# Shreyas911/MITgcm

Hardware: AMD Instinct MI355X
Metric: model-days/wallclock-sec (higher is better)
Workload: dtype f64; 1 GPU; BASELINE config 2, verification/global_ocean.90x40x15 as verified: 90x40x15 global lat-lon ocean, 1 tile of 90x40 (OL=3) on 1 GPU, restarted from the committed pickup at nIter0=36000; r* coordinate with non-linear free surface (UPDATE_CG2D every step), JMD95P, GM/Redi gkw91, CD scheme, biharmonic + harmonic viscosity, quasi-hydrostatic + NH metric + 3-D Coriolis, implicit vertical diffusion, IVDC,; tiles_per_gpu=1, parallelism=replicas1, cg2d=single-GPU kernel

## Files before the change

include/mitgcm_amd.h:

```cpp
#ifndef MITGCM_AMD_H
#define MITGCM_AMD_H

#include <stddef.h>

#ifdef __cplusplus
extern "C" {
#endif

typedef struct mgcm_model mgcm_model;

mgcm_model *mgcm_create(int sNx, int sNy, int OLx, int OLy, int Nr, int nSx, int nSy, int device);
void mgcm_destroy(mgcm_model *m);
const char *mgcm_last_error(void);

int mgcm_exch2_maps(int sNx, int sNy, int OL, int nTiles, int ldNb, int ldT, const int *tBasex, const int *tBasey,
                    const int *isNedge, const int *isSedge, const int *isEedge, const int *isWedge,
                    const int *nNeighbours, const int *neighbourId, const int *opposingSend, const int *pij,
                    const int *oi, const int *oj, const int *iLo, const int *iHi, const int *jLo, const int *jHi,
                    int useCubedSphereExchange, long *src, long *u1, long *v1, long *u0, long *v0);

int mgcm_set_param(mgcm_model *m, const char *name, double value);
double mgcm_get_param(mgcm_model *m, const char *name);

int mgcm_set_iter(mgcm_model *m, int myIter);
int mgcm_add_iter(mgcm_model *m, int inc);
int mgcm_tracer_parity(mgcm_model *m, int set);

int mgcm_ptracers_alloc(mgcm_model *m, int n);
int mgcm_ptracer_param(mgcm_model *m, int iTracer, const char *name, double value);
double mgcm_ptracer_param_get(mgcm_model *m, int iTracer, const char *name);
int mgcm_ptracers_count(mgcm_model *m);

int mgcm_put(mgcm_model *m, const char *name, const double *host, long count);
int mgcm_get(mgcm_model *m, const char *name, double *host, long count);
int mgcm_put_async(mgcm_model *m, const char *name, const double *host, long count);
int mgcm_put_batch_async(mgcm_model *m, int n, const char *const *names, const double *const *hosts,
                         const long *counts);
double *mgcm_device_ptr(mgcm_model *m, const char *name);

int mgcm_set_halo_map(mgcm_model *m, const long *src_of_point, long count);

int mgcm_set_uv_map(mgcm_model *m, const long *u1, const long *v1, const long *u0, const long *v0,
                    const int *tileFace, const int *tileEdge, long count);

int mgcm_init(mgcm_model *m);

int mgcm_thermodynamics(mgcm_model *m);
int mgcm_dynamics(mgcm_model *m);
int mgcm_solve_for_pressure(mgcm_model *m);
int mgcm_momentum_correction_step(mgcm_model *m);
int mgcm_integr_continuity(mgcm_model *m);
int mgcm_update_r_star(mgcm_model *m);
int mgcm_calc_r_star(mgcm_model *m);
int mgcm_blocking_exchanges(mgcm_model *m);
int mgcm_oceanic_phys(mgcm_model *m);
int mgcm_tracer_step(mgcm_model *m);
int mgcm_stagger_exchanges(mgcm_model *m);
int mgcm_exchange_host(mgcm_model *m, double *u, double *v, int nz, int vector, int withSigns);
const char *mgcm_param_name(int i);
long mgcm_field_count(mgcm_model *m, const char *name);
int mgcm_prepare(mgcm_model *m);
int mgcm_forward_step(mgcm_model *m, int nsteps);
int mgcm_set_tile_range(mgcm_model *m, int t0, int nT);
int mgcm_set_stream(mgcm_model *m, void *stream);
int mgcm_exchange_nfields(mgcm_model *m);
int mgcm_halo_pack(mgcm_model *m, const long *idx, long n, double *buf, int unpack);
int mgcm_exchange_nfields_group(mgcm_model *m, int group);
int mgcm_halo_pack_group(mgcm_model *m, int group, const long *idx, long n, double *buf, int unpack);
int mgcm_stream_handoff(mgcm_model *m, void *other, int direction);
int mgcm_tile_copy(mgcm_model *m, const char *name, int t0, int nT, void *buf, int toField);
int mgcm_begin_steps(mgcm_model *m);
int mgcm_end_steps(mgcm_model *m, int nsteps);
int mgcm_step_phase(mgcm_model *m, int phase);
int mgcm_cg2d_op(mgcm_model *m, int op, double a0, double *part);
int mgcm_cg2d_shared_bytes(mgcm_model *m);
int mgcm_cg2d_shared_export(mgcm_model *m, void *handle);
int mgcm_cg2d_shared_import(mgcm_model *m, const void *handle);
void *mgcm_get_stream(mgcm_model *m);
long mgcm_halo_sources(mgcm_model *m, int t0, int nT, long *out, long cap);
int mgcm_cg2d_tiles(mgcm_model *m, int t0, int nT);
int mgcm_cg2d_share(mgcm_model *m, mgcm_model *owner);
int mgcm_cg2d_record(mgcm_model *m, double firstResidual, double lastResidual, double rhsMax, double sumRHS,
                     int numIters, double minResidualSq, int nIterMin);
int mgcm_field_pack(mgcm_model *m, const char *name, const long *idx, long n, double *buf, int unpack);
int mgcm_exchange_field(mgcm_model *m, const char *name);

int mgcm_sync(mgcm_model *m);

int mgcm_cg2d(mgcm_model *m, double *cg2d_b, double *cg2d_x, double *firstResidual,
              double *minResidualSq, double *lastResidual, int *numIters, int *nIterMin);

int mgcm_cg2d_sum_plan(mgcm_model *m, int *plan, long capacity, int *NT, int *PPT, int *NG);

// ... 62 lines not shown
```

mitgcm_amd/_lib.py:

```python
import ctypes
import os

HERE = os.path.dirname(os.path.abspath(__file__))
LIBPATH = os.environ.get("MGCM_LIB") or os.path.join(HERE, "libmitgcm_amd.so")
_lib = None


class MgcmError(RuntimeError):
    pass


def lib():
    global _lib
    if _lib is not None:
        return _lib
    if not os.path.exists(LIBPATH):
        raise MgcmError("libmitgcm_amd.so not built (run __graft_entry__.build() or "
                        "python mitgcm_amd/build.py): the MI355X path has no CPU fallback")
    L = ctypes.CDLL(LIBPATH)
    vp, ci, cd, cs, cl = ctypes.c_void_p, ctypes.c_int, ctypes.c_double, ctypes.c_char_p, ctypes.c_long
    PD, PI, PL = ctypes.POINTER(cd), ctypes.POINTER(ci), ctypes.POINTER(cl)
    sig = {
        "mgcm_create": (vp, [ci] * 8),
        "mgcm_destroy": (None, [vp]),
        "mgcm_last_error": (cs, []),
        "mgcm_set_param": (ci, [vp, cs, cd]),
        "mgcm_set_iter": (ci, [vp, ci]),
        "mgcm_add_iter": (ci, [vp, ci]),
        "mgcm_exch2_maps": (ci, [ci] * 6 + [PI] * 16 + [ci] + [PL] * 5),
        "mgcm_tracer_parity": (ci, [vp, ci]),
        "mgcm_ptracers_alloc": (ci, [vp, ci]),
        "mgcm_ptracers_count": (ci, [vp]),
        "mgcm_ptracer_param": (ci, [vp, ci, cs, cd]),
        "mgcm_ptracer_param_get": (cd, [vp, ci, cs]),
        "mgcm_get_param": (cd, [vp, cs]),
        "mgcm_put": (ci, [vp, cs, PD, cl]),
        "mgcm_put_async": (ci, [vp, cs, PD, cl]),
        "mgcm_put_batch_async": (ci, [vp, ctypes.c_int, ctypes.POINTER(cs), ctypes.POINTER(PD), ctypes.POINTER(cl)]),
        "mgcm_get": (ci, [vp, cs, PD, cl]),
        "mgcm_device_ptr": (vp, [vp, cs]),
        "mgcm_set_halo_map": (ci, [vp, PL, cl]),
        "mgcm_set_uv_map": (ci, [vp, PL, PL, PL, PL, PI, PI, cl]),
        "mgcm_init": (ci, [vp]),
        "mgcm_dynamics": (ci, [vp]),
        "mgcm_thermodynamics": (ci, [vp]),
        "mgcm_prepare": (ci, [vp]),
        "mgcm_solve_for_pressure": (ci, [vp]),
        "mgcm_momentum_correction_step": (ci, [vp]),
        "mgcm_integr_continuity": (ci, [vp]),
        "mgcm_blocking_exchanges": (ci, [vp]),
        "mgcm_forward_step": (ci, [vp, ci]),
        "mgcm_sync": (ci, [vp]),
        "mgcm_cg2d": (ci, [vp, PD, PD, PD, PD, PD, PI, PI]),
        "mgcm_cg2d_sum_plan": (ci, [vp, PI, cl, PI, PI, PI]),
        "mgcm_solve_stats": (ci, [vp, ci, PD, PD, PI, PD]),
        "mgcm_solve_minres": (ci, [vp, ci, PD, PI]),
        "mgcm_stream_triad": (ci, [ci, cl, ci, PD]),
        "mgcm_solve_history": (ci, [vp, ci, PI, PD, PD]),
        "mgcm_monitor": (ci, [vp, PD]),
        "mgcm_kernel_ms": (cd, [vp, cs, PI]),
        "mgcm_kernel_timing": (None, [vp, ci]),
        "mgcm_set_tile_range": (ci, [vp, ci, ci]),
        "mgcm_set_stream": (ci, [vp, vp]),
        "mgcm_exchange_nfields": (ci, [vp]),
        "mgcm_halo_pack": (ci, [vp, vp, cl, vp, ci]),
        "mgcm_halo_pack_group": (ci, [vp, ci, vp, cl, vp, ci]),
        "mgcm_exchange_nfields_group": (ci, [vp, ci]),
        "mgcm_stream_handoff": (ci, [vp, vp, ci]),
        "mgcm_begin_steps": (ci, [vp]),
        "mgcm_end_steps": (ci, [vp, ci]),
        "mgcm_cg2d_shared_bytes": (ci, [vp]),
        "mgcm_cg2d_shared_export": (ci, [vp, vp]),
        "mgcm_cg2d_shared_import": (ci, [vp, vp]),
        "mgcm_tile_copy": (ci, [vp, cs, ci, ci, vp, ci]),
        "mgcm_step_phase": (ci, [vp, ci]),
        "mgcm_cg2d_op": (ci, [vp, ci, cd, vp]),
        "mgcm_cg2d_record": (ci, [vp, cd, cd, cd, cd, ci, cd, ci]),
        "mgcm_field_pack": (ci, [vp, cs, vp, cl, vp, ci]),
        "mgcm_exchange_field": (ci, [vp, cs]),
        "mgcm_oceanic_phys": (ci, [vp]),
        "mgcm_tracer_step": (ci, [vp]),
        "mgcm_stagger_exchanges": (ci, [vp]),
        "mgcm_exchange_host": (ci, [vp, PD, PD, ci, ci, ci]),
        "mgcm_field_count": (cl, [vp, cs]),
        "mgcm_param_name": (cs, [ci]),
        "mgcm_update_r_star": (ci, [vp]),
        "mgcm_calc_r_star": (ci, [vp]),
        "mgcm_get_stream": (vp, [vp]),
        "mgcm_halo_sources": (cl, [vp, ci, ci, PL, cl]),
        "mgcm_cg2d_tiles": (ci, [vp, ci, ci]),
        "mgcm_cg2d_share": (ci, [vp, vp]),
        "ini_cg2d_amd_": (None, [PI] * 6 + [PD] * 8 + [PI]),
        "cg2d_amd_": (None, [PD, PD, PD, PD, PD, PI, PI, PI]),
    }
    for name, (res, args) in sig.items():
        fn = getattr(L, name)
        fn.restype = res
        fn.argtypes = args
    _lib = L
    return L


EXPORTS = ["mgcm_create", "mgcm_destroy", "mgcm_last_error", "mgcm_set_param", "mgcm_get_param", "mgcm_put", "mgcm_put_async", "mgcm_put_batch_async",
           "mgcm_get", "mgcm_device_ptr", "mgcm_set_halo_map", "mgcm_set_uv_map", "mgcm_init", "mgcm_dynamics", "mgcm_thermodynamics",
           "mgcm_solve_for_pressure", "mgcm_momentum_correction_step", "mgcm_integr_continuity",
           "mgcm_blocking_exchanges", "mgcm_prepare", "mgcm_forward_step", "mgcm_sync", "mgcm_cg2d", "mgcm_cg2d_sum_plan", "mgcm_solve_stats", "mgcm_solve_minres", "mgcm_stream_triad", "mgcm_solve_history", "mgcm_monitor",
           "mgcm_kernel_ms", "mgcm_kernel_timing", "mgcm_set_tile_range", "mgcm_set_stream",
           "mgcm_exchange_nfields", "mgcm_halo_pack", "mgcm_tile_copy", "mgcm_begin_steps", "mgcm_step_phase", "mgcm_cg2d_op",
           "mgcm_cg2d_record", "mgcm_field_pack", "mgcm_exchange_field", "ini_cg2d_amd_",
           "cg2d_amd_", "mgcm_oceanic_phys", "mgcm_tracer_step", "mgcm_stagger_exchanges", "mgcm_exchange_host", "mgcm_field_count", "mgcm_param_name",
           "mgcm_amd_setup_", "mgcm_amd_param_", "mgcm_amd_bind_", "mgcm_amd_init_", "do_oceanic_phys_amd_",
           "thermodynamics_amd_", "dynamics_amd_", "solve_for_pressure_amd_", "momentum_correction_step_amd_",
           "integr_continuity_amd_", "do_fields_blocking_exchanges_amd_", "do_stagger_fields_exchanges_amd_", "exch_xy_rl_amd_", "exch_xyz_rl_amd_",
           "exch_uv_xy_rl_amd_", "exch_uv_xyz_rl_amd_", "global_sum_tile_rl_amd_",
           "mgcm_update_r_star", "mgcm_calc_r_star", "update_r_star_amd_", "update_cg2d_amd_", "calc_r_star_amd_",
           "mgcm_set_iter", "mgcm_add_iter", "mgcm_tracer_parity", "mgcm_exch2_maps", "mgcm_amd_host_sync_", "mgcm_amd_device_sync_", "mgcm_amd_transfer_stats_",
           "mgcm_amd_step_fence_", "mgcm_halo_pack_group", "mgcm_exchange_nfields_group", "mgcm_stream_handoff",
           "mgcm_end_steps", "mgcm_cg2d_shared_bytes", "mgcm_cg2d_shared_export", "mgcm_cg2d_shared_import",
           "mgcm_amd_set_maps_", "mgcm_amd_set_w2_", "mgcm_get_stream", "mgcm_halo_sources", "mgcm_cg2d_tiles", "mgcm_cg2d_share",
           "mgcm_ptracers_alloc", "mgcm_ptracers_count", "mgcm_ptracer_param", "mgcm_ptracer_param_get"]


def check(rc, what):
    if rc != 0:
        raise MgcmError("%s failed: %s" % (what, lib().mgcm_last_error().decode()))
```

mitgcm_amd/csrc/common.h:

```cpp
#pragma once
#include <hip/hip_runtime.h>
#include <stdint.h>
#include <stdlib.h>

namespace mgcm {

struct Dims {
  int sNx, sNy, OLx, OLy, Nr, nSx, nSy, nTiles;
  int t0, nT;
  int nx, ny;
  long n2, n3;
  long N2all, N3all;
};

#define MG_F2D_LIST(X) X(dxF) X(dyF) X(dxG) X(dyG) X(dxC) X(dyC) X(dxV) X(dyU) X(rA) X(rAw) X(rAs) X(recip_dxF) \
    X(recip_dyF) X(recip_dxC) X(recip_dyC) X(recip_dxV) X(recip_dyU) X(recip_rA) X(recip_rAw) X(recip_rAs) \
    X(fCori) X(Bo_surf) X(recip_Bo) X(tanPhiAtU) X(tanPhiAtV) X(maskInC) X(SST) X(lambdaThetaClimRelax) X(aW2d) \
    X(aS2d) X(aC2d) X(pW) X(pS) X(pC) X(etaN) X(fu) X(fv) X(etaH) X(surfaceForcingT) X(surfaceForcingS) \
    X(cg2d_b) X(cg2d_x) X(Qnet) X(EmPmR) X(SSS) X(lambdaSaltClimRelax) X(etaNm1) X(fCoriCos) X(recip_Rcol) \
    X(rSurfW) X(rSurfS) X(rLowW) X(rLowS) X(Ro_surf) X(R_low) X(rStarFacC) X(rStarFacW) X(rStarFacS) \
    X(rStarExpC) X(rStarExpW) X(rStarExpS) X(rStarDhCDt) X(rStarDhWDt) X(rStarDhSDt) X(PmEpR) X(dEtaHdt) \
    X(maskInW) X(maskInS) X(fCoriG) X(recip_rAz) X(recip_dxG) X(recip_dyG) X(etaHnm1) X(cg2d_r) X(cg2d_s) X(cg2d_q) \
    X(cg2d_min) X(cg2d_y) X(cg2d_v) X(EmPmRnext) X(rStarFacCPrev) X(rStarFacWPrev) X(rStarFacSPrev)
#define MG_F3D_LIST(X) X(hFacC) X(hFacW) X(hFacS) X(recip_hFacC) X(recip_hFacW) X(recip_hFacS) X(maskC) X(maskW) \
// ... 125 lines not shown
    if (q_ >= np_) return;                                                              \
    i = (i0) + q_ % (ni);                                                               \
    j = (j0) + q_ / (ni);                                                               \
  }
#define MG_PLANE_THREADS 256

__host__ __device__ inline int mg_col_kp(int Nr) { int kp = 1; while (kp < Nr) kp <<= 1; return kp; }
#define MG_COLS(i0, ni, j0, nj, Nr)                                                    \
  const int KP_ = mg_col_kp(Nr), NC_ = 256 / KP_;                                        \
  const int cc = (int)threadIdx.x % NC_, kk = (int)threadIdx.x / NC_;                   \
  const long col_ = (long)mg_xcd_block() * NC_ + cc;                                    \
  const long npl_ = (long)(ni) * (nj);                                                  \
  const bool valid = col_ < npl_ * d.nT;                                                \
  const int t = d.t0 + (int)(valid ? col_ / npl_ : 0);                                  \
  const int i = (i0) + (int)((valid ? col_ % npl_ : 0) % (ni));                         \
  const int j = (j0) + (int)((valid ? col_ % npl_ : 0) / (ni));
inline unsigned mg_col_blocks(int ni, int nj, int nT, int Nr) {
  const int nc = 256 / mg_col_kp(Nr);
  return (unsigned)(((long)ni * nj * nT + nc - 1) / nc);
}
#define MG_COLF(i0, ni, j0, nj, NCv)                                                   \
  const int NC_ = (NCv), KW_ = 256 / NC_;                                              \
  const int cc = (int)threadIdx.x % NC_, kk = (int)threadIdx.x / NC_;                  \
  const long col_ = (long)mg_xcd_block() * NC_ + cc;                                   \
  const long npl_ = (long)(ni) * (nj);                                                 \
  const bool valid = col_ < npl_ * d.nT;                                               \
  const int t = d.t0 + (int)(valid ? col_ / npl_ : 0);                                 \
  const int i = (i0) + (int)((valid ? col_ % npl_ : 0) % (ni));                        \
  const int j = (j0) + (int)((valid ? col_ % npl_ : 0) / (ni));
#define MG_COLF_LB(i0, ni, j0, nj, NCv, LB)                                            \
  const int NC_ = (NCv), KW_ = 256 / NC_;                                              \
  const int cc = (int)threadIdx.x % NC_, kk = (int)threadIdx.x / NC_;                  \
  const long col_ = (long)(LB) * NC_ + cc;                                             \
  const long npl_ = (long)(ni) * (nj);                                                 \
  const bool valid = col_ < npl_ * d.nT;                                               \
  const int t = d.t0 + (int)(valid ? col_ / npl_ : 0);                                 \
  const int i = (i0) + (int)((valid ? col_ % npl_ : 0) % (ni));                        \
  const int j = (j0) + (int)((valid ? col_ % npl_ : 0) / (ni));
#define MG_COLF_K(kvar) for (int kvar = kk + 1; kvar <= d.Nr; kvar += KW_)
inline int mg_colf_nc(long ncols, int Nr, int nArr) {
  (void)ncols; (void)Nr; (void)nArr;
  return 16;
}
inline size_t mg_colf_lds(int Nr, int nc, int nArr) { return (size_t)nArr * Nr * nc * sizeof(double); }
#define MG_ALLOW_LDS(kern)                                                                              \
  do {                                                                                                  \
    static const bool set_ = (hipFuncSetAttribute((const void *)(kern),                                 \
                                                  hipFuncAttributeMaxDynamicSharedMemorySize, 160 * 1024) == hipSuccess); \
    (void)set_;                                                                                         \
  } while (0)
inline unsigned mg_colf_blocks(long ncols, int nc) { return (unsigned)((ncols + nc - 1) / nc); }
enum { MG_FUSE_SFP = 1, MG_FUSE_PHI = 4, MG_FUSE_END = 8, MG_FUSE_TREX = 64, MG_FUSE_DT = 128, MG_FUSE_ETAX = 256,
       MG_FUSE_OPE = 1024, MG_FUSE_RING = 2048, MG_FUSE_RINGP = 4096, MG_FUSE_ENDS = 8192, MG_FUSE_PIPE = 16384,
       MG_FUSE_PHIP = 32768, MG_FUSE_SPEC = 65536 };
inline int mg_fuse_mask() {
  return getenv("MGCM_STEP_FUSE") ? atoi(getenv("MGCM_STEP_FUSE"))
                                  : MG_FUSE_SFP | MG_FUSE_PHI | MG_FUSE_END | MG_FUSE_DT | MG_FUSE_ETAX | MG_FUSE_OPE |
                                        MG_FUSE_RING | MG_FUSE_RINGP | MG_FUSE_ENDS | MG_FUSE_PIPE | MG_FUSE_PHIP | MG_FUSE_SPEC;
}
inline bool mg_fuse_on(int bit) { return (mg_fuse_mask() & bit) != 0; }
inline int mg_fuse_retired(const char **what) {
  static const struct { int bit; const char *what; } R[] = {
      {2, "EXCH(cg2d_x) + etaN in the single-workgroup CG2D's epilogue"},
      {16, "DO_OCEANIC_PHYS + CALC_PHI_HYD in one column pass"},
      {32, "EXCH(cg2d_x) + etaN on a third stream"},
      {512, "THERMODYNAMICS beside the pressure solve under r*"}};
  for (const auto &r : R)
    if (mg_fuse_mask() & r.bit) { *what = r.what; return r.bit; }
  return 0;
}
inline bool mg_hfuse(int bit, long nx, long ny, long nT, long Nr) {
  return mg_fuse_on(bit) && nx * ny * nT * Nr <= (1L << 21);
}
inline unsigned mg_plane_blocks(int ni, int nj, int nz) {
  return (unsigned)(((ni) * (nj) + MG_PLANE_THREADS - 1) / MG_PLANE_THREADS * (nz));
}

#define MG_OPT_LIST(X)                                                                              \
  X(momAdvection, p.momAdvection != 0, p.momAdvection != 0)        \
  X(momViscosity, p.momViscosity != 0, true)                                                        \
  X(momForcing, p.momForcing != 0, true)                                                            \
  X(rstar, p.nonlinFreeSurf > 0 && p.select_rStar > 0, true)                    \
  X(rstarOn, p.select_rStar > 0, true)                                                              \
  X(rstar2, p.select_rStar >= 2, true)                                                              \
  X(nlfs0, p.nonlinFreeSurf > 0, true)                                                              \
  X(nlfs2, p.nonlinFreeSurf > 1, true)                                                              \
  X(nlfs4, p.nonlinFreeSurf >= 4, true)                                                             \
  X(biharmonic, p.viscA4D != 0.0 || p.viscA4Z != 0.0, true)                                         \
  X(noSlipSides, p.no_slip_sides != 0, true)                                                        \
  X(noSlipBottom, p.no_slip_bottom != 0, true)                                                      \
  X(nhmTerms, p.useNHMTerms != 0, true)                                                             \
  X(metricSphere, p.metricSphere != 0, true)                                                        \
  X(coriolis, p.useCoriolis != 0, true)                                                             \
  X(cori3d, p.select3dCoriScheme >= 1, true)                                                        \
  X(cdScheme, p.useCDscheme != 0, true)                                                             \
  X(dissipInAB, p.momDissip_In_AB != 0, true)                                                       \
  X(forcingOutAB, p.momForcingOutAB == 1, false)                                                    \
  X(implicitViscosity, p.implicitViscosity != 0, false)                                             \
  X(gmAdvForm, p.GM_AdvForm != 0, false)                                                            \
  X(gmExtraDiag, p.GM_ExtraDiag != 0, false)                                                        \
  X(implicitDiffusion, p.implicitDiffusion != 0, true)                                              \
  X(tracForcingOutAB, p.tracForcingOutAB != 0, false)
struct OptsRun {
  static constexpr bool pinned = false;
#define MG_OPT_RUN(name, expr, pin) \
  __host__ __device__ __forceinline__ static bool name(const Params &p) { return (expr); }
  MG_OPT_LIST(MG_OPT_RUN)
#undef MG_OPT_RUN
};
struct OptsGO90 {
  static constexpr bool pinned = true;
#define MG_OPT_PIN(name, expr, pin) \
  __host__ __device__ __forceinline__ static constexpr bool name(const Params &p) { (void)p; return (pin); }
  MG_OPT_LIST(MG_OPT_PIN)
#undef MG_OPT_PIN
};
inline bool opts_match(const Params &p) {
#define MG_OPT_EQ(name, expr, pin) \
  if (OptsRun::name(p) != OptsGO90::name(p)) return false;
  MG_OPT_LIST(MG_OPT_EQ)
#undef MG_OPT_EQ
  return true;
}

__device__ __forceinline__ void sfp_rhs_column(const Dims &d, const Params &p, const Fields &f, long q, bool inner,
                                               const double *sE, const double *sW, const double *sN, const double *sS,
                                               int NC_, int cc) {
  if (p.useCDscheme) f.etaNm1[q] = f.etaN[q];
  f.cg2d_x[q] = f.Bo_surf[q] * f.etaN[q];
  double b = 0.0;
  if (inner) {
    if (p.useRealFreshWaterFlux) {
      const double tmpFac = p.freeSurfFac * (1.0 / p.rhoConst) * p.implicDiv2DFlow;
      b = tmpFac * f.rA[q] * f.EmPmR[q] / p.deltaTMom * f.maskInC[q];
    }
    for (int k2 = d.Nr; k2 >= 1; k2--) {
      const int s2 = (k2 - 1) * NC_ + cc;
      b = b + sE[s2] - sW[s2];
      b = b + sN[s2] - sS[s2];
    }
    b = b - p.freeSurfFac * f.rA[q] / p.deltaTMom / p.deltaTFreeSurf * (p.exactConserv ? f.etaH[q] : f.etaN[q]);
  }
  f.cg2d_b[q] = b;
}

struct TracerArgs {
  const double *tr;
  double *trNext;
  double *gNm1;
  double *scr;
  double *cp;
  const double *sfc;
  double diffKh, diffKr, dT;
  int advection, multiDim, useAB, forcing;
  int limiter;
  int scheme;
  double *gNm2;
  double relaxRate;
  double relaxVal;
  double src;
  int gm;
  double *adv1, *adv2, *gAdv;
  const double *advU, *advV, *advW;
};
__device__ __forceinline__ double ptr_surf_relax(const TracerArgs &a, double trSurf, double drF1, double hFacC1) {
  return (((a.relaxRate * (a.relaxVal - trSurf)) * drF1) * hFacC1);
}

#define MG_XMAX 8
struct XFields {
  double *p[MG_XMAX];
  int nz[MG_XMAX];
  int n;
};

__device__ __forceinline__ void exchange_multi_body(const Dims &d, const XFields &x, const long *__restrict__ map,
                                                    int nHalo, int *ctr, int hb, int k, int fi) {
  const int h = hb * (int)blockDim.x + (int)threadIdx.x;
  if (ctr && h == 0 && k == 0 && fi == 0) { ctr[0] += 1; ctr[1] += 1; }
  if (h >= nHalo || fi >= x.n || k >= x.nz[fi]) return;
  const long dst = map[2 * h], src = map[2 * h + 1];
  const long dt = dst / d.n2, dl = dst % d.n2, st = src / d.n2, sl = src % d.n2;
  const long lvl = (long)d.n2 * x.nz[fi];
  double *a = x.p[fi];
  a[dt * lvl + (long)k * d.n2 + dl] = a[st * lvl + (long)k * d.n2 + sl];
}

__device__ __forceinline__ void exchange_mixed_body(const Dims &d, double *u, double *v, int nzUV,
                                                    const long *__restrict__ uvMap, int nU, int nV, const XFields &x,
                                                    const long *__restrict__ map, int nHalo, int *ctr, int hb, int k,
                                                    int z) {
  const int h = hb * (int)blockDim.x + (int)threadIdx.x;
  if (ctr && h == 0 && k == 0 && z == 0) { ctr[0] += 1; ctr[1] += 1; }
  if (z == 0) {
    if (h >= nU + nV || k >= nzUV) return;
    const long dst = uvMap[2 * h], code = uvMap[2 * h + 1];
    const long N2 = d.n2 * d.nTiles, s = (code > 0 ? code : -code) - 1;
    const long n3 = d.n2 * nzUV, lvl = (long)k * d.n2;
    auto at = [&](long g) -> long { return (g / d.n2) * n3 + lvl + g % d.n2; };
    const double val = s < N2 ? u[at(s)] : v[at(s - N2)];
    (h < nU ? u : v)[at(dst)] = code > 0 ? val : -val;
    return;
  }
  const int fi = z - 1;
  if (h >= nHalo || fi >= x.n || k >= x.nz[fi]) return;
  const long dst = map[2 * h], src = map[2 * h + 1];
  const long dt = dst / d.n2, dl = dst % d.n2, st = src / d.n2, sl = src % d.n2;
  const long lvl = (long)d.n2 * x.nz[fi];
  double *a = x.p[fi];
  a[dt * lvl + (long)k * d.n2 + dl] = a[st * lvl + (long)k * d.n2 + sl];
}

struct MwgTables {
  const int *ownG;
  const int *ownC;
  const unsigned *ownNb;
  const unsigned *ownExp;
  const int *ringG;
  const unsigned *ringNb;
  const int *impC;
// ... 36 lines not shown
```

mitgcm_amd/csrc/gm_tensor.h:

```cpp
#pragma once
#include "common.h"

namespace mgcm {

__device__ __forceinline__ void gm_slope_gkw91(const Params &p, double dSx, double dSy, double dSr, double &SlopeX,
                                               double &SlopeY, double &SlopeSqr, double &taper) {
  const double GM_bigSlope = 1.0e+02, maxSlopeSqr = p.GM_maxSlope * p.GM_maxSlope;
  if (dSr != 0.0 && dSr <= p.GM_Small_Number) dSr = p.GM_Small_Number;
  if (dSr == 0.0) {
    SlopeX = dSx != 0.0 ? copysign(GM_bigSlope, dSx) : 0.0;
    SlopeY = dSy != 0.0 ? copysign(GM_bigSlope, dSy) : 0.0;
  } else {
    const double dRdSigmaLtd = 1.0 / dSr;
    SlopeX = dSx * dRdSigmaLtd;
    SlopeY = dSy * dRdSigmaLtd;
  }
  SlopeSqr = SlopeX * SlopeX + SlopeY * SlopeY;
  taper = 1.0;
  if (SlopeSqr >= p.GM_slopeSqCutoff) { SlopeSqr = p.GM_slopeSqCutoff; taper = 0.0; }
  if (SlopeSqr == 0.0) taper = 1.0;
  else if (SlopeSqr > maxSlopeSqr && SlopeSqr < p.GM_slopeSqCutoff) taper = maxSlopeSqr / SlopeSqr;
}

__device__ __forceinline__ void gm_tensor_body(const Dims &d, const Params &p, const Fields &f, int lb) {
  MG_PLANE_LB(2 - d.OLx, d.nx - 2, 2 - d.OLy, d.ny - 2, z, lb)
  const int t = d.t0 + z / d.Nr, k = z % d.Nr + 1;
  const int Nr = d.Nr;
  auto rho = [&](int ii, int jj, int kk) { return f.rhoInSitu[MG_I3(d, ii, jj, kk, t)]; };
  auto sX = [&](int ii, int jj, int kk) {
    return f.maskW[MG_I3(d, ii, jj, kk, t)] * f.recip_dxC[MG_I2(d, ii, jj, t)] * (rho(ii, jj, kk) - rho(ii - 1, jj, kk));
  };
  auto sY = [&](int ii, int jj, int kk) {
    return f.maskS[MG_I3(d, ii, jj, kk, t)] * f.recip_dyC[MG_I2(d, ii, jj, t)] * (rho(ii, jj, kk) - rho(ii, jj - 1, kk));
  };
  auto sR = [&](int ii, int jj, int kk) { return f.sigmaR[MG_I3(d, ii, jj, kk, t)]; };
  const double op25 = 0.25, op5 = 0.5, gs = p.gravitySign;
  const long q3 = MG_I3(d, i, j, k, t);
  const double isopycK = p.GM_isopycK * (1.0 + 1.0) * op5, bolus_K = p.GM_background_K * (1.0 + 1.0) * op5;
  double SlopeX, SlopeY, SlopeSqr, taper;
  double kwx = 0.0, kwy = 0.0, kwz = 0.0;
  if (k >= 2) {
    const double maskFk = f.maskC[MG_I3(d, i, j, k - 1, t)] * f.maskC[q3];
    const double dSx = op25 * (sX(i + 1, j, k - 1) + sX(i, j, k - 1) + sX(i + 1, j, k) + sX(i, j, k)) * maskFk;
    const double dSy = op25 * (sY(i, j + 1, k - 1) + sY(i, j, k - 1) + sY(i, j + 1, k) + sY(i, j, k)) * maskFk;
    gm_slope_gkw91(p, dSx, dSy, gs * sR(i, j, k), SlopeX, SlopeY, SlopeSqr, taper);
    kwx = -gs * SlopeX * taper;
    kwy = -gs * SlopeY * taper;
    kwz = SlopeSqr * taper;
  }
  const double Kgm_tmp = isopycK * 1.0 + p.GM_skewflx * bolus_K * 1.0;
  f.Kwx[q3] = Kgm_tmp * kwx;
  f.Kwy[q3] = Kgm_tmp * kwy;
  f.Kwz[q3] = (isopycK * 1.0) * kwz;
  const int kp1 = k + 1 < Nr ? k + 1 : Nr;
  const double maskp1 = k >= Nr ? 0.0 : 1.0;
  {
    const double mW = f.maskW[q3];
    const double dSx = sX(i, j, k) * mW;
    const double dSy = op25 * (sY(i - 1, j + 1, k) + sY(i, j + 1, k) + sY(i - 1, j, k) + sY(i, j, k)) * mW;
    const double dSr = op25 * (sR(i - 1, j, k) + sR(i, j, k) + (sR(i - 1, j, kp1) + sR(i, j, kp1)) * maskp1) * mW * gs;
    gm_slope_gkw91(p, dSx, dSy, dSr, SlopeX, SlopeY, SlopeSqr, taper);
    f.Kux[q3] = fmax((p.GM_isopycK * 1.0 * op5 * (1.0 + 1.0)) * taper, p.GM_Kmin_horiz);
    if (p.GM_ExtraDiag)
      f.Kuz[q3] = -gs * (p.GM_isopycK * 1.0 * op5 * (1.0 + 1.0) - p.GM_skewflx * p.GM_background_K * 1.0 * op5 * (1.0 + 1.0)) *
                  SlopeX * taper;
  }
  {
    const double mS = f.maskS[q3];
    const double dSx = op25 * (sX(i, j, k) + sX(i + 1, j, k) + sX(i, j - 1, k) + sX(i + 1, j - 1, k)) * mS;
    const double dSy = sY(i, j, k) * mS;
    const double dSr = op25 * (sR(i, j - 1, k) + sR(i, j, k) + (sR(i, j - 1, kp1) + sR(i, j, kp1)) * maskp1) * mS * gs;
    gm_slope_gkw91(p, dSx, dSy, dSr, SlopeX, SlopeY, SlopeSqr, taper);
    f.Kvy[q3] = fmax((p.GM_isopycK * 1.0 * op5 * (1.0 + 1.0)) * taper, p.GM_Kmin_horiz);
    if (p.GM_ExtraDiag)
      f.Kvz[q3] = -gs * (p.GM_isopycK * 1.0 * op5 * (1.0 + 1.0) - p.GM_skewflx * p.GM_background_K * 1.0 * op5 * (1.0 + 1.0)) *
                  SlopeY * taper;
  }
  if (p.GM_AdvForm) {
    double psx = 0.0, psy = 0.0;
    if (k >= 2) {
      const double halfRL = 0.5, halfSign = halfRL * gs, half_K = p.GM_background_K * (1.0 + 1.0) * op25;
      const double slopeCutoff = sqrt(p.GM_slopeSqCutoff), loc_maxSlope = p.GM_maxSlope * 1.0;
      const double maxSlopeSqr = loc_maxSlope * loc_maxSlope;
      auto psi = [&](double Slope, double dSdr) {
        if (dSdr <= p.GM_Small_Number) dSdr = p.GM_Small_Number;
        Slope = Slope / dSdr;
        double tp = 1.0;
        if (fabs(Slope) >= slopeCutoff) { Slope = copysign(slopeCutoff, Slope); tp = 0.0; }
        const double Smod = fabs(Slope);
        if (Smod > loc_maxSlope && Smod < slopeCutoff) tp = maxSlopeSqr / (Slope * Slope + p.GM_Small_Number);
        return Slope * tp * (half_K * (1.0 + 1.0));
      };
      const double mkW = f.maskW[MG_I3(d, i, j, k - 1, t)] * f.maskW[q3];
      psx = psi((sX(i, j, k - 1) + sX(i, j, k)) * halfRL * mkW, (sR(i - 1, j, k) + sR(i, j, k)) * halfSign * mkW);
      const double mkS = f.maskS[MG_I3(d, i, j, k - 1, t)] * f.maskS[q3];
      psy = psi((sY(i, j, k - 1) + sY(i, j, k)) * halfRL * mkS, (sR(i, j - 1, k) + sR(i, j, k)) * halfSign * mkS);
    }
    f.GM_PsiX[q3] = psx;
    f.GM_PsiY[q3] = psy;
  }
}

}
```

mitgcm_amd/csrc/kernels_dyn.hip:

```cpp
#include <cstdlib>

#include "common.h"
#include "launch.h"
#include "phys.h"
#include "rstar.h"
#include <cstring>
#include <cstdio>
#include <type_traits>

namespace mgcm {

__device__ __forceinline__ double hfacz(const Dims &d, const Fields &f, int i, int j, int k, int t) {
  if (i < 2 - d.OLx || j < 2 - d.OLy) return 0.0;
  double h = fmin(f.hFacW[MG_I3(d, i, j, k, t)], f.hFacW[MG_I3(d, i, j - 1, k, t)]);
  h = fmin(f.hFacS[MG_I3(d, i, j, k, t)], h);
  h = fmin(f.hFacS[MG_I3(d, i - 1, j, k, t)], h);
  return h;
}

template <class O = OptsRun>
__device__ __forceinline__ double h0facz(const Dims &d, const Params &p, const Fields &f, int i, int j, int k, int t) {
  if (!(O::momViscosity(p) && O::noSlipSides(p) && O::nlfs0(p))) return hfacz(d, f, i, j, k, t);
  if (i < 2 - d.OLx || j < 2 - d.OLy) return 0.0;
  return fmin(fmin(f.h0FacW[MG_I3(d, i, j, k, t)], f.h0FacW[MG_I3(d, i, j - 1, k, t)]),
              fmin(f.h0FacS[MG_I3(d, i, j, k, t)], f.h0FacS[MG_I3(d, i - 1, j, k, t)]));
}

template <bool HO = false>
__device__ __forceinline__ void del2uv_body(const Dims &d, const Params &p, const Fields &f, int lb,
                                            const long *__restrict__ srcOf = nullptr) {
  MG_PLANE_LB(1 - d.OLx, d.nx, 1 - d.OLy, d.ny, z, lb)
  const int t = d.t0 + z / d.Nr, k = z % d.Nr + 1;
  const long q3 = MG_I3(d, i, j, k, t);
  if (i < 2 - d.OLx || i > d.sNx + d.OLx - 1 || j < 2 - d.OLy || j > d.sNy + d.OLy - 1) {
    f.del2u[q3] = 0.0;
    f.del2v[q3] = 0.0;
    return;
  }
  const double drF = f.drF[k - 1];
  auto uv3 = [&](int ii, int jj) { return HO ? mg_at_source3(d, srcOf, ii, jj, k, t) : MG_I3(d, ii, jj, k, t); };
  const long qv[5] = {uv3(i, j), uv3(i - 1, j), uv3(i + 1, j), uv3(i, j - 1), uv3(i, j + 1)};
  auto qvAt = [&](int ii, int jj) { return qv[jj == j ? (ii == i ? 0 : ii < i ? 1 : 2) : (jj < j ? 3 : 4)]; };
#define U(ii, jj) f.uVel[HO ? qvAt(ii, jj) : MG_I3(d, ii, jj, k, t)]
#define V(ii, jj) f.vVel[HO ? qvAt(ii, jj) : MG_I3(d, ii, jj, k, t)]
#define G2(a, ii, jj) f.a[MG_I2(d, ii, jj, t)]
#define G3(a, ii, jj) f.a[MG_I3(d, ii, jj, k, t)]
  {
    auto fz = [&](int ii) { return drF * G3(hFacC, ii, j) * G2(dyF, ii, j) * G2(recip_dxF, ii, j) * (U(ii + 1, j) - U(ii, j)) * 1.0; };
    auto fm = [&](int jj) {
      return drF * hfacz(d, f, i, jj, k, t) * G2(dxV, i, jj) * G2(recip_dyU, i, jj) * (U(i, jj) - U(i, jj - 1));
    };
    double v4 = f.recip_drF[k - 1] * G3(recip_hFacW, i, j) * G2(recip_rAw, i, j) *
                (fz(i) - fz(i - 1) + fm(j + 1) - fm(j)) * G3(maskW, i, j);
    if (p.no_slip_sides) {
      const double hS = G3(h0FacW, i, j) - h0facz(d, p, f, i, j, k, t);
      const double hN = G3(h0FacW, i, j) - h0facz(d, p, f, i, j + 1, k, t);
      v4 = v4 - G3(recip_hFacW, i, j) * G2(recip_rAw, i, j) *
                    (hS * G2(dxV, i, j) * G2(recip_dyU, i, j) + hN * G2(dxV, i, j + 1) * G2(recip_dyU, i, j + 1)) * U(i, j) *
                    p.sideDragFactor * G3(maskW, i, j);
    }
    f.del2u[q3] = v4;
  }
  {
    auto fz = [&](int ii) {
      return drF * hfacz(d, f, ii, j, k, t) * G2(dyU, ii, j) * G2(recip_dxV, ii, j) * (V(ii, j) - V(ii - 1, j)) * 1.0;
    };
    auto fm = [&](int jj) { return drF * G3(hFacC, i, jj) * G2(dxF, i, jj) * G2(recip_dyF, i, jj) * (V(i, jj + 1) - V(i, jj)); };
    double v4 = f.recip_drF[k - 1] * G3(recip_hFacS, i, j) * G2(recip_rAs, i, j) *
                (fz(i + 1) - fz(i) + fm(j) - fm(j - 1)) * G3(maskS, i, j);
    if (p.no_slip_sides) {
      const double hW = G3(h0FacS, i, j) - h0facz(d, p, f, i, j, k, t);
      const double hE = G3(h0FacS, i, j) - h0facz(d, p, f, i + 1, j, k, t);
      v4 = v4 - G3(recip_hFacS, i, j) * G2(recip_rAs, i, j) *
                    (hW * G2(dyU, i, j) * G2(recip_dxV, i, j) + hE * G2(dyU, i + 1, j) * G2(recip_dxV, i + 1, j)) * V(i, j) *
                    p.sideDragFactor * G3(maskS, i, j);
    }
    f.del2v[q3] = v4;
  }
#undef U
#undef V
#undef G2
#undef G3
}
__global__ void __launch_bounds__(256) k_del2uv(Dims d, Params p, Fields f) { del2uv_body(d, p, f, mg_xcd_block()); }

template <bool HO = false>
__device__ __forceinline__ void phi_hyd_body(const Dims &d, const Params &p, const Fields &f, int nc, int lb,
                                             const long *__restrict__ srcOf = nullptr, int fromX = 0) {
  extern __shared__ __attribute__((aligned(16))) double lds[];
  MG_COLF_LB(-1, d.sNx + 3, -1, d.sNy + 3, nc, lb)
  const int Nr = d.Nr, NS = Nr * NC_;
  double *sM = lds, *sP = lds + NS, *sPh = lds + 2 * NS, *sC = lds + 3 * NS, *sU = lds + 4 * NS, *sV = lds + 5 * NS;
  const bool qh = p.quasiHydrostatic && (p.select3dCoriScheme >= 1 || p.useNHMTerms);
  const bool rstar = p.nonlinFreeSurf > 0 && p.select_rStar > 0;
  const bool ring = i >= 0 && j >= 0;
  const double recip_rhoConst = 1.0 / p.rhoConst;
  const long q2 = MG_I2(d, i, j, t);
  double hoFacC = 0.0, hoDhC = 0.0, hoDhW = 0.0, hoDhS = 0.0;
  const bool hoStash = HO && Nr >= 2 && KW_ >= 4;
  auto hoD0 = [&](long r) {
    double fc_ = 0.0, c_ = 0.0, w_ = 0.0, s_ = 0.0;
    if constexpr (HO) r_star_next_point<false>(d, p, f, srcOf, r, fromX, fc_, c_, w_, s_);
    return c_ * (f.Ro_surf[r] - f.R_low[r]) * f.rA[r];
  };
  bool hoHave = false;
  if (valid) MG_COLF_K(k) {
    const int me = (k - 1) * NC_ + cc;
    double dRlocM = 0.5 * f.drC[k - 1];
    if (k == 1) dRlocM = f.rF[0] - f.rC[0];
    const double dRlocP = (k == Nr) ? (f.rC[k - 1] - f.rF[k]) : 0.5 * f.drC[k];
    const long q3 = MG_I3(d, i, j, k, t);
    double hoOp[7] = {0.0, 0.0, 0.0, 0.0, 0.0, 0.0, 0.0};
    if constexpr (HO) {
      if (rstar) {
        hoOp[0] = f.drF[k - 1]; hoOp[1] = f.h0FacC[q3]; hoOp[2] = f.rA[q2];
        if (ring) { hoOp[3] = f.h0FacW[q3]; hoOp[4] = f.rAw[q2]; hoOp[5] = f.h0FacS[q3]; hoOp[6] = f.rAs[q2]; }
      }
    }
    double a = f.rhoInSitu[q3];
    if (qh) {
      const double scalingFactor = p.rhoConst * p.gravitySign * (1.0 / p.gravity);
      const long qc = HO ? mg_at_source3(d, srcOf, i, j, k, t) : q3;
      const long qe = HO ? mg_at_source3(d, srcOf, i + 1, j, k, t) : MG_I3(d, i + 1, j, k, t);
      const long qn = HO ? mg_at_source3(d, srcOf, i, j + 1, k, t) : MG_I3(d, i, j + 1, k, t);
      const double u0 = f.uVel[qc], u1 = f.uVel[qe];
      const double v0 = f.vVel[qc], v1 = f.vVel[qn];
      double gW = 0.0;
      if (p.select3dCoriScheme >= 1) gW = f.fCoriCos[q2] * (1.0 * 0.5 * (u0 + u1) - 0.0 * 0.5 * (v0 + v1));
      if (p.useNHMTerms) gW = gW + ((u0 * u0 + u1 * u1) + (v0 * v0 + v1 * v1)) * 0.5 * p.recip_rSphere;
      a = a + scalingFactor * gW;
    }
    if (rstar) f.alphaRho[q3] = a;
    sM[me] = dRlocM * p.gravity * a * recip_rhoConst;
    sP[me] = dRlocP * p.gravity * a * recip_rhoConst;
    if (rstar) {
      if constexpr (HO) {
        if (!hoHave) {
          r_star_next_point<true>(d, p, f, srcOf, q2, fromX, hoFacC, hoDhC, hoDhW, hoDhS);
          hoHave = true;
        }
        sC[me] = hoDhC * hoOp[0] * hoOp[1] * hoOp[2];
        if (ring) {
          sU[me] = hoDhW * hoOp[0] * hoOp[3] * hoOp[4];
          sV[me] = hoDhS * hoOp[0] * hoOp[5] * hoOp[6];
        }
      } else {
        const double drF = f.drF[k - 1];
        sC[me] = f.rStarDhCDt[q2] * drF * f.h0FacC[q3] * f.rA[q2];
        if (ring) {
          sU[me] = f.rStarDhWDt[q2] * drF * f.h0FacW[q3] * f.rAw[q2];
          sV[me] = f.rStarDhSDt[q2] * drF * f.h0FacS[q3] * f.rAs[q2];
        }
      }
    }
  }
  if constexpr (HO) {
    if (valid && rstar) {
      if (!hoHave && kk == 0) r_star_next_point<true>(d, p, f, srcOf, q2, fromX, hoFacC, hoDhC, hoDhW, hoDhS);
      if (hoStash && ring) {
        if (kk == KW_ / 4) sPh[cc] = hoD0(q2 - 1);
        if (kk == KW_ / 2) sPh[NC_ + cc] = hoD0(q2 - d.nx);
      }
    }
  }
  __syncthreads();
  if (valid && kk == 0) {
    double hoW = 0.0, hoS = 0.0;
    if constexpr (HO) {
      if (rstar && hoStash && ring) { hoW = sPh[cc]; hoS = sPh[NC_ + cc]; }
    }
    double phF = 0.0;
    for (int k2 = 1; k2 <= Nr; k2++) {
      const int s2 = (k2 - 1) * NC_ + cc;
      const double phC = phF + sM[s2];
      phF = phC + sP[s2];
      sPh[s2] = phC;
    }
    if (rstar) {
      auto d0 = [&](long r) {
        if constexpr (HO) {
          if (r == q2) return hoDhC * (f.Ro_surf[r] - f.R_low[r]) * f.rA[r];
          if (hoStash) return r == q2 - 1 ? hoW : hoS;
          return hoD0(r);
        } else {
          return f.rStarDhCDt[r] * (f.Ro_surf[r] - f.R_low[r]) * f.rA[r];
        }
      };
      double c = d0(q2);
      double u = ring ? 0.5 * (d0(q2 - 1) + c) : 0.0, v = ring ? 0.5 * (d0(q2 - d.nx) + c) : 0.0;
      for (int k2 = 1; k2 <= Nr; k2++) {
        const int s2 = (k2 - 1) * NC_ + cc;
        const double cc2 = sC[s2];
        sC[s2] = c;
        c = c - cc2;
        if (ring) {
          const double uu = sU[s2], vv = sV[s2];
          sU[s2] = u;
          sV[s2] = v;
          u = u - uu;
          v = v - vv;
        }
      }
    }
  }
  __syncthreads();
  if (valid) MG_COLF_K(k) {
    const int me = (k - 1) * NC_ + cc;
    const long q3 = MG_I3(d, i, j, k, t);
    if (rstar) {
      f.dWtC[q3] = sC[me];
      if (ring) { f.dWtU[q3] = sU[me]; f.dWtV[q3] = sV[me]; }
    }
    if (ring) {
      const double phC = sPh[me];
      f.phiHydC[q3] = phC;
      if (p.storePhiHyd4Phys) {
        double tot;
        if (rstar && p.nonlinFreeSurf >= 4) {
          const double dPhiRef = (f.Ro_surf[q2] - f.rC[k - 1]) * p.gravity;
          if constexpr (HO) tot = phC * hoFacC + fmax(dPhiRef, 0.0) * (hoFacC - 1.0) + 0.0;
          else tot = phC * f.rStarFacC[q2] + fmax(dPhiRef, 0.0) * (f.rStarFacC[q2] - 1.0) + 0.0;
        } else {
          tot = phC + f.Bo_surf[q2] * f.etaN[q2] + 0.0;
        }
        f.totPhiHyd[q3] = tot;
      }
    }
  }
}
__global__ void __launch_bounds__(256) k_phi_hyd(Dims d, Params p, Fields f, int nc) {
  phi_hyd_body(d, p, f, nc, mg_xcd_block());
}
constexpr int PHI_CH = 10;
template <bool RS, bool QH, int NRC = 0>
__device__ __forceinline__ void phi_flat_body(const Dims &d, const Params &p, const Fields &f, int lb) {
  constexpr int o = RS ? 1 : 0;
// ... 1848 lines not shown
```

mitgcm_amd/csrc/kernels_rstar.hip:

```cpp
#include "common.h"
#include "launch.h"
#include "phys.h"
#include "rstar.h"
#include "ucg2d.h"

namespace mgcm {

template <bool FUSE>
__global__ void __launch_bounds__(256) k_calc_r_star(Dims d, Params p, Fields f, const long *__restrict__ srcOf, int fromX) {
  calc_r_star_body<FUSE>(d, p, f, srcOf, (int)blockIdx.x, fromX);
}
template <bool FUSE>
__global__ void __launch_bounds__(256) k_rstar_exch(Dims d, Params p, Fields f, const long *__restrict__ srcOf, int nbR,
                                                    XFields x, const long *__restrict__ map, int nHalo, int *ctr, int nbX,
                                                    int nzMax, int fromX, int empNext) {
  const int b = (int)blockIdx.x;
  if (b < nbR) { calc_r_star_body<FUSE>(d, p, f, srcOf, b, fromX, empNext); return; }
  const int r = b - nbR;
  exchange_multi_body(d, x, map, nHalo, ctr, r % nbX, (r / nbX) % nzMax, r / (nbX * nzMax));
}

template <bool FUSE>
__global__ void __launch_bounds__(256) k_rstar_exmix(Dims d, Params p, Fields f, const long *__restrict__ srcOf, int nbR,
                                                     int fromX, double *u, double *v, int nzUV,
                                                     const long *__restrict__ uvMap, int nU, int nV, XFields x,
                                                     const long *__restrict__ map, int nHalo, int nbH, int nzMax) {
  const int b = (int)blockIdx.x;
  if (b < nbR) { calc_r_star_body<FUSE>(d, p, f, srcOf, b, fromX); return; }
  const int r = b - nbR;
  exchange_mixed_body(d, u, v, nzUV, uvMap, nU, nV, x, map, nHalo, nullptr, r % nbH, (r / nbH) % nzMax, r / (nbH * nzMax));
}

template <bool SFP, int PH>
__global__ void __launch_bounds__(256) k_update_r_star_cg2d_a(Dims d, Params p, Fields f, int nc, int opIn,
                                                              const long *__restrict__ srcOf, int nbPc,
                                                              const int *iterPtr, int nbPh) {
  extern __shared__ __attribute__((aligned(16))) double lds[];
  int lb = mg_xcd_block();
  if constexpr (PH != 0) {
    if (lb < nbPh) { phys_hoist_body(d, p, f, iterPtr, srcOf, lb); return; }
    lb -= nbPh;
  }
  if (lb < nbPc) { ucg2d_p_point(d, p, f, srcOf, lb); return; }
  lb -= nbPc;
  MG_COLF_LB(1 - d.OLx, d.nx, 1 - d.OLy, d.ny, nc, lb)
  const int NS = d.Nr * NC_;
  double *sW = lds, *sS = lds + NS;
  double *fE = lds + 2 * NS, *fW = lds + 3 * NS, *fN = lds + 4 * NS, *fS = lds + 5 * NS;
  const long q = MG_I2(d, i, j, t);
  const bool op = opIn && p.nonlinFreeSurf > 2 && i >= 1 && i <= d.sNx + 1 && j >= 1 && j <= d.sNy + 1;
  const bool inner = i >= 1 && i <= d.sNx && j >= 1 && j <= d.sNy;
  if (valid) {
    const double fc = f.rStarFacC[q], fw = f.rStarFacW[q], fs = f.rStarFacS[q];
    if constexpr (PH == 2) {
      if (kk == 0) { f.rStarFacCPrev[q] = fc; f.rStarFacWPrev[q] = fw; f.rStarFacSPrev[q] = fs; }
    }
    double fwE = 0.0, fsN = 0.0;
    if (SFP && inner) { fwE = f.rStarFacW[MG_I2(d, i + 1, j, t)]; fsN = f.rStarFacS[MG_I2(d, i, j + 1, t)]; }
    MG_COLF_K(k) {
      const long q3 = MG_I3(d, i, j, k, t);
      const double hC = f.h0FacC[q3] * fc, hW = f.h0FacW[q3] * fw, hS = f.h0FacS[q3] * fs;
      f.hFacC[q3] = hC;
      f.hFacW[q3] = hW;
      f.hFacS[q3] = hS;
      if (f.maskC[q3] != 0.0) f.recip_hFacC[q3] = 1.0 / hC;
      if (f.maskW[q3] != 0.0) f.recip_hFacW[q3] = 1.0 / hW;
      if (f.maskS[q3] != 0.0) f.recip_hFacS[q3] = 1.0 / hS;
      const int me = (k - 1) * NC_ + cc;
      if (op) {
        double faceArea = f.dyG[q] * f.drF[k - 1] * hW;
        sW[me] = faceArea * f.recip_dxC[q];
        faceArea = f.dxG[q] * f.drF[k - 1] * hS;
        sS[me] = faceArea * f.recip_dyC[q];
      }
      if (SFP) {
        if (p.useCDscheme) {
          f.uNM1[q3] = f.uVel[q3];
          f.vNM1[q3] = f.vVel[q3];
        }
        if (inner) {
          const double drF = f.drF[k - 1];
          const long qE = MG_I3(d, i + 1, j, k, t), qN = MG_I3(d, i, j + 1, k, t);
          fE[me] = f.dyG[MG_I2(d, i + 1, j, t)] * drF * (f.h0FacW[qE] * fwE) * f.gU[qE] / p.deltaTMom;
          fW[me] = f.dyG[q] * drF * hW * f.gU[q3] / p.deltaTMom;
          fN[me] = f.dxG[MG_I2(d, i, j + 1, t)] * drF * (f.h0FacS[qN] * fsN) * f.gV[qN] / p.deltaTMom;
          fS[me] = f.dxG[q] * drF * hS * f.gV[q3] / p.deltaTMom;
        }
      }
    }
  }
  __syncthreads();
  if (!valid || kk != 0) return;
  if (opIn && p.nonlinFreeSurf > 2) {
    double aW = 0.0, aS = 0.0;
    if (op) {
      for (int k = 1; k <= d.Nr; k++) {
        const int me = (k - 1) * NC_ + cc;
        aW = aW + sW[me];
        aS = aS + sS[me];
      }
      aW = aW * p.cg2dNorm * p.implicSurfPress * p.implicDiv2DFlow;
      aS = aS * p.cg2dNorm * p.implicSurfPress * p.implicDiv2DFlow;
    }
    f.aW2d[q] = aW;
    f.aS2d[q] = aS;
  }
  if (SFP) sfp_rhs_column(d, p, f, q, inner, fE, fW, fN, fS, NC_, cc);
}

__global__ void __launch_bounds__(256) k_update_cg2d_p(Dims d, Params p, Fields f, const long *__restrict__ srcOf) {
  ucg2d_p_point(d, p, f, srcOf, (int)blockIdx.x);
}

hipError_t launch_calc_r_star(const Dims &d, const Params &p, const Fields &f, const long *srcOf, hipStream_t s,
                              bool fuseEtaH, int fromX) {
  const long n = d.n2 * d.nTiles;
  hipLaunchKernelGGL(fuseEtaH ? k_calc_r_star<true> : k_calc_r_star<false>, dim3((unsigned)((n + 255) / 256)), dim3(256),
                     0, s, d, p, f, srcOf, fromX);
  return hipGetLastError();
}

hipError_t launch_rstar_exch(const Dims &d, const Params &p, const Fields &f, const long *srcOf, bool fuseEtaH,
                             const XFields &x, const long *map, int nHalo, int *ctr, hipStream_t s, int fromX, int empNext) {
  const long n = d.n2 * d.nTiles;
  const int nbR = (int)((n + 255) / 256);
  int nzMax = 1;
  for (int q = 0; q < x.n; q++) nzMax = x.nz[q] > nzMax ? x.nz[q] : nzMax;
  const int nbX = ((nHalo > 0 ? nHalo : 1) + 255) / 256;
  const unsigned nb = (unsigned)(nbR + nbX * nzMax * (x.n > 0 ? x.n : 1));
  hipLaunchKernelGGL(fuseEtaH ? k_rstar_exch<true> : k_rstar_exch<false>, dim3(nb), dim3(256), 0, s, d, p, f, srcOf, nbR, x,
                     map, nHalo, ctr, nbX, nzMax, fromX, fuseEtaH ? empNext : 0);
  return hipGetLastError();
}

hipError_t launch_rstar_exmix(const Dims &d, const Params &p, const Fields &f, const long *srcOf, bool fuseEtaH, int fromX,
                              double *u, double *v, int nzUV, const long *uvMap, int nU, int nV, const XFields &x,
                              const long *map, int nHalo, hipStream_t s) {
  const long n = d.n2 * d.nTiles;
  const int nbR = (int)((n + 255) / 256);
  int nzMax = nzUV;
  for (int q = 0; q < x.n; q++) nzMax = x.nz[q] > nzMax ? x.nz[q] : nzMax;
  const int nh = (nU + nV) > nHalo ? nU + nV : nHalo;
  const int nbH = ((nh > 0 ? nh : 1) + 255) / 256;
  const unsigned nb = (unsigned)(nbR + nbH * nzMax * (1 + x.n));
  hipLaunchKernelGGL(fuseEtaH ? k_rstar_exmix<true> : k_rstar_exmix<false>, dim3(nb), dim3(256), 0, s, d, p, f, srcOf, nbR,
                     fromX, u, v, nzUV, uvMap, nU, nV, x, map, nHalo, nbH, nzMax);
  return hipGetLastError();
}

hipError_t launch_update_r_star_cg2d(const Dims &d, const Params &p, const Fields &f, const long *srcOf, hipStream_t s,
                                     bool sfp, bool opEarly, bool pcHere, const int *iterPtr, bool keepFac) {
  const long n = d.n2 * d.nTiles;
  const unsigned nb = (unsigned)((n + 255) / 256);
  const long ncol = (long)d.nx * d.ny * d.nT;
  const int nArr = sfp ? 6 : 2;
  const int nc = mg_colf_nc(ncol, d.Nr, nArr);
  auto kPlain = k_update_r_star_cg2d_a<false, 0>, kSfp = k_update_r_star_cg2d_a<true, 0>,
       kSfpPhys = k_update_r_star_cg2d_a<true, 1>, kSfpPhysKeep = k_update_r_star_cg2d_a<true, 2>;
  MG_ALLOW_LDS(kPlain);
  MG_ALLOW_LDS(kSfp);
  const int nbPc = (opEarly && pcHere && p.nonlinFreeSurf > 2) ? (int)nb : 0;
  if (iterPtr) {
    if (!sfp) return hipErrorInvalidValue;
    MG_ALLOW_LDS(kSfpPhys);
    MG_ALLOW_LDS(kSfpPhysKeep);
    const int nbPh = phys_hoist_blocks(d);
    hipLaunchKernelGGL(keepFac ? kSfpPhysKeep : kSfpPhys, dim3(mg_colf_blocks(ncol, nc) + (unsigned)(nbPc + nbPh)), dim3(256),
                       mg_colf_lds(d.Nr, nc, nArr), s, d, p, f, nc, opEarly ? 0 : 1, srcOf, nbPc, iterPtr, nbPh);
  } else if (keepFac) {
    return hipErrorInvalidValue;
  } else
    hipLaunchKernelGGL(sfp ? kSfp : kPlain, dim3(mg_colf_blocks(ncol, nc) + (unsigned)nbPc), dim3(256),
                       mg_colf_lds(d.Nr, nc, nArr), s, d, p, f, nc, opEarly ? 0 : 1, srcOf, nbPc, (const int *)nullptr, 0);
  if (p.nonlinFreeSurf > 2 && !opEarly) hipLaunchKernelGGL(k_update_cg2d_p, dim3(nb), dim3(256), 0, s, d, p, f, srcOf);
  return hipGetLastError();
}

}
```

mitgcm_amd/csrc/kernels_solve.hip:

```cpp
#include <cstdlib>

#include "cg2d.h"
#include "launch.h"
#include "gm_tensor.h"

namespace mgcm {

constexpr int CG_THREADS = 1024;
constexpr int CG_WAVES = CG_THREADS / 64;

template <int CTRL>
__device__ __forceinline__ double dpp_f64(double v) {
  const long long b = __builtin_bit_cast(long long, v);
  const int lo = __builtin_amdgcn_mov_dpp((int)(b & 0xffffffff), CTRL, 0xF, 0xF, true);
  const int hi = __builtin_amdgcn_mov_dpp((int)(b >> 32), CTRL, 0xF, 0xF, true);
  return __builtin_bit_cast(double, ((long long)hi << 32) | (unsigned)lo);
}
__device__ __forceinline__ double row_sum16(double v) {
  v = v + dpp_f64<0xB1>(v);
  v = v + dpp_f64<0x4E>(v);
  v = v + dpp_f64<0x141>(v);
  v = v + dpp_f64<0x140>(v);
  return v;
}
// ... 831 lines not shown
  (h < nU ? u : v)[at(dst)] = code > 0 ? val : -val;
}

struct UVPairs {
  double *u[3], *v[3];
  int n;
};
__global__ void __launch_bounds__(256) k_exchange_uv_pairs(Dims d, UVPairs pr, const long *__restrict__ map, int nU,
                                                           int nV) {
  const int h = (int)(blockIdx.x * blockDim.x + threadIdx.x);
  const int c = (int)blockIdx.y;
  if (h >= nU + nV || c >= pr.n) return;
  double *u = pr.u[c], *v = pr.v[c];
  const long dst = map[2 * h], code = map[2 * h + 1];
  const long N2 = d.n2 * d.nTiles, s = (code > 0 ? code : -code) - 1;
  const double val = s < N2 ? u[s] : v[s - N2];
  (h < nU ? u : v)[dst] = code > 0 ? val : -val;
}

__global__ void __launch_bounds__(256) k_exchange_mixed(Dims d, double *u, double *v, int nzUV,
                                                        const long *__restrict__ uvMap, int nU, int nV, XFields x,
                                                        const long *__restrict__ map, int nHalo, int *ctr) {
  exchange_mixed_body(d, u, v, nzUV, uvMap, nU, nV, x, map, nHalo, ctr, (int)blockIdx.x, (int)blockIdx.y, (int)blockIdx.z);
}

__global__ void __launch_bounds__(256) k_exch_eta(Dims d, Fields f, const long *__restrict__ srcOf) {
  const long q = (long)blockIdx.x * blockDim.x + threadIdx.x;
  if (q >= d.n2 * d.nTiles) return;
  const long sq = srcOf[q];
  double x = f.cg2d_x[q];
  if (sq >= 0) { x = f.cg2d_x[sq]; f.cg2d_x[q] = x; }
  f.etaN[q] = f.recip_Bo[q] * x;
}

__global__ void __launch_bounds__(256) k_exch_etaH(Dims d, Params p, Fields f, const long *__restrict__ srcOf, int atInit,
                                                   int fromX) {
  const long q = (long)blockIdx.x * blockDim.x + threadIdx.x;
  if (q >= d.n2 * d.nTiles) return;
  if (!atInit && p.nonlinFreeSurf > 0 && p.useRealFreshWaterFlux) f.PmEpR[q] = -f.EmPmR[q];
  const long sq = srcOf[q];
  const double *e = f.cg2d_b;
  double x;
  if (sq >= 0) x = e[sq];
  else {
    const long l = q % d.n2;
    const int i = (int)(l % d.nx) - d.OLx + 1, j = (int)(l / d.nx) - d.OLy + 1;
    x = (i >= 1 && i <= d.sNx && j >= 1 && j <= d.sNy) ? e[q] : fromX ? f.recip_Bo[q] * f.cg2d_x[q] : f.etaN[q];
  }
  f.etaHnm1[q] = f.etaH[q];
  f.etaN[q] = x;
  f.etaH[q] = x;
}

template <bool GM>
__global__ void __launch_bounds__(256) k_corr_cont(Dims d, Params p, Fields f, int atInit, int nc,
                                                   const long *__restrict__ etaSrc, int nbGm) {
  extern __shared__ __attribute__((aligned(16))) double lds[];
  int lb = mg_xcd_block();
  if constexpr (GM) {
    if (lb < nbGm) { gm_tensor_body(d, p, f, lb); return; }
    lb -= nbGm;
  }
  MG_COLF_LB(1, d.sNx, 1, d.sNy, nc, lb)
  const int NS = d.Nr * NC_;
  double *sDiv = lds, *sMask = lds + NS, *sU = lds + 2 * NS, *sV = lds + 3 * NS, *sH0 = lds + 4 * NS;
  const long q = MG_I2(d, i, j, t);
  const bool rstar = p.nonlinFreeSurf > 0 && p.select_rStar != 0;
  if (valid && atInit != 0) MG_COLF_K(k) {
    const int me = (k - 1) * NC_ + cc;
    const double drF = f.drF[k - 1];
    const double u0 = f.uVel[MG_I3(d, i, j, k, t)], u1 = f.uVel[MG_I3(d, i + 1, j, k, t)];
    const double v0 = f.vVel[MG_I3(d, i, j, k, t)], v1 = f.vVel[MG_I3(d, i, j + 1, k, t)];
    const double uT1 = u1 * f.dyG[MG_I2(d, i + 1, j, t)] * drF * f.hFacW[MG_I3(d, i + 1, j, k, t)];
    const double uT0 = u0 * f.dyG[q] * drF * f.hFacW[MG_I3(d, i, j, k, t)];
    const double vT1 = v1 * f.dxG[MG_I2(d, i, j + 1, t)] * drF * f.hFacS[MG_I3(d, i, j + 1, k, t)];
    const double vT0 = v0 * f.dxG[q] * drF * f.hFacS[MG_I3(d, i, j, k, t)];
    sDiv[me] = uT1 - uT0 + vT1 - vT0;
    sMask[me] = f.maskC[MG_I3(d, i, j, k, t)];
    if (rstar) sH0[me] = f.h0FacC[MG_I3(d, i, j, k, t)];
  } else if (valid) {
    const double psFac = p.pfFacMom * p.implicSurfPress;
    auto eta = [&](long qq) {
      if (!etaSrc) return f.etaN[qq];
      const long sq = etaSrc[qq];
      return f.recip_Bo[qq] * f.cg2d_x[sq >= 0 ? sq : qq];
    };
    auto phiX = [&](int ii, int jj) {
      const long qq = MG_I2(d, ii, jj, t);
      return f.recip_dxC[qq] * (f.Bo_surf[qq] * eta(qq) - f.Bo_surf[MG_I2(d, ii - 1, jj, t)] * eta(MG_I2(d, ii - 1, jj, t)));
    };
    auto phiY = [&](int ii, int jj) {
      const long qq = MG_I2(d, ii, jj, t);
      return f.recip_dyC[qq] * (f.Bo_surf[qq] * eta(qq) - f.Bo_surf[MG_I2(d, ii, jj - 1, t)] * eta(MG_I2(d, ii, jj - 1, t)));
    };
    const double pX0 = phiX(i, j), pX1 = phiX(i + 1, j), pY0 = phiY(i, j), pY1 = phiY(i, j + 1);
    MG_COLF_K(k) {
      const int me = (k - 1) * NC_ + cc;
      const long q3c = MG_I3(d, i, j, k, t), q3e = MG_I3(d, i + 1, j, k, t), q3n = MG_I3(d, i, j + 1, k, t);
      const double hW0 = f.hFacW[q3c], hW1 = f.hFacW[q3e], hS0 = f.hFacS[q3c], hS1 = f.hFacS[q3n];
      auto uCor = [&](long q3, double hW, double phiSurfX) {
        const double mW = hW != 0.0 ? 1.0 : 0.0;
        return (f.gU[q3] + p.deltaTMom * (-psFac * phiSurfX * mW)) * mW;
      };
      auto vCor = [&](long q3, double hS, double phiSurfY) {
        const double mS = hS != 0.0 ? 1.0 : 0.0;
        return (f.gV[q3] + p.deltaTMom * (-psFac * phiSurfY * mS)) * mS;
      };
      const double u0 = uCor(q3c, hW0, pX0), u1 = uCor(q3e, hW1, pX1);
      const double v0 = vCor(q3c, hS0, pY0), v1 = vCor(q3n, hS1, pY1);
      sU[me] = u0;
      sV[me] = v0;
      const double drF = f.drF[k - 1];
      const double uT1 = u1 * f.dyG[MG_I2(d, i + 1, j, t)] * drF * hW1;
      const double uT0 = u0 * f.dyG[q] * drF * hW0;
      const double vT1 = v1 * f.dxG[MG_I2(d, i, j + 1, t)] * drF * hS1;
      const double vT0 = v0 * f.dxG[q] * drF * hS0;
      sDiv[me] = uT1 - uT0 + vT1 - vT0;
      sMask[me] = f.maskC[MG_I3(d, i, j, k, t)];
      if (rstar) sH0[me] = f.h0FacC[MG_I3(d, i, j, k, t)];
    }
  }
  __syncthreads();
  if (valid && kk == 0) {
    double rStarDhDt = 0.0;
    if (p.exactConserv) {
      double hDiv = 0.0;
      for (int k2 = 1; k2 <= d.Nr; k2++) hDiv = hDiv + sMask[(k2 - 1) * NC_ + cc] * sDiv[(k2 - 1) * NC_ + cc];
      double dEtaHdt;
      if (atInit == 1 && p.nIter0 != 0 && p.useRealFreshWaterFlux) {
        dEtaHdt = f.dEtaHdt[q];
        double pm = dEtaHdt + hDiv * f.recip_rA[q];
        f.PmEpR[q] = pm * p.rhoConst;
        f.cg2d_b[q] = f.etaN[q];
      } else if (atInit == 1) {
        dEtaHdt = -(hDiv * f.recip_rA[q]);
        if (f.PmEpR) f.PmEpR[q] = 0.0;
        f.cg2d_b[q] = f.etaN[q];
      } else {
        const double facEmP = p.useRealFreshWaterFlux ? 1.0 / p.rhoConst : 0.0;
        dEtaHdt = -(hDiv * f.recip_rA[q]) - facEmP * f.EmPmR[q];
        f.cg2d_b[q] = f.etaH[q] + p.implicDiv2DFlow * dEtaHdt * p.deltaTFreeSurf;
      }
      if (f.dEtaHdt) f.dEtaHdt[q] = dEtaHdt;
      if (rstar) rStarDhDt = dEtaHdt * f.recip_Rcol[q];
    }
    double wBelow = 0.0;
    const double rA1 = f.recip_rA[q];
    for (int k2 = d.Nr; k2 >= 1; k2--) {
      const int s2 = (k2 - 1) * NC_ + cc;
      const double conv2d = -sDiv[s2];
      double w;
      if (rstar) {
        const double dh = rStarDhDt * f.drF[k2 - 1] * sH0[s2];
        if (k2 == d.Nr) w = (conv2d * rA1 - dh) * sMask[s2];
        else w = (wBelow + conv2d * rA1 - dh) * sMask[s2];
      } else if (k2 == d.Nr) {
        w = conv2d * rA1 * sMask[s2];
      } else {
        w = (wBelow + conv2d * rA1) * sMask[s2];
      }
      sDiv[s2] = w;
      wBelow = w;
    }
  }
  __syncthreads();
  if (valid) MG_COLF_K(k) {
    const int me = (k - 1) * NC_ + cc;
    const long q3 = MG_I3(d, i, j, k, t);
    f.wVel[q3] = sDiv[me];
    if (atInit == 0) { f.uVel[q3] = sU[me]; f.vVel[q3] = sV[me]; }
  }
}

template <int NR>
__device__ __forceinline__ void corr_cont_column(const Dims &d, const Params &p, long q, long q3b, long nx, long n2,
                                                 double pX0, double pX1, double pY0, double pY1, double dyG0, double dyG1,
                                                 double dxG0, double dxG1, double rA1, const double *__restrict__ gU,
                                                 const double *__restrict__ gV, const double *__restrict__ hFacW,
                                                 const double *__restrict__ hFacS, const double *__restrict__ maskC,
                                                 const double *__restrict__ drFv, double *__restrict__ uVel,
                                                 double *__restrict__ vVel, double *__restrict__ wVel, double &hDiv) {
  const double psFac = p.pfFacMom * p.implicSurfPress;
  auto uCor = [&](long q3, double hW, double phiSurfX) {
    const double mW = hW != 0.0 ? 1.0 : 0.0;
    return (gU[q3] + p.deltaTMom * (-psFac * phiSurfX * mW)) * mW;
  };
  auto vCor = [&](long q3, double hS, double phiSurfY) {
    const double mS = hS != 0.0 ? 1.0 : 0.0;
    return (gV[q3] + p.deltaTMom * (-psFac * phiSurfY * mS)) * mS;
  };
  double prod[NR];
  double wBelow = 0.0;
// ... 178 lines not shown
  hipLaunchKernelGGL(k_correction, grd, blk, 0, s, d, p, f);
  return hipGetLastError();
}

hipError_t launch_exchange_multi(const Dims &d, const XFields &x, const long *map, int nHalo, int *ctr, hipStream_t s) {
  int nzMax = 1;
  for (int q = 0; q < x.n; q++) nzMax = x.nz[q] > nzMax ? x.nz[q] : nzMax;
  dim3 blk(256), grd((unsigned)((nHalo > 0 ? nHalo : 1) + 255) / 256, nzMax, x.n);
  hipLaunchKernelGGL(k_exchange_multi, grd, blk, 0, s, d, x, map, nHalo, ctr);
  return hipGetLastError();
}

hipError_t launch_exchange_mixed(const Dims &d, double *u, double *v, int nzUV, const long *uvMap, int nU, int nV,
                                 const XFields &x, const long *map, int nHalo, int *ctr, hipStream_t s) {
  int nzMax = nzUV;
  for (int q = 0; q < x.n; q++) nzMax = x.nz[q] > nzMax ? x.nz[q] : nzMax;
  const int nh = (nU + nV) > nHalo ? nU + nV : nHalo;
  dim3 blk(256), grd((unsigned)((nh > 0 ? nh : 1) + 255) / 256, nzMax, 1 + x.n);
  hipLaunchKernelGGL(k_exchange_mixed, grd, blk, 0, s, d, u, v, nzUV, uvMap, nU, nV, x, map, nHalo, ctr);
  return hipGetLastError();
}

hipError_t launch_exchange_uv(const Dims &d, double *u, double *v, const long *map, int nU, int nV, int nz,
                              hipStream_t s) {
  if (nU + nV <= 0) return hipSuccess;
  Dims dz = d;
  dz.n3 = d.n2 * nz;
  hipLaunchKernelGGL(k_exchange_uv, dim3((unsigned)((nU + nV + 255) / 256), nz), dim3(256), 0, s, dz, u, v, map, nU,
                     nV);
  return hipGetLastError();
}

hipError_t launch_exchange_uv_pairs(const Dims &d, double *const *u, double *const *v, int n, const long *map, int nU,
                                   int nV, hipStream_t s) {
  if (nU + nV <= 0 || n <= 0) return hipSuccess;
  if (n > 3) return hipErrorInvalidValue;
  UVPairs pr{};
  for (int c = 0; c < n; c++) { pr.u[c] = u[c]; pr.v[c] = v[c]; }
  pr.n = n;
  hipLaunchKernelGGL(k_exchange_uv_pairs, dim3((unsigned)((nU + nV + 255) / 256), n), dim3(256), 0, s, d, pr, map, nU,
                     nV);
  return hipGetLastError();
}

hipError_t launch_exch_eta(const Dims &d, const Params &p, const Fields &f, const long *srcOf, bool etaH, int atInit,
                           hipStream_t s, int fromX) {
  const long n = d.n2 * d.nTiles;
  if (etaH) hipLaunchKernelGGL(k_exch_etaH, dim3((unsigned)((n + 255) / 256)), dim3(256), 0, s, d, p, f, srcOf, atInit, fromX);
  else hipLaunchKernelGGL(k_exch_eta, dim3((unsigned)((n + 255) / 256)), dim3(256), 0, s, d, f, srcOf);
  return hipGetLastError();
}

hipError_t launch_corr_cont(const Dims &d, const Params &p, const Fields &f, int atInit, hipStream_t s,
                            const long *etaSrc, bool gmNext) {
  const long ncol = (long)d.sNx * d.sNy * d.nT;
  const int nArr = (p.nonlinFreeSurf > 0 && p.select_rStar != 0) ? 5 : 4;
  if (atInit == 0 && !(p.nonlinFreeSurf > 0 && p.select_rStar != 0) && d.Nr == 50) {
    if (gmNext) return hipErrorInvalidValue;
    hipLaunchKernelGGL(k_corr_cont_march<50>, dim3((unsigned)((ncol + 255) / 256)), dim3(256), 0, s, d, p, f, etaSrc);
    return hipGetLastError();
  }
  const int nc = d.Nr >= 30 ? 32 : 16;
  if (gmNext) {
    const int nbGm = (int)mg_plane_blocks(d.nx - 2, d.ny - 2, d.nT * d.Nr);
    MG_ALLOW_LDS(k_corr_cont<true>);
    hipLaunchKernelGGL(k_corr_cont<true>, dim3(mg_colf_blocks(ncol, nc) + (unsigned)nbGm), dim3(256),
                       mg_colf_lds(d.Nr, nc, nArr), s, d, p, f, atInit, nc, etaSrc, nbGm);
    return hipGetLastError();
  }
  MG_ALLOW_LDS(k_corr_cont<false>);
  hipLaunchKernelGGL(k_corr_cont<false>, dim3(mg_colf_blocks(ncol, nc)), dim3(256), mg_colf_lds(d.Nr, nc, nArr), s, d, p, f,
                     atInit, nc, etaSrc, 0);
  return hipGetLastError();
}

hipError_t launch_halo_pack(const Dims &d, const XFields &x, const long *idx, long n, double *buf, int unpack,
                            hipStream_t s) {
  if (n <= 0) return hipSuccess;
  hipLaunchKernelGGL(k_halo_pack, dim3((unsigned)((n + 255) / 256), d.Nr, x.n), dim3(256), 0, s, d, x, idx, n, buf,
                     unpack);
  return hipGetLastError();
}

hipError_t launch_bump_counter(int *c, int nIncr, hipStream_t s) {
  hipLaunchKernelGGL(k_bump_counter, dim3(1), dim3(64), 0, s, c, nIncr);
  return hipGetLastError();
}

}
```

mitgcm_amd/csrc/kernels_step.hip:

```cpp
#include "launch.h"
#include "kernels_dyn.hip"
#include "kernels_thermo.hip"
#include "ucg2d.h"
#include "rstar.h"

namespace mgcm {

template <bool GM>
__global__ void __launch_bounds__(256) k_dt_front(Dims d, Params p, Fields f, TracerArgs aT, TracerArgs aS,
                                                  const int *iterPtr, int nc, int nbPhi, int nbDel, int nbTr) {
  int lb = mg_xcd_block();
  if (lb < nbPhi) { phi_hyd_body(d, p, f, nc, lb); return; }
  lb -= nbPhi;
  if (lb < nbDel) { del2uv_body(d, p, f, lb); return; }
  lb -= nbDel;
  if (lb < nbTr) tracer_rhs_body_br<GM>(d, p, f, aT, iterPtr, lb);
  else tracer_rhs_body_br<GM>(d, p, f, aS, iterPtr, lb - nbTr);
}

__global__ void __launch_bounds__(256) k_dt_back(Dims d, Params p, Fields f, TracerArgs aT, TracerArgs aS,
                                                 const int *iterPtr, int nc, int nbMom, int nbImp) {
  int lb = mg_xcd_block();
  if (lb < nbMom) {
    if (lb & 1) mom_step_point<false, 2>(d, p, f, iterPtr, lb >> 1);
// ... 194 lines not shown
  const int nc = mg_colf_nc(ncol, d.Nr, 3);
  const int nbImp = (int)mg_colf_blocks(ncol, nc);
  MG_ALLOW_LDS(k_tr_impl_pair);
  hipLaunchKernelGGL(k_tr_impl_pair, dim3((unsigned)(2 * nbImp)), dim3(256), mg_colf_lds(d.Nr, nc, 3), s, d, p, f, aT, aS, nc,
                     nbImp);
  return hipGetLastError();
}

hipError_t launch_dyn_thermo(const Dims &d, const Params &p, const Fields &f, const TracerArgs &aT, const TracerArgs &aS,
                             const int *iterPtr, hipStream_t s, const long *srcOf, bool gmHere, bool l1Here, bool spec) {
  const dim3 blk(256);
  int ncPhi, nArrPhi, nbPhi;
  phi_frame(d, p, ncPhi, nArrPhi, nbPhi);
  const int nbDel = del2_needed(p) ? (int)mg_plane_blocks(d.nx, d.ny, d.nT * d.Nr) : 0;
  const int nbTr = (int)mg_plane_blocks(d.sNx, d.sNy, d.nT * d.Nr);
  if (dyn_thermo_takes_gm(p)) {
    const int nbU = srcOf ? ucg2d_blocks(d) : 0;
    const int nbOp1 = 0, nbPc2 = 0, nbOp2 = nbU, nbPc3 = nbU;
    if (l1Here) launch_l1(d, p, f, nbDel, s, nbOp1, gmHere);
    else if (gmHere) return hipErrorInvalidValue;
    const bool ff4 = mom_ff4_on(true);
    const int nbMom = ff4 ? mom_ff4_blocks(d) : 2 * (int)mg_plane_blocks(d.nx, d.ny, d.nT * d.Nr);
    if (spec && (ff4 || !opts_match(p))) return hipErrorInvalidValue;
    auto l2 = ff4 ? k_dt_l2<true, true> : spec ? k_dt_l2<true, false, OptsGO90> : k_dt_l2<true, false>;
    hipLaunchKernelGGL(l2, dim3((unsigned)(nbPc2 + nbOp2 + nbMom + 2 * nbTr)), blk, 0, s, d, p, f, aT, aS, iterPtr, nbMom, nbTr,
                       srcOf, nbPc2, nbOp2, dt_long_first());
    const long ncolTr = (long)d.sNx * d.sNy * d.nT;
    const int ncTr = mg_colf_nc(ncolTr, d.Nr, 3);
    const int nbImp = (int)mg_colf_blocks(ncolTr, ncTr);
    const int nbCd = (int)mg_plane_blocks(d.nx - 2, d.ny - 2, d.nT * d.Nr);
    MG_ALLOW_LDS(k_dt_l3<OptsRun>);
    MG_ALLOW_LDS(k_dt_l3<OptsGO90>);
    auto l3 = spec ? k_dt_l3<OptsGO90> : k_dt_l3<OptsRun>;
    hipLaunchKernelGGL(l3, dim3((unsigned)(nbPc3 + nbCd + 2 * nbImp)), blk, mg_colf_lds(d.Nr, ncTr, 3), s, d, p, f, aT,
                       aS, iterPtr, ncTr, nbCd, nbImp, srcOf, nbPc3, dt_long_first());
    return hipGetLastError();
  }
  if (srcOf || !gmHere || !l1Here || spec) return hipErrorInvalidValue;
  MG_ALLOW_LDS(k_dt_front<true>);
  hipLaunchKernelGGL(k_dt_front<true>, dim3((unsigned)(nbPhi + nbDel + 2 * nbTr)), blk,
                     mg_colf_lds(d.Nr, ncPhi, nArrPhi), s, d, p, f, aT, aS, iterPtr, ncPhi, nbPhi, nbDel, nbTr);
  const int nbMom = 2 * (int)mg_plane_blocks(d.nx, d.ny, d.nT * d.Nr);
  const long ncolTr = (long)d.sNx * d.sNy * d.nT;
  const int ncTr = mg_colf_nc(ncolTr, d.Nr, 3);
  const int nbImp = (int)mg_colf_blocks(ncolTr, ncTr);
  MG_ALLOW_LDS(k_dt_back);
  hipLaunchKernelGGL(k_dt_back, dim3((unsigned)(nbMom + 2 * nbImp)), blk, mg_colf_lds(d.Nr, ncTr, 3), s, d, p, f, aT, aS,
                     iterPtr, ncTr, nbMom, nbImp);
  const hipError_t e = hipGetLastError();
  if (e != hipSuccess) return e;
  return launch_mom_tail(d, p, f, iterPtr, s);
}

__global__ void __launch_bounds__(256) k_rstar_exch_phi(Dims d, Params p, Fields f, const long *__restrict__ srcOf, int nbR,
                                                        XFields x, const long *__restrict__ map, int nHalo, int *ctr,
                                                        int nbX, int nzMax, int nbXall, int fromX, int empNext, int nc,
                                                        int nbPhi) {
  int lb = mg_xcd_block();
  if (lb < nbPhi) { phi_hyd_body<true>(d, p, f, nc, lb, srcOf, fromX); return; }
  lb -= nbPhi;
  if (lb < nbR) { calc_r_star_body<true>(d, p, f, srcOf, lb, fromX, empNext); return; }
  lb -= nbR;
  if (lb < nbXall) { exchange_multi_body(d, x, map, nHalo, ctr, lb % nbX, (lb / nbX) % nzMax, lb / (nbX * nzMax)); return; }
  del2uv_body<true>(d, p, f, lb - nbXall, srcOf);
}

bool phi_pipe_ok(const Dims &d, const Params &p) {
  (void)d;
  return mg_fuse_on(MG_FUSE_PHIP) && p.nonlinFreeSurf > 0 && p.select_rStar > 0 && p.exactConserv && !p.cubeCorners &&
         dyn_thermo_takes_gm(p) && !phi_flat_on(p);
}

hipError_t launch_phi_del2(const Dims &d, const Params &p, const Fields &f, hipStream_t s) {
  launch_l1(d, p, f, del2_needed(p) ? (int)mg_plane_blocks(d.nx, d.ny, d.nT * d.Nr) : 0, s, 0, false);
  return hipGetLastError();
}

hipError_t launch_rstar_exch_phi(const Dims &d, const Params &p, const Fields &f, const long *srcOf, const XFields &x,
                                 const long *map, int nHalo, int *ctr, hipStream_t s, int fromX, int empNext) {
  if (!phi_pipe_ok(d, p) || !srcOf || d.nT != d.nTiles) return hipErrorInvalidValue;
  const long n = d.n2 * d.nTiles;
  const int nbR = (int)((n + 255) / 256);
  int nzMax = 1;
  for (int q = 0; q < x.n; q++) nzMax = x.nz[q] > nzMax ? x.nz[q] : nzMax;
  const int nbX = ((nHalo > 0 ? nHalo : 1) + 255) / 256;
  const int nbXall = nbX * nzMax * (x.n > 0 ? x.n : 1);
  int nc, nArr, nbPhi;
  phi_frame(d, p, nc, nArr, nbPhi);
  const int nbDel = del2_needed(p) ? (int)mg_plane_blocks(d.nx, d.ny, d.nT * d.Nr) : 0;
  MG_ALLOW_LDS(k_rstar_exch_phi);
  hipLaunchKernelGGL(k_rstar_exch_phi, dim3((unsigned)(nbPhi + nbR + nbXall + nbDel)), dim3(256), mg_colf_lds(d.Nr, nc, nArr),
                     s, d, p, f, srcOf, nbR, x, map, nHalo, ctr, nbX, nzMax, nbXall, fromX, empNext, nc, nbPhi);
  return hipGetLastError();
}

}

#include "kernels_ptracers.hip"
```

mitgcm_amd/csrc/launch.h:

```cpp
#pragma once
#include "common.h"

namespace mgcm {

hipError_t launch_mom_step(const Dims &, const Params &, const Fields &, const int *, hipStream_t, bool ring = true);
bool mom_ring_separable(const Dims &, const Params &);
hipError_t launch_mom_ring(const Dims &, const Params &, const Fields &, const int *, hipStream_t);
hipError_t launch_phys_ring(const Dims &, const Params &, const Fields &, const int *, hipStream_t);
hipError_t launch_phi_hyd(const Dims &, const Params &, const Fields &, hipStream_t);

hipError_t launch_sfp_rhs(const Dims &, const Params &, const Fields &, hipStream_t);
hipError_t launch_exchange(const Dims &, double *, const long *, int, int, hipStream_t);
hipError_t launch_correction(const Dims &, const Params &, const Fields &, hipStream_t);
hipError_t launch_bump_counter(int *, int, hipStream_t);
hipError_t launch_exchange_multi(const Dims &, const XFields &, const long *, int, int *, hipStream_t);
hipError_t launch_exchange_uv(const Dims &, double *, double *, const long *, int, int, int, hipStream_t);
hipError_t launch_exchange_mixed(const Dims &, double *, double *, int, const long *, int, int, const XFields &,
                                 const long *, int, int *, hipStream_t);
hipError_t launch_exchange_uv_pairs(const Dims &, double *const *, double *const *, int, const long *, int, int,
                                   hipStream_t);
hipError_t launch_exch_eta(const Dims &, const Params &, const Fields &, const long *, bool, int, hipStream_t,
                           int fromX = 0);
hipError_t launch_corr_cont(const Dims &, const Params &, const Fields &, int, hipStream_t, const long *etaSrc = nullptr,
                            bool gmNext = false);
hipError_t launch_halo_pack(const Dims &, const XFields &, const long *, long, double *, int, hipStream_t);

hipError_t launch_cgd(const Dims &, const Params &, const Fields &, int, double, double *, hipStream_t);
hipError_t launch_cgd_record(SolveRecord *, const int *, double, double, double, double, int, double, int, hipStream_t);
hipError_t launch_field_pack(double *, const long *, long, double *, int, hipStream_t);

hipError_t launch_calc_r_star(const Dims &, const Params &, const Fields &, const long *, hipStream_t, bool fuseEtaH = false,
                              int fromX = 0);
hipError_t launch_rstar_exmix(const Dims &, const Params &, const Fields &, const long *, bool, int, double *, double *, int,
                              const long *, int, int, const XFields &, const long *, int, hipStream_t);
hipError_t launch_rstar_exch(const Dims &, const Params &, const Fields &, const long *, bool, const XFields &, const long *,
                             int, int *, hipStream_t, int fromX = 0, int empNext = 0);
hipError_t launch_update_r_star_cg2d(const Dims &, const Params &, const Fields &, const long *, hipStream_t, bool sfp = false,
                                     bool opEarly = false, bool pcHere = false, const int *iterPtr = nullptr,
                                     bool keepFac = false);

bool phys_ring_ok(const Dims &, const Params &, const Fields &);
hipError_t launch_oceanic_phys(const Dims &, const Params &, const Fields &, const int *, hipStream_t, bool gm = true,
                               bool ring = false);
hipError_t launch_tracer_step(const Dims &, const Params &, const Fields &, const TracerArgs &, const int *, hipStream_t,
                              bool impl = true, int *nLaunch = nullptr);
hipError_t launch_gm_tensor(const Dims &, const Params &, const Fields &, hipStream_t);
hipError_t launch_gm_residual_flow(const Dims &, const Params &, const Fields &, hipStream_t);

bool dyn_thermo_fusable(const Dims &, const Params &, const TracerArgs &, const TracerArgs &);
hipError_t launch_dyn_thermo(const Dims &, const Params &, const Fields &, const TracerArgs &, const TracerArgs &, const int *,
                             hipStream_t, const long *srcOf = nullptr, bool gmHere = true, bool l1Here = true, bool spec = false);
bool dyn_thermo_spec_ok(const Params &);
bool phi_pipe_ok(const Dims &, const Params &);
hipError_t launch_phi_del2(const Dims &, const Params &, const Fields &, hipStream_t);
hipError_t launch_rstar_exch_phi(const Dims &, const Params &, const Fields &, const long *, const XFields &, const long *, int,
                                 int *, hipStream_t, int fromX, int empNext);
bool dyn_thermo_takes_gm(const Params &);
bool gm_phi_fusable(const Dims &, const Params &);
hipError_t launch_gm_phi(const Dims &, const Params &, const Fields &, hipStream_t, bool op = false);
bool tracer_hpair_ok(const Dims &, const Params &, const TracerArgs &, const TracerArgs &);
hipError_t launch_tracer_hpair(const Dims &, const Params &, const Fields &, const TracerArgs &, const TracerArgs &,
                               const int *, hipStream_t);

hipError_t launch_mon_stats(const Dims &, const MonSpecs &, int, double *, int, hipStream_t);

bool ptr_batch_ok(const Dims &, const Params &, bool md);
hipError_t launch_ptracers_batch(const Dims &, const Params &, const Fields &, const TracerArgs *, const int *, int, int, int,
                                 int, const int *, hipStream_t, int *nLaunch = nullptr);

}
```

mitgcm_amd/csrc/model.hip:

```cpp
#include <hip/hip_runtime.h>

#include <cmath>
#include <cstdarg>
#include <cstdio>
#include <cstdlib>
#include <cstring>
#include <algorithm>
#include <map>
#include <utility>
#include <string>
#include <vector>

#include "../../include/mitgcm_amd.h"
#include "cg2d.h"
#include "launch.h"

namespace mgcm {
static std::vector<std::pair<uintptr_t, uintptr_t>> g_hostReg;
void mg_host_ranges_set(const uintptr_t *lo, const uintptr_t *hi, size_t n) {
  g_hostReg.clear();
  for (size_t i = 0; i < n; i++) g_hostReg.push_back({lo[i], hi[i]});
  std::sort(g_hostReg.begin(), g_hostReg.end());
}
hipError_t mg_host_copy(void *dst, const void *src, size_t bytes, hipMemcpyKind kind, hipStream_t s) {
// ... 57 lines not shown
struct PDesc {
  const char *name;
  size_t off;
  bool isint;
};
#define PD(n) {#n, offsetof(Params, n), false}
#define PI_(n) {#n, offsetof(Params, n), true}
static const PDesc PARAMS[] = {
    PD(deltaTMom), PD(deltaTFreeSurf), PD(deltaTClock), PD(abEps), PD(alph_AB), PD(beta_AB), PI_(useAB3), PD(rhoConst), PD(gBaro), PD(viscAhD), PD(viscAhZ),
    PD(viscA4D), PD(viscA4Z), PD(viscAr), PD(sideDragFactor), PD(freeSurfFac), PD(implicSurfPress),
    PD(implicDiv2DFlow), PD(rkSign), PD(afFacMom), PD(vfFacMom), PD(pfFacMom), PD(cfFacMom), PD(foFacMom),
    PD(mtFacMom), PD(cg2dNorm), PD(cg2dTolerance_sq),
    PI_(momAdvection), PI_(momViscosity), PI_(momForcing), PI_(useCoriolis), PI_(no_slip_sides),
    PI_(no_slip_bottom), PI_(selectCoriScheme), PI_(momForcingOutAB), PI_(momDissip_In_AB),
    PI_(implicitViscosity), PI_(cg2dMaxIters), PI_(cg2dUseMinResSol), PI_(cg2dNormaliseRHS), PI_(nIter0), PI_(cg2dUseFMA), PI_(useSRCGSolver), PI_(cg2dRefOrder),
    PD(gravity), PD(gravitySign), PD(rhoNil), PD(tAlpha), PD(sBeta), PD(ivdc_kappa), PD(diffKhT), PD(diffKrT),
    PD(deltaTtracer), PI_(exactConserv), PI_(tempStepping), PI_(tempAdvection), PI_(tempForcing),
    PI_(implicitDiffusion), PI_(tempAdvScheme), PI_(saltStepping), PI_(saltAdvection), PI_(saltForcing),
    PI_(saltAdvScheme), PD(diffKhS), PD(diffKrS), PI_(multiDimAdvection), PI_(multiDimCompressible), PI_(momStepping),
    PI_(eosType), PI_(allowFreezing), PI_(useRealFreshWaterFlux), PI_(useCDscheme), PI_(useGMRedi),
    PI_(periodicExternalForcing), PI_(nForcRec), PD(HeatCapacity_Cp), PD(convertFW2Salt), PD(temp_EvPrRn),
    PD(salt_EvPrRn), PD(rCD), PD(epsAB_CD), PD(externForcingPeriod), PD(externForcingCycle), PD(GM_background_K),
    PD(GM_isopycK), PD(GM_skewflx), PD(GM_maxSlope), PD(GM_Kmin_horiz), PD(GM_Small_Number), PD(GM_slopeSqCutoff),
    PI_(GM_AdvForm), PI_(GM_ExtraDiag),
    PI_(nonlinFreeSurf), PI_(select_rStar), PI_(quasiHydrostatic), PI_(useNHMTerms), PI_(select3dCoriScheme),
    PI_(selectP_inEOS_Zc), PI_(storePhiHyd4Phys), PD(hFacInf),
    PI_(vectorInvariantMomentum), PI_(selectVortScheme), PI_(selectKEscheme), PI_(upwindShear),
    PI_(staggerTimeStep), PI_(tracForcingOutAB),
};
#undef PD
#undef PI_

enum Kern { K_MOM, K_RHS, K_CG2D, K_EXCH, K_ETA, K_CORR, K_CONT, K_PHYS, K_TEMP, K_RSTAR, K_PHI, K_N };
static const char *KNAMES[K_N] = {"mom_step",   "sfp_rhs",    "cg2d",         "exchange",  "eta_update",
                                  "correction", "continuity", "oceanic_phys", "temp_step", "r_star", "phi_hyd"};

enum StepSeq { SEQ_PLAIN2 = 0, SEQ_HOIST2, SEQ_HOIST_LAST, SEQ_PLAIN1, SEQ_LAST1, SEQ_N };

struct mgcm_model {
  Dims d{};
  Params p{};
  Fields f{};
  int device = 0;
  hipStream_t stream = nullptr;
  hipStream_t ownStream = nullptr;
  hipStream_t stream2 = nullptr;
  hipEvent_t evFork = nullptr, evJoin = nullptr;
  hipEvent_t evHand = nullptr;
  bool overlap = true;
  std::vector<void *> allocs;
  std::map<std::string, double> extra;
  long *d_halo = nullptr;
  long *d_srcOf = nullptr;
  int nHalo = 0;
  long *d_haloAll = nullptr;
  int nHaloAll = 0;
  std::vector<long> h_halo;
  enum class Cg2dSolver { Bxy = 3, Mwg = 4, BlockRef = 5, MwgRef = 6 };
  Cg2dSolver solver = Cg2dSolver::Bxy;
  bool useMwg() const { return solver == Cg2dSolver::Mwg || solver == Cg2dSolver::MwgRef; }
  int nPts = 0;
  unsigned *d_nbr = nullptr;
  int *d_gofs = nullptr;
  unsigned *d_nbx = nullptr;
  int *d_blkx = nullptr;
  int nBlkX = 0;
  int bxyVar = -1;
  std::vector<int> h_dropG;
  int *d_dropG = nullptr;
  int nDropBlk = 0;
  bool noCompact = false;
  int *h_guard = nullptr;
  int *d_guard = nullptr;
  bool latlonTopology = true;
  MwgTables mwg{};
  std::vector<void *> mwgAllocs;
  void *mwgShared = nullptr;
  void *mwgBlock = nullptr;
  std::vector<int> mwgPlan;
  bool uvMap = false;
  std::vector<long> h_uv[2];
  long *d_uv[2] = {nullptr, nullptr};
  int nUvU[2] = {0, 0}, nUvV[2] = {0, 0};
  long *d_uvAll[2] = {nullptr, nullptr};
  int nUvUAll[2] = {0, 0}, nUvVAll[2] = {0, 0};
  struct UvPre { const long *map = nullptr; int nU = 0, nV = 0; } uvPre[2][2];
  int *d_tileInfo = nullptr;
  double *exchBuf[2] = {nullptr, nullptr};
  long exchCap = 0;
  bool useGraph = true;
  struct StepGraph {
    hipGraphExec_t exec = nullptr;
    double *tr[4] = {};
    int flip = 0;
    int layout = 0;
  };
  StepGraph graphs[2][8][SEQ_N];
  bool ovlAuto = false, ovlDecided = false;
  float ovlMs[2] = {0.f, 0.f};
  hipEvent_t ovlEv[2] = {nullptr, nullptr};
  double *thetaA = nullptr, *saltA = nullptr;
  int stepLayout = 0;
  int ptrRoute = 0, ptrLaunches = 0;
  int gmResFlow = 0;
  struct PTracer {
    int advScheme = 2, useGMRedi = -1;
// ... 72 lines not shown
    m->evPool.push_back(e);
  }
  return (int)m->evUsed++;
}
static int ev_begin(mgcm_model *m, int k) {
  (void)k;
  if (!m->timing) return -1;
  const int i = ev_next(m);
  if (i < 0) return -1;
  hipEventRecord(m->evPool[i], m->stream);
  return i;
}
static void ev_end(mgcm_model *m, int k, int startIdx) {
  if (!m->timing || startIdx < 0) return;
  const int i = ev_next(m);
  if (i < 0) return;
  hipEventRecord(m->evPool[i], m->stream);
  m->evPairs.push_back({k, startIdx});
}
static void ev_collect(mgcm_model *m) {
  for (auto &pr : m->evPairs) {
    float ms = 0.f;
    if (hipEventElapsedTime(&ms, m->evPool[pr.second], m->evPool[pr.second + 1]) == hipSuccess) {
      m->kms[pr.first] += ms;
      m->kcnt[pr.first] += 1;
    }
  }
  m->evPairs.clear();
  m->evUsed = 0;
}
static void ev_free(mgcm_model *m) {
  for (auto e : m->evPool) hipEventDestroy(e);
  m->evPool.clear();
  m->evUsed = 0;
}

static void build_latlon_halo(mgcm_model *m) {
  const Dims &d = m->d;
  const int Nx = d.sNx * d.nSx, Ny = d.sNy * d.nSy;
  m->h_halo.clear();
  for (int t = 0; t < d.nTiles; t++) {
    const int bi = t % d.nSx, bj = t / d.nSx;
    for (int j = 1 - d.OLy; j <= d.sNy + d.OLy; j++)
      for (int i = 1 - d.OLx; i <= d.sNx + d.OLx; i++) {
        if (i >= 1 && i <= d.sNx && j >= 1 && j <= d.sNy) continue;
        int iG = ((bi * d.sNx + i - 1) % Nx + Nx) % Nx, jG = ((bj * d.sNy + j - 1) % Ny + Ny) % Ny;
        int st = (jG / d.sNy) * d.nSx + iG / d.sNx;
        m->h_halo.push_back(MG_I2(d, i, j, t));
        m->h_halo.push_back(MG_I2(d, iG % d.sNx + 1, jG % d.sNy + 1, st));
      }
  }
}

static int upload_halo(mgcm_model *m) {
  if (m->d_halo) { hipFree(m->d_halo); m->d_halo = nullptr; }
  if (m->d_srcOf) { hipFree(m->d_srcOf); m->d_srcOf = nullptr; }
  const long N2 = m->d.n2 * m->d.nTiles;
  std::vector<long> srcOf(N2, -1);
  for (size_t h = 0; h + 1 < m->h_halo.size(); h += 2) srcOf[m->h_halo[h]] = m->h_halo[h + 1];
  HIPCHK(hipMalloc(&m->d_srcOf, N2 * sizeof(long)));
  HIPCHK(hipMemcpy(m->d_srcOf, srcOf.data(), N2 * sizeof(long), hipMemcpyHostToDevice));
  std::vector<long> loc;
  const long lo = (long)m->d.t0 * m->d.n2, hi = (long)(m->d.t0 + m->d.nT) * m->d.n2;
  for (size_t h = 0; h + 1 < m->h_halo.size(); h += 2)
    if (m->h_halo[h] >= lo && m->h_halo[h] < hi) { loc.push_back(m->h_halo[h]); loc.push_back(m->h_halo[h + 1]); }
  m->nHalo = (int)(loc.size() / 2);
  if (m->d_haloAll) { hipFree(m->d_haloAll); m->d_haloAll = nullptr; }
  m->nHaloAll = 0;
  if (m->d.nT < m->d.nTiles && !m->h_halo.empty()) {
    HIPCHK(hipMalloc(&m->d_haloAll, m->h_halo.size() * sizeof(long)));
    HIPCHK(hipMemcpy(m->d_haloAll, m->h_halo.data(), m->h_halo.size() * sizeof(long), hipMemcpyHostToDevice));
    m->nHaloAll = (int)(m->h_halo.size() / 2);
  }
  if (m->uvMap) {
    const long N2 = m->d.n2 * m->d.nTiles;
    for (int all = 0; all < 2; all++)
      for (int w = 0; w < 2; w++) {
        long *&dm = all ? m->d_uvAll[w] : m->d_uv[w];
        if (dm) { hipFree(dm); dm = nullptr; }
        const long l0 = all ? 0 : lo, l1 = all ? N2 : hi;
        const std::vector<long> &code = m->h_uv[w];
        auto srcOfCode = [](long c) { return (c > 0 ? c : -c) - 1; };
        auto early = [&](long c) { return c != 0 && code[(size_t)srcOfCode(c)] != 0; };
        std::vector<long> e, pre;
        int nu = 0, nv = 0, pu = 0, pv = 0;
        for (int c = 0; c < 2; c++)
          for (long q = l0; q < l1; q++) {
            const long cd = code[(size_t)c * N2 + q];
            if (cd == 0) continue;
            if (early(cd)) {
              if (early(code[(size_t)srcOfCode(cd)]))
                return set_err("EXCH2 vector map: the halo of tile %ld copies a halo point that itself copies one "
                               "(tiles narrower than the halo are not supported on the device)", q / m->d.n2 + 1);
              if (m->d.nT < m->d.nTiles)
                return set_err("EXCH2 vector map: tiles as narrow as the halo are not supported in tile-sharded runs");
              pre.push_back(q); pre.push_back(cd);
              (c ? pv : pu)++;
              continue;
            }
            e.push_back(q); e.push_back(cd);
            (c ? nv : nu)++;
          }
        (all ? m->nUvUAll : m->nUvU)[w] = nu;
        (all ? m->nUvVAll : m->nUvV)[w] = nv;
        m->uvPre[all][w] = mgcm_model::UvPre{};
        const size_t nMain = e.size();
        e.insert(e.end(), pre.begin(), pre.end());
        if (!e.empty()) {
          HIPCHK(hipMalloc(&dm, e.size() * sizeof(long)));
          HIPCHK(hipMemcpy(dm, e.data(), e.size() * sizeof(long), hipMemcpyHostToDevice));
          m->uvPre[all][w].map = dm + nMain;
          m->uvPre[all][w].nU = pu;
          m->uvPre[all][w].nV = pv;
        }
// ... 430 lines not shown
  const long arenaN[2] = {(long)F2_COUNT * d.N2all, (long)F3_COUNT * d.N3all};
  for (int q = 0; q < 2; q++) {
    if (hipMalloc(&arena[q], arenaN[q] * sizeof(double)) != hipSuccess ||
        hipMemset(arena[q], 0, arenaN[q] * sizeof(double)) != hipSuccess) {
      set_err("mgcm_create: hipMalloc of the %s arena (%ld doubles)", q ? "3-D" : "2-D", arenaN[q]);
      mgcm_destroy(m);
      return nullptr;
    }
    m->allocs.push_back(arena[q]);
  }
  m->f.a2 = arena[0];
  m->f.a3 = arena[1];
  int n2i = 0, n3i = 0;
  for (auto &fd : FIELDS) {
    const long n = field_count(m, fd.kind);
    double *ptr = nullptr;
    if (fd.kind == F2D) ptr = arena[0] + (long)(n2i++) * d.N2all;
    else if (fd.kind == F3D) ptr = arena[1] + (long)(n3i++) * d.N3all;
    else if (hipMalloc(&ptr, n * sizeof(double)) != hipSuccess || hipMemset(ptr, 0, n * sizeof(double)) != hipSuccess) {
      set_err("mgcm_create: hipMalloc %s (%ld doubles)", fd.name, n);
      mgcm_destroy(m);
      return nullptr;
    } else {
      m->allocs.push_back(ptr);
    }
    field_ptr(m, &fd) = ptr;
  }
  if (hipMalloc(&m->d_ctr, 2 * sizeof(int)) != hipSuccess || hipMemset(m->d_ctr, 0, 2 * sizeof(int)) != hipSuccess ||
      hipMalloc(&m->d_rec, m->maxRec * sizeof(SolveRecord)) != hipSuccess) {
    set_err("mgcm_create: counters");
    mgcm_destroy(m);
    return nullptr;
  }
  build_latlon_halo(m);
  if (hipDeviceSynchronize() != hipSuccess) {
    set_err("mgcm_create: zero fill");
    mgcm_destroy(m);
    return nullptr;
  }
  return m;
}

void mgcm_destroy(mgcm_model *m) {
  if (!m) return;
  hipSetDevice(m->device);
  if (m->stream) hipStreamSynchronize(m->stream);
  ev_collect(m);
  ev_free(m);
  drop_graphs(m);
  for (void *p : m->allocs) hipFree(p);
  if (m->monBuf) hipFree(m->monBuf);
  if (m->d_halo) hipFree(m->d_halo);
  if (m->d_srcOf) hipFree(m->d_srcOf);
  if (m->d_haloAll) hipFree(m->d_haloAll);
  for (int q = 0; q < 2; q++) {
    if (m->d_uv[q]) hipFree(m->d_uv[q]);
    if (m->d_uvAll[q]) hipFree(m->d_uvAll[q]);
  }
  if (m->d_tileInfo) hipFree(m->d_tileInfo);
  if (m->d_nbr) hipFree(m->d_nbr);
  if (m->d_gofs) hipFree(m->d_gofs);
  if (m->d_nbx) hipFree(m->d_nbx);
  if (m->d_blkx) hipFree(m->d_blkx);
  if (m->d_dropG) hipFree(m->d_dropG);
  if (m->h_guard) hipHostFree(m->h_guard);
  if (m->d_ctr) hipFree(m->d_ctr);
  for (auto &q : m->exchBuf)
    if (q) hipFree(q);
  if (m->d_rec) hipFree(m->d_rec);
  if (m->mwgShared) (void)hipIpcCloseMemHandle(m->mwgShared);
  for (void *q : m->mwgAllocs) hipFree(q);
  for (int q = 0; q < 2; q++) {
    if (m->stHost[q]) hipHostFree(m->stHost[q]);
    if (m->stEv[q]) hipEventDestroy(m->stEv[q]);
    if (m->stCopied[q]) hipEventDestroy(m->stCopied[q]);
    if (m->stDev[q]) hipFree(m->stDev[q]);
  }
  if (m->stCopy) hipStreamDestroy(m->stCopy);
  if (m->ownStream) hipStreamDestroy(m->ownStream);
  if (m->stream2) hipStreamDestroy(m->stream2);
  if (m->evFork) hipEventDestroy(m->evFork);
  if (m->evHand) hipEventDestroy(m->evHand);
  if (m->evJoin) hipEventDestroy(m->evJoin);
  for (auto &ev : m->ovlEv)
    if (ev) hipEventDestroy(ev);
  delete m;
}

int mgcm_set_param(mgcm_model *m, const char *name, double value) {
  drop_graphs(m);
  m->ptrTabDirty = true;
  if (!strcmp(name, "myIter")) {
    int it = (int)value;
    HIPCHK(hipSetDevice(m->device));
    HIPCHK(hipMemcpyAsync(m->d_ctr, &it, sizeof(int), hipMemcpyHostToDevice, m->stream));
    HIPCHK(hipStreamSynchronize(m->stream));
    return 0;
  }
  for (auto &pd : PARAMS)
    if (!strcmp(pd.name, name)) {
      char *ptr = reinterpret_cast<char *>(&m->p) + pd.off;
      if (pd.isint) *reinterpret_cast<int *>(ptr) = (int)value;
      else *reinterpret_cast<double *>(ptr) = value;
      return 0;
    }
  static const char *inert[] = {"implicitFreeSurface"};
// ... 265 lines not shown
  for (int t = 0; t < m->d.nTiles; t++) { info[t] = tileFace[t]; info[m->d.nTiles + t] = tileEdge[t]; }
  HIPCHK(hipSetDevice(m->device));
  if (m->d_tileInfo) (void)hipFree(m->d_tileInfo);
  HIPCHK(hipMalloc(&m->d_tileInfo, info.size() * sizeof(int)));
  HIPCHK(hipMemcpy(m->d_tileInfo, info.data(), info.size() * sizeof(int), hipMemcpyHostToDevice));
  m->f.tileFace = m->d_tileInfo;
  m->f.tileEdge = m->d_tileInfo + m->d.nTiles;
  m->p.cubeCorners = 1;
  m->uvMap = true;
  m->ready = false;
  drop_graphs(m);
  return 0;
}

static hipError_t uv_pre(mgcm_model *m, const Dims &d, double *u, double *v, int nz, int w, bool all = false) {
  const mgcm_model::UvPre &p = m->uvPre[all ? 1 : 0][w];
  return launch_exchange_uv(d, u, v, p.map, p.nU, p.nV, nz, m->stream);
}

static int exchange_uv(mgcm_model *m, double *u, double *v, int nz, bool withSigns) {
  if (!m->uvMap) {
    HIPCHK(launch_exchange(m->d, u, m->d_halo, m->nHalo, nz, m->stream));
    HIPCHK(launch_exchange(m->d, v, m->d_halo, m->nHalo, nz, m->stream));
    return 0;
  }
  const int w = withSigns ? 1 : 0;
  HIPCHK(uv_pre(m, m->d, u, v, nz, w));
  HIPCHK(launch_exchange_uv(m->d, u, v, m->d_uv[w], m->nUvU[w], m->nUvV[w], nz, m->stream));
  return 0;
}

static Dims all_tiles(const Dims &d) { Dims a = d; a.t0 = 0; a.nT = d.nTiles; return a; }

static hipError_t calc_r_star(mgcm_model *m, bool fuseEtaH = false, int fromX = 0, bool stagEx = false) {
  const Dims da = all_tiles(m->d);
  hipError_t e;
  if (stagEx) {
    XFields xw{};
    xw.p[0] = m->f.wVel; xw.nz[0] = m->d.Nr; xw.n = 1;
    e = uv_pre(m, m->d, m->f.uVel, m->f.vVel, m->d.Nr, 1);
    if (e != hipSuccess) return e;
    e = launch_rstar_exmix(da, m->p, m->f, m->d_srcOf, fuseEtaH, fromX, m->f.uVel, m->f.vVel, m->d.Nr, m->d_uv[1],
                           m->nUvU[1], m->nUvV[1], xw, m->d_halo, m->nHalo, m->stream);
  } else
    e = launch_calc_r_star(da, m->p, m->f, m->d_srcOf, m->stream, fuseEtaH, fromX);
  if (e != hipSuccess || !m->uvMap) return e;
  double *us[3] = {m->f.rStarFacW, m->f.rStarDhWDt, m->f.rStarExpW}, *vs[3] = {m->f.rStarFacS, m->f.rStarDhSDt,
                                                                                 m->f.rStarExpS};
  for (int q = 0; q < 3; q++)
    if ((e = uv_pre(m, da, us[q], vs[q], 1, 0, true)) != hipSuccess) return e;
  return launch_exchange_uv_pairs(da, us, vs, 3, m->d_uvAll[0], m->nUvUAll[0], m->nUvVAll[0], m->stream);
}
static hipError_t update_r_star_cg2d(mgcm_model *m, bool sfp = false, bool opEarly = false, bool pcHere = false,
                                     const int *physNext = nullptr, bool keepFac = false) {
  return launch_update_r_star_cg2d(all_tiles(m->d), m->p, m->f, m->d_srcOf, m->stream, sfp, opEarly, pcHere, physNext,
                                   keepFac);
}

int mgcm_init(mgcm_model *m) {
  auto ext = [&](const char *n, double dflt) { auto it = m->extra.find(n); return it == m->extra.end() ? dflt : it->second; };
  HIPCHK(hipSetDevice(m->device));
  const char *retired = nullptr;
  if (const int bit = mg_fuse_retired(&retired))
    return set_err("mgcm_init: MGCM_STEP_FUSE bit %d (%s) was measured slower than the default and removed in round 10 "
                   "(common.h); unset it", bit, retired);
  if (upload_halo(m)) return -1;
  m->noCompact = false;
  m->nPts = m->d.nTiles * m->d.sNx * m->d.sNy;
  BxyChoice bxy;
  if (choose_bxy(m, bxy)) return -1;
  if (m->p.cg2dRefOrder) {
    if (m->p.useSRCGSolver) return set_err("mgcm_init: cg2dRefOrder with useSRCGSolver not implemented");
    m->solver = m->nPts > cg2d_ref_max_points() ? Cg2dSolver::MwgRef : Cg2dSolver::BlockRef;
  } else
    m->solver = (bxy.var < 0 || ext("cg2dForceMwg", 0.0) != 0.0) ? Cg2dSolver::Mwg : Cg2dSolver::Bxy;
  if (m->p.useSRCGSolver && m->solver == Cg2dSolver::BlockRef)
    return set_err("mgcm_init: useSRCGSolver (CG2D_SR) is implemented in the blocked single-workgroup and the "
                   "multi-workgroup CG2D only");
  clear_bxy(m);
  if (m->solver == Cg2dSolver::Bxy ? build_bxy(m, bxy) : m->solver == Cg2dSolver::BlockRef ? build_block(m) : build_mwg(m))
    return -1;
  if (!m->h_dropG.empty()) {
    const long n2a = m->d.n2 * m->d.nTiles;
    std::vector<double> eta((size_t)n2a);
    for (const char *nm : {"etaN", "etaH"}) {
      if (!strcmp(nm, "etaH") && m->p.nIter0 == 0) continue;
      HIPCHK(hipMemcpy(eta.data(), !strcmp(nm, "etaN") ? m->f.etaN : m->f.etaH, n2a * sizeof(double), hipMemcpyDeviceToHost));
      if (land_eta_check(m, nm, eta.data(), n2a)) return -1;
    }
  }
  if ((m->p.viscA4D != 0.0 || m->p.viscA4Z != 0.0) && (m->d.OLx < 3 || m->d.OLy < 3))
    return set_err("mgcm_init: biharmonic viscosity needs OLx, OLy >= 3 (del2u of the halo ring)");
  const bool rstar = m->p.nonlinFreeSurf > 0;
  if (rstar) {
    if (m->p.nonlinFreeSurf != 4 || m->p.select_rStar != 2)
      return set_err("mgcm_init: the non-linear free surface is implemented for nonlinFreeSurf=4, select_rStar=2 only");
    if (!m->p.exactConserv) return set_err("mgcm_init: nonlinFreeSurf needs exactConserv");
  }
  if (m->p.selectP_inEOS_Zc > 2) return set_err("mgcm_init: selectP_inEOS_Zc = 3 needs the non-hydrostatic pressure");
  if (m->p.selectP_inEOS_Zc == 2 && !m->p.storePhiHyd4Phys)
    return set_err("mgcm_init: selectP_inEOS_Zc = 2 needs storePhiHyd4Phys (set_parms.F:297)");
  if (m->p.implicitViscosity && (ext("momImplVertAdv", 0.0) != 0.0 || ext("selectImplicitDrag", 0.0) != 0.0))
    return set_err("mgcm_init: momImplVertAdv / selectImplicitDrag not implemented on the device");
  if (m->p.vectorInvariantMomentum) {
    if (m->d.OLx < 2 || m->d.OLy < 2) return set_err("mgcm_init: vector-invariant momentum needs OLx, OLy >= 2");
    if (m->p.viscA4D != 0.0 || m->p.viscA4Z != 0.0)
      return set_err("mgcm_init: biharmonic viscosity with vectorInvariantMomentum not implemented on the device");
    if (m->p.useNHMTerms || m->p.select3dCoriScheme > 0 || m->p.useCDscheme)
      return set_err("mgcm_init: NH metric / 3-D Coriolis / CD scheme with vectorInvariantMomentum not implemented");
// ... 419 lines not shown

const char *mgcm_param_name(int i) {
  const int n = (int)(sizeof(PARAMS) / sizeof(PARAMS[0]));
  return (i >= 0 && i < n) ? PARAMS[i].name : nullptr;
}

long mgcm_field_count(mgcm_model *m, const char *name) {
  double *dev = nullptr;
  long n = 0;
  if (!lookup_field(m, name, &dev, &n)) { set_err("mgcm_field_count: unknown field %s", name); return -1; }
  return n;
}

static XFields blocking_fields(const mgcm_model *m, int tracers, bool totPhi) {
  XFields x{};
  double *fl[] = {m->f.uVel, m->f.vVel, m->f.wVel, m->f.theta, m->f.salt, m->f.uVelD, m->f.vVelD, m->f.totPhiHyd};
  const bool use[] = {!m->uvMap, !m->uvMap, true, m->p.tempStepping != 0, m->p.saltStepping != 0, m->p.useCDscheme != 0,
                      m->p.useCDscheme != 0, m->p.storePhiHyd4Phys != 0 && totPhi};
  for (int q = 0; q < 8; q++) {
    const bool tr = q == 3 || q == 4;
    if (use[q] && (tracers == 1 || (tracers == 2) == tr)) { x.p[x.n] = fl[q]; x.nz[x.n] = m->d.Nr; x.n++; }
  }
  return x;
}

enum StepMode {
  STEP_PLAIN = 0,
  STEP_HOIST = 1,
  STEP_LAST = 2
};
#define MG_PIPE_MIN_STEPS 4

struct StepPlan {
  bool mom, rstar;
  bool stagger;
  bool tracers;
  bool canFork, forkable, fork;
  bool forkLate, thermoLate, forkEarly, thermoInline;
  bool trEx;
  bool ringLate, ringAside;
  bool dtFused;
  bool gmPhi;
  bool physGm;
  bool ringPhys, momRing;
  bool opEarly;
  bool sfpFused;
  bool etaX;
  bool fuseEtaH, etaHAlone;
  bool endFused;
  bool stagEx;
  bool pipeOk, phiPipeOk, pipe, hoist, valid, phiPipe, phiNext, empNext;
  bool resFlow, resFlowFold;
  bool spec;
};
static StepPlan plan_step(const mgcm_model *m, StepMode mode) {
  const Params &p = m->p;
  const Dims &d = m->d;
  const bool whole = d.nT == d.nTiles;
  StepPlan pl{};
  pl.mom = p.momStepping != 0;
  pl.rstar = p.nonlinFreeSurf > 0;
  pl.stagger = p.staggerTimeStep != 0 && pl.mom;
  pl.tracers = p.tempStepping || p.saltStepping || !m->ptr.empty();
  pl.canFork = !pl.stagger && pl.mom && pl.tracers;
  pl.forkable = pl.canFork && m->overlap;
  pl.fork = pl.forkable && !m->timing;
  pl.forkLate = !pl.rstar;
  pl.thermoLate = pl.fork && pl.forkLate;
  pl.trEx = pl.thermoLate && mg_fuse_on(MG_FUSE_TREX);
  const bool ringSep = mom_ring_separable(d, p);
  pl.ringLate = pl.forkLate && ringSep && mg_fuse_on(MG_FUSE_RING);
  pl.ringAside = pl.thermoLate && pl.ringLate;
  pl.resFlow = takes_res_flow(m);
  pl.dtFused = pl.forkable && pl.rstar && dyn_thermo_fusable(d, p, tracer_args(m, false), tracer_args(m, true));
  const bool gmFold = pl.dtFused && dyn_thermo_takes_gm(p);
  pl.spec = gmFold && dyn_thermo_spec_ok(p);
  pl.forkEarly = pl.fork && !pl.thermoLate && !pl.dtFused;
  pl.thermoInline = !pl.stagger && !pl.fork && !pl.dtFused;
  pl.gmPhi = (pl.stagger || pl.thermoLate) && !pl.dtFused && !m->timing && gm_phi_fusable(d, p);
  pl.physGm = !gmFold && !pl.gmPhi;
  pl.opEarly = gmFold && p.nonlinFreeSurf > 2 && whole && mg_fuse_on(MG_FUSE_OPE);
  pl.sfpFused = mg_fuse_on(MG_FUSE_SFP) && pl.rstar && whole;
  pl.etaX = p.exactConserv && mg_fuse_on(MG_FUSE_ETAX) && whole;
  pl.fuseEtaH = p.exactConserv && pl.rstar;
  pl.etaHAlone = p.exactConserv && !pl.fuseEtaH;
  pl.endFused = pl.mom && pl.rstar && !pl.stagger && !m->uvMap && whole && mg_hfuse(MG_FUSE_END, d.nx, d.ny, d.nT, d.Nr);
  pl.stagEx = pl.mom && pl.rstar && !pl.endFused && pl.stagger && pl.tracers && m->uvMap && whole &&
              mg_hfuse(MG_FUSE_ENDS, d.nx, d.ny, d.nT, d.Nr);
  const bool totPhiHalo = p.eosType == 1 && p.selectP_inEOS_Zc == 2 && !p.storePhiHyd4Phys;
  pl.resFlowFold = pl.resFlow && pl.dtFused;
  pl.pipeOk = gmFold && pl.sfpFused && pl.endFused && mg_fuse_on(MG_FUSE_PIPE) && p.select_rStar > 0 &&
              p.useRealFreshWaterFlux && p.exactConserv && m->d_srcOf && !totPhiHalo && !pl.resFlow;
  pl.phiPipeOk = pl.pipeOk && phi_pipe_ok(d, p);
  pl.pipe = mode != STEP_PLAIN;
  pl.hoist = mode == STEP_HOIST;
  pl.valid = !pl.pipe || pl.pipeOk;
  pl.phiPipe = pl.pipe && pl.phiPipeOk;
  pl.phiNext = pl.hoist && pl.phiPipe;
  pl.empNext = pl.hoist && p.periodicExternalForcing;
  pl.ringPhys = !pl.pipe && !pl.ringAside && ringSep && mg_fuse_on(MG_FUSE_RINGP) && phys_ring_ok(d, p, m->f);
  pl.momRing = !pl.ringAside && !pl.ringPhys;
  return pl;
}
static int step_layout_bits(const StepPlan &pl) {
  return (pl.dtFused ? 1 : 0) | (pl.forkable && !pl.dtFused ? 4 : 0) | (pl.forkable && pl.forkLate ? 8 : 0) |
         (pl.pipe ? 16 : 0) | (pl.phiPipe ? 32 : 0) | (pl.spec ? 64 : 0);
}

static int fork_thermo(mgcm_model *m, bool ring, bool trEx) {
  HIPCHK(hipEventRecord(m->evFork, m->stream));
  HIPCHK(hipStreamWaitEvent(m->stream2, m->evFork, 0));
  if (ring) HIPCHK(launch_mom_ring(m->d, m->p, m->f, m->d_ctr, m->stream2));
  if (tracers_on(m, m->stream2)) return -1;
  if (trEx) {
    const XFields xt = blocking_fields(m, 2);
    if (xt.n > 0) HIPCHK(launch_exchange_multi(m->d, xt, m->d_halo, m->nHalo, nullptr, m->stream2));
  }
  HIPCHK(hipEventRecord(m->evJoin, m->stream2));
  return 0;
}

static int one_step(mgcm_model *m, StepMode mode = STEP_PLAIN) {
  const StepPlan pl = plan_step(m, mode);
  if (!pl.valid) return set_err("one_step: the pipelined step does not apply to this model");
  const int fromX = pl.etaX ? 1 : 0;
  m->mwg.exclusive = pl.thermoLate ? 1 : 0;
  m->stepLayout = step_layout_bits(pl);
  m->gmResFlow = 0;
  if (!pl.pipe) TIMED(K_PHYS, launch_oceanic_phys(m->d, m->p, m->f, m->d_ctr, m->stream, pl.physGm, pl.ringPhys));
  if (pl.forkEarly && fork_thermo(m, false, false)) return -1;
  if (pl.thermoInline && tracers_on(m, m->stream)) return -1;
  if (pl.mom) {
    if (pl.dtFused) {
      TIMED(K_MOM, launch_dyn_thermo(m->d, m->p, m->f, tracer_args(m, false), tracer_args(m, true), m->d_ctr, m->stream,
                                     pl.opEarly ? m->d_srcOf : nullptr, !pl.pipe, !pl.phiPipe, pl.spec));
      std::swap(m->f.theta, m->f.thetaNext);
      std::swap(m->f.salt, m->f.saltNext);
      if (pl.resFlowFold && res_flow_on(m, m->stream)) return -1;
      if (ptracers_on(m, m->stream)) return -1;
    } else if (pl.gmPhi) {
      TIMED(K_PHI, launch_gm_phi(m->d, m->p, m->f, m->stream));
      TIMED(K_MOM, launch_mom_step(m->d, m->p, m->f, m->d_ctr, m->stream, pl.momRing));
    } else if (dynamics_on(m, pl.momRing)) return -1;
    if (pl.forkEarly) HIPCHK(hipStreamWaitEvent(m->stream, m->evJoin, 0));
    if (pl.rstar)
      TIMED(K_RSTAR, update_r_star_cg2d(m, pl.sfpFused, pl.opEarly, false, pl.hoist ? m->d_ctr : nullptr, pl.phiNext));
    if (!pl.sfpFused) TIMED(K_RHS, launch_sfp_rhs(m->d, m->p, m->f, m->stream));
    if (pl.thermoLate && fork_thermo(m, pl.ringAside, pl.trEx)) return -1;
    TIMED(K_CG2D, launch_cg2d(m, m->p.cg2dMaxIters, m->p.cg2dUseMinResSol - 1));
    if (!pl.etaX) TIMED(K_ETA, launch_exch_eta(m->d, m->p, m->f, m->d_srcOf, false, 0, m->stream));
    if (pl.thermoLate) HIPCHK(hipStreamWaitEvent(m->stream, m->evJoin, 0));
    TIMED(K_CONT, launch_corr_cont(m->d, m->p, m->f, 0, m->stream, pl.etaX ? m->d_srcOf : nullptr, pl.hoist));
    if (pl.etaHAlone) TIMED(K_ETA, launch_exch_eta(m->d, m->p, m->f, m->d_srcOf, true, 0, m->stream, fromX));
    if (pl.endFused && pl.phiNext)
      TIMED(K_RSTAR, launch_rstar_exch_phi(m->d, m->p, m->f, m->d_srcOf, blocking_fields(m, 1, false), m->d_halo, m->nHalo,
                                           m->d_ctr, m->stream, fromX, pl.empNext ? 1 : 0));
    else if (pl.endFused)
      TIMED(K_RSTAR, launch_rstar_exch(m->d, m->p, m->f, m->d_srcOf, pl.fuseEtaH, blocking_fields(m), m->d_halo, m->nHalo,
                                       m->d_ctr, m->stream, fromX, pl.empNext ? 1 : 0));
    else if (pl.rstar)
      TIMED(K_RSTAR, calc_r_star(m, pl.fuseEtaH, fromX, pl.stagEx));
  } else {
    if (mgcm_integr_continuity(m)) return -1;
  }
  if (pl.stagger && pl.tracers) {
    if (!pl.stagEx && mgcm_stagger_exchanges(m)) return -1;
    if (tracers_on(m, m->stream)) return -1;
  }
  if (pl.endFused) return 0;
  const XFields xEnd = blocking_fields(m, pl.trEx ? 0 : 1);
  if (m->uvMap) {
    HIPCHK(uv_pre(m, m->d, m->f.uVel, m->f.vVel, m->d.Nr, 1));
    TIMED(K_EXCH, launch_exchange_mixed(m->d, m->f.uVel, m->f.vVel, m->d.Nr, m->d_uv[1], m->nUvU[1], m->nUvV[1], xEnd,
                                        m->d_halo, m->nHalo, m->d_ctr, m->stream));
  } else
    TIMED(K_EXCH, launch_exchange_multi(m->d, xEnd, m->d_halo, m->nHalo, m->d_ctr, m->stream));
  return 0;
}

static void drop_graphs(mgcm_model *m) {
  for (auto &row : m->graphs)
    for (auto &col : row)
      for (auto &g : col)
        if (g.exec) { (void)hipGraphExecDestroy(g.exec); g = mgcm_model::StepGraph{}; }
}

static int buffer_parity(const mgcm_model *m) {
  return (m->f.theta == m->thetaA ? 0 : 1) + (m->f.salt == m->saltA ? 0 : 2) + (m->ptrFlip ? 4 : 0);
}

static const struct { int n; StepMode mode[2]; } STEP_SEQS[SEQ_N] = {
    {2, {STEP_PLAIN, STEP_PLAIN}},
    {2, {STEP_HOIST, STEP_HOIST}},
    {2, {STEP_HOIST, STEP_LAST}},
    {1, {STEP_PLAIN, STEP_PLAIN}},
    {1, {STEP_LAST, STEP_LAST}},
};
static int step_graph(mgcm_model *m, StepSeq seq, mgcm_model::StepGraph **out = nullptr) {
  mgcm_model::StepGraph &sg = m->graphs[m->overlap ? 1 : 0][buffer_parity(m)][seq];
  if (!sg.exec) {
    double **tr[4] = {&m->f.theta, &m->f.thetaNext, &m->f.salt, &m->f.saltNext};
    double *pre[4];
    for (int k = 0; k < 4; k++) pre[k] = *tr[k];
    const int preFlip = m->ptrFlip;
    hipGraph_t g = nullptr;
    HIPCHK(hipStreamBeginCapture(m->stream, hipStreamCaptureModeThreadLocal));
    int rc = 0;
    for (int k = 0; k < STEP_SEQS[seq].n && !rc; k++) rc = one_step(m, STEP_SEQS[seq].mode[k]);
// ... 752 lines not shown
```

mitgcm_amd/csrc/phys.h:

```cpp
#pragma once
#include "common.h"

namespace mgcm {

__device__ __forceinline__ double jmd95_rho(const Params &p, double locPres, double t, double s) {
  const double t2 = t * t, t3 = t2 * t, t4 = t3 * t;
  double s3o2;
  if (s > 0.0) s3o2 = s * sqrt(s);
  else { s = 0.0; s3o2 = 0.0; }
  const double rfresh = 999.842594 + 6.793952e-02 * t + -9.095290e-03 * t2 + 1.001685e-04 * t3 +
                        -1.120083e-06 * t4 + 6.536332e-09 * t4 * t;
  const double rsalt = s * (8.24493e-01 + -4.0899e-03 * t + 7.6438e-05 * t2 + -8.2467e-07 * t3 + 5.3875e-09 * t4) +
                       s3o2 * (-5.72466e-03 + 1.0227e-04 * t + -1.6546e-06 * t2) + 4.8314e-04 * s * s;
  const double rhoP0 = rfresh + rsalt;
  const double pb = locPres * 1.0e-05, p2 = pb * pb;
  const double bMfresh = 1.965933e+04 + 1.444304e+02 * t + -1.706103e+00 * t2 + 9.648704e-03 * t3 +
                         -4.190253e-05 * t4;
  const double bMsalt = s * (5.284855e+01 + -3.101089e-01 * t + 6.283263e-03 * t2 + -5.084188e-05 * t3) +
                        s3o2 * (3.886640e-01 + 9.085835e-03 * t + -4.619924e-04 * t2);
  const double bMpres = pb * (3.186519e+00 + 2.212276e-02 * t + -2.984642e-04 * t2 + 1.956415e-06 * t3) +
                        pb * s * (6.704388e-03 + -1.847318e-04 * t + 2.059331e-07 * t2) + pb * s3o2 * 1.480266e-04 +
                        p2 * (2.102898e-04 + -1.202016e-05 * t + 1.394680e-07 * t2) +
                        p2 * s * (-2.040237e-06 + 6.128773e-08 * t + 6.207323e-10 * t2);
  const double bulkMod = bMfresh + bMsalt + bMpres;
  return rhoP0 / (1.0 - locPres * 1.0e-05 / bulkMod) - p.rhoConst;
}
__device__ __forceinline__ double pressure_for_eos(const Params &p, const Fields &f, int kRef, long q3) {
  if (p.selectP_inEOS_Zc == 2) return p.rhoConst * (f.totPhiHyd[q3] + f.phiRefC[kRef - 1]) + 0.0;
  return f.pRef4EOS[kRef - 1] + 0.0;
}
__device__ __forceinline__ double find_rho(const Params &p, const Fields &f, int kRef, long q3, double t, double s) {
  if (p.eosType == 1) return jmd95_rho(p, pressure_for_eos(p, f, kRef, q3), t, s);
  const double refTemp = f.tRef[kRef - 1], refSalt = f.sRef[kRef - 1];
  const double dRho = p.rhoNil - p.rhoConst;
  return p.rhoNil * (p.sBeta * (s - refSalt) - p.tAlpha * (t - refTemp)) + dRho;
}

template <bool HOIST>
__device__ __forceinline__ double oceanic_phys_point_t(const Dims &d, const Params &p, const Fields &f, const int *iterPtr,
                                                       const long *__restrict__ srcOf, int i, int j, int k, int t) {
  const long q = MG_I2(d, i, j, t), q31 = MG_I3(d, i, j, 1, t);
  long r31 = q31;
  bool own = true;
  if constexpr (HOIST) {
    const long sq = srcOf[q];
    if (sq >= 0) { r31 = (sq / d.n2) * d.n3 + sq % d.n2; own = false; }
  }
  auto theta_at = [&](int kk) {
    const double v = f.theta[HOIST ? r31 + (long)(kk - 1) * d.n2 : MG_I3(d, i, j, kk, t)];
    return (kk == 1 && p.allowFreezing && v < -1.9) ? -1.9 : v;
  };
  if (k == 1 && p.periodicExternalForcing) {
    const long N2 = d.n2 * d.nTiles;
    const double cycleLength = p.externForcingCycle, recSpacing = p.externForcingPeriod;
    const double currentTime = (double)(*iterPtr + (HOIST ? 1 : 0)) * p.deltaTClock;
    const int nbRec = (int)llround(cycleLength / recSpacing);
    const double locTime = currentTime - recSpacing * 0.5 + cycleLength * (double)(2 - llround(currentTime / cycleLength));
    const double tmpTime = fmod(locTime, cycleLength);
    const int tRec1 = 1 + (int)(tmpTime / recSpacing);
    const int tRec2 = 1 + tRec1 % nbRec;
    const double aW = (tmpTime - recSpacing * (double)(tRec1 - 1)) / recSpacing;
    const double bW = 1.0 - aW;
    double *dst[6] = {f.SST, f.SSS, f.fu, f.fv, f.Qnet, HOIST ? f.EmPmRnext : f.EmPmR};
#pragma unroll
    for (int v = 0; v < 6; v++) {
      const double *r = f.forcRec + (long)v * p.nForcRec * N2;
      dst[v][q] = bW * r[(long)(tRec1 - 1) * N2 + q] + aW * r[(long)(tRec2 - 1) * N2 + q];
    }
  }
  if (k == 1) {
    const double th1 = theta_at(1), s1 = f.salt[HOIST ? r31 : q31];
    if (p.allowFreezing && own) f.theta[q31] = th1;
    const double mass2rUnit = 1.0 / p.rhoConst, recip_Cp = 1.0 / p.HeatCapacity_Cp;
    const double hFac1 = HOIST ? f.h0FacC[q31] * f.rStarFacC[q] : f.hFacC[q31];
    double sfT = -(f.lambdaThetaClimRelax[q] * (th1 - f.SST[q]) * f.drF[0] * hFac1);
    double sfS = -(f.lambdaSaltClimRelax[q] * (s1 - f.SSS[q]) * f.drF[0] * hFac1);
    sfT = sfT - f.Qnet[q] * recip_Cp * mass2rUnit;
    sfS = sfS - 0.0 * mass2rUnit;
    const double UNSET_RL = 123456.7;
    if (p.nonlinFreeSurf > 0 && p.useRealFreshWaterFlux) {
      const double pmepr = HOIST ? -f.EmPmR[q] : f.PmEpR[q];
      if (p.temp_EvPrRn != UNSET_RL) sfT = sfT + pmepr * (p.temp_EvPrRn - th1) * mass2rUnit;
      if (p.salt_EvPrRn != UNSET_RL) sfS = sfS + pmepr * (p.salt_EvPrRn - s1) * mass2rUnit;
    } else if (p.convertFW2Salt == -1.0) {
      if (p.temp_EvPrRn != UNSET_RL) sfT = sfT + f.EmPmR[q] * (th1 - p.temp_EvPrRn) * mass2rUnit;
      if (p.salt_EvPrRn != UNSET_RL) sfS = sfS + f.EmPmR[q] * (s1 - p.salt_EvPrRn) * mass2rUnit;
    } else {
      if (p.temp_EvPrRn != UNSET_RL) sfT = sfT + f.EmPmR[q] * (f.tRef[0] - p.temp_EvPrRn) * mass2rUnit;
      if (p.salt_EvPrRn != UNSET_RL) sfS = sfS + f.EmPmR[q] * (p.convertFW2Salt - p.salt_EvPrRn) * mass2rUnit;
    }
    f.surfaceForcingT[q] = sfT;
    f.surfaceForcingS[q] = sfS;
  }
  const long q3 = MG_I3(d, i, j, k, t);
  const long r3 = HOIST ? r31 + (long)(k - 1) * d.n2 : q3;
  const double rho = find_rho(p, f, k, r3, theta_at(k), f.salt[r3]);
  f.rhoInSitu[q3] = rho;
  const bool calcConvect = p.ivdc_kappa != 0.0;
  double conv = 0.0, sigmaR = 0.0;
  if (k >= 2 && (calcConvect || p.useGMRedi)) {
    const long q3u = MG_I3(d, i, j, k - 1, t);
    const double rhoKm1 = find_rho(p, f, k, r3, theta_at(k - 1), f.salt[r3 - d.n2]);
    sigmaR = f.maskC[q3] * f.maskC[q3u] * f.recip_drC[k - 1] * p.rkSign * (rho - rhoKm1);
    if (calcConvect) conv = (-sigmaR * p.gravitySign > 0.0) ? 1.0 : 0.0;
  }
  f.IVDConvCount[q3] = conv;
  if (p.useGMRedi) f.sigmaR[q3] = sigmaR;
  return rho;
}
__device__ __forceinline__ double oceanic_phys_point(const Dims &d, const Params &p, const Fields &f, const int *iterPtr,
                                                     int i, int j, int k, int t) {
  return oceanic_phys_point_t<false>(d, p, f, iterPtr, nullptr, i, j, k, t);
}
__device__ __forceinline__ void phys_hoist_body(const Dims &d, const Params &p, const Fields &f, const int *iterPtr,
                                                const long *__restrict__ srcOf, int lb) {
  MG_PLANE_LB(1 - d.OLx, d.nx, 1 - d.OLy, d.ny, z, lb)
  const int t = d.t0 + z / d.Nr, k = z % d.Nr + 1;
  oceanic_phys_point_t<true>(d, p, f, iterPtr, srcOf, i, j, k, t);
}
inline int phys_hoist_blocks(const Dims &d) { return (int)mg_plane_blocks(d.nx, d.ny, d.nT * d.Nr); }


}
```

mitgcm_amd/csrc/rstar.h:

```cpp
#pragma once
#include "common.h"

namespace mgcm {

__device__ __forceinline__ double eta_exch(const Dims &d, const Fields &f, const long *srcOf, long q, int fromX) {
  const long sq = srcOf[q];
  if (sq >= 0) return f.cg2d_b[sq];
  const long l = q % d.n2;
  const int i = (int)(l % d.nx) - d.OLx + 1, j = (int)(l / d.nx) - d.OLy + 1;
  if (i >= 1 && i <= d.sNx && j >= 1 && j <= d.sNy) return f.cg2d_b[q];
  return fromX ? f.recip_Bo[q] * f.cg2d_x[q] : f.etaN[q];
}

template <bool NARROW>
__device__ __forceinline__ void mg_ij_of(const Dims &d, long q, int &i, int &j) {
  if constexpr (NARROW) {
    const int l = (int)q % (int)d.n2;
    i = l % d.nx - d.OLx + 1;
    j = l / d.nx - d.OLy + 1;
  } else {
    const long l = q % d.n2;
    i = (int)(l % d.nx) - d.OLx + 1;
    j = (int)(l / d.nx) - d.OLy + 1;
  }
}

template <bool FUSE, bool WS = true, bool SHORT = false>
__device__ __forceinline__ void calc_r_star_fac(const Dims &d, const Params &p, const Fields &f,
                                                const long *__restrict__ srcOf, long q, int fromX, double oc, double ow,
                                                double os, double &fc, double &fw, double &fs) {
  auto inner = [&](int ii, int jj) { return ii >= 1 && ii <= d.sNx && jj >= 1 && jj <= d.sNy; };
  int i, j;
  long r;
  if constexpr (SHORT) {
    mg_ij_of<true>(d, q, i, j);
    r = q;
    if (!inner(i, j)) {
      const long sq = srcOf[q];
      if (sq >= 0) { r = sq; mg_ij_of<true>(d, r, i, j); }
    }
  } else {
    const long sq = srcOf[q];
    r = sq >= 0 ? sq : q;
    mg_ij_of<false>(d, r, i, j);
  }
  auto eta = [&](long qq, int ii, int jj) {
    if constexpr (SHORT) {
      if (inner(ii, jj)) return f.cg2d_b[qq];
      const long sqq = srcOf[qq];
      if (sqq >= 0) return f.cg2d_b[sqq];
      return fromX ? f.recip_Bo[qq] * f.cg2d_x[qq] : f.etaN[qq];
    } else {
      return FUSE ? eta_exch(d, f, srcOf, qq, fromX) : f.etaH[qq];
    }
  };
  fc = oc;
  fw = ow;
  fs = os;
  if (i >= 0 && i <= d.sNx + 1 && j >= 0 && j <= d.sNy + 1)
    fc = (f.maskInC[r] != 0.0) ? (eta(r, i, j) + f.Ro_surf[r] - f.R_low[r]) * f.recip_Rcol[r] : 1.0;
  if constexpr (WS) {
    const long rv = (!SHORT && p.cubeCorners) ? q : r;
    int iv = i, jv = j;
    if constexpr (!SHORT) mg_ij_of<false>(d, rv, iv, jv);
    if (iv >= 1 && iv <= d.sNx + 1 && jv >= 1 && jv <= d.sNy) {
      if (f.maskInW[rv] != 0.0) {
        const double tmp = f.rSurfW[rv] - f.rLowW[rv];
        fw = (0.5 * (eta(rv - 1, iv - 1, jv) * f.rA[rv - 1] + eta(rv, iv, jv) * f.rA[rv]) * f.recip_rAw[rv] + tmp) / tmp;
      } else {
        fw = 1.0;
      }
    }
    if (iv >= 1 && iv <= d.sNx && jv >= 1 && jv <= d.sNy + 1) {
      if (f.maskInS[rv] != 0.0) {
        const double tmp = f.rSurfS[rv] - f.rLowS[rv];
        fs = (0.5 * (eta(rv - d.nx, iv, jv - 1) * f.rA[rv - d.nx] + eta(rv, iv, jv) * f.rA[rv]) * f.recip_rAs[rv] + tmp) / tmp;
      } else {
        fs = 1.0;
      }
    }
  }
}

template <bool FUSE>
__device__ __forceinline__ void calc_r_star_body(const Dims &d, const Params &p, const Fields &f,
                                                 const long *__restrict__ srcOf, int lb, int fromX, int empNext = 0) {
  const long q = (long)lb * blockDim.x + threadIdx.x;
  if (q >= d.n2 * d.nTiles) return;
  const int t = (int)(q / d.n2);
  if (t < d.t0 || t >= d.t0 + d.nT) return;
  if constexpr (FUSE) {
    if (p.nonlinFreeSurf > 0 && p.useRealFreshWaterFlux) f.PmEpR[q] = -f.EmPmR[q];
    if (empNext) f.EmPmR[q] = f.EmPmRnext[q];
    const double x = eta_exch(d, f, srcOf, q, fromX);
    f.etaHnm1[q] = f.etaH[q];
    f.etaN[q] = x;
    f.etaH[q] = x;
  }
  const double oc = f.rStarFacC[q], ow = f.rStarFacW[q], os = f.rStarFacS[q];
  double fc, fw, fs;
  calc_r_star_fac<FUSE>(d, p, f, srcOf, q, fromX, oc, ow, os, fc, fw, fs);
  f.rStarFacC[q] = fc;
  f.rStarFacW[q] = fw;
  f.rStarFacS[q] = fs;
  f.rStarDhCDt[q] = (fc - oc) / p.deltaTFreeSurf;
  f.rStarDhWDt[q] = (fw - ow) / p.deltaTFreeSurf;
  f.rStarDhSDt[q] = (fs - os) / p.deltaTFreeSurf;
  f.rStarExpC[q] = fc / oc;
  f.rStarExpW[q] = fw / ow;
  f.rStarExpS[q] = fs / os;
}

template <bool WS>
__device__ __forceinline__ void r_star_next_point(const Dims &d, const Params &p, const Fields &f,
                                                  const long *__restrict__ srcOf, long q, int fromX, double &facC,
                                                  double &dhC, double &dhW, double &dhS) {
  const double oc = f.rStarFacCPrev[q], ow = WS ? f.rStarFacWPrev[q] : 0.0, os = WS ? f.rStarFacSPrev[q] : 0.0;
  double fc, fw, fs;
  calc_r_star_fac<true, WS, true>(d, p, f, srcOf, q, fromX, oc, ow, os, fc, fw, fs);
  facC = fc;
  dhC = (fc - oc) / p.deltaTFreeSurf;
  if constexpr (WS) {
    dhW = (fw - ow) / p.deltaTFreeSurf;
    dhS = (fs - os) / p.deltaTFreeSurf;
  }
}

__device__ __forceinline__ long mg_at_source3(const Dims &d, const long *__restrict__ srcOf, int i, int j, int k, int t) {
  if (i >= 1 && i <= d.sNx && j >= 1 && j <= d.sNy) return MG_I3(d, i, j, k, t);
  const long sq = srcOf[MG_I2(d, i, j, t)];
  if (sq < 0) return MG_I3(d, i, j, k, t);
  return (sq / d.n2) * d.n3 + (long)(k - 1) * d.n2 + sq % d.n2;
}

}
```

mitgcm_amd/model.py:

```python
import ctypes

import numpy as np

from ._lib import check, lib, MgcmError

GRID_2D = ("dxF", "dyF", "dxG", "dyG", "dxC", "dyC", "dxV", "dyU", "rA", "rAw", "rAs",
           "recip_dxF", "recip_dyF", "recip_dxC", "recip_dyC", "recip_dxV", "recip_dyU",
           "recip_rA", "recip_rAw", "recip_rAs", "fCori", "Bo_surf", "recip_Bo",
           "aW2d", "aS2d", "aC2d", "pW", "pS", "pC", "maskInC", "tanPhiAtU", "tanPhiAtV",
           "fCoriCos", "recip_Rcol", "rSurfW", "rSurfS", "rLowW", "rLowS", "Ro_surf", "R_low", "maskInW", "maskInS",
           "fCoriG", "recip_rAz", "recip_dxG", "recip_dyG")
GRID_3D = ("hFacC", "hFacW", "hFacS", "recip_hFacC", "recip_hFacW", "recip_hFacS", "maskC", "maskW", "maskS",
           "h0FacC", "h0FacW", "h0FacS")
GRID_1D = ("drF", "drC", "recip_drF", "recip_drC", "rF", "rC")
STATE_1D = ("tRef", "sRef", "pRef4EOS", "phiRefC")
STATE_3D = ("uVel", "vVel", "wVel", "theta", "salt", "gU", "gV", "guNm1", "gvNm1", "gtNm1", "gsNm1", "rhoInSitu",
            "IVDConvCount", "sigmaR", "Kwx", "Kwy", "Kwz", "Kux", "Kvy", "uVelD", "vVelD", "uNM1", "vNM1",
            "totPhiHyd", "alphaRho", "del2u", "del2v", "Kuz", "Kvz", "GM_PsiX", "GM_PsiY")
WORK_3D = ("phiHydC", "dWtC", "dWtU", "dWtV")
STATE_2D = ("etaN", "etaH", "fu", "fv", "SST", "lambdaThetaClimRelax", "surfaceForcingT", "surfaceForcingS",
            "Qnet", "EmPmR", "SSS", "lambdaSaltClimRelax", "etaNm1", "rStarFacC", "rStarFacW", "rStarFacS",
            "rStarExpC", "rStarExpW", "rStarExpS", "rStarDhCDt", "rStarDhWDt", "rStarDhSDt", "PmEpR", "dEtaHdt")
FORCING_ORDER = ("SST", "SSS", "taux", "tauy", "Qnet", "EmPmR")

# ... 175 lines not shown

    def trcstat(self):
        return trcstat(self)

    def solve_stats(self, back=0):
        f, la, rm = ctypes.c_double(), ctypes.c_double(), ctypes.c_double()
        it = ctypes.c_int()
        check(lib().mgcm_solve_stats(self.h, back, ctypes.byref(f), ctypes.byref(la), ctypes.byref(it),
                                     ctypes.byref(rm)), "mgcm_solve_stats")
        return {"cg2d_init_res": f.value, "cg2d_last_res": la.value, "cg2d_iters": it.value,
                "cg2d_rhs_max": rm.value}

    def solve_minres(self, back=0):
        r, n = ctypes.c_double(), ctypes.c_int()
        check(lib().mgcm_solve_minres(self.h, back, ctypes.byref(r), ctypes.byref(n)), "mgcm_solve_minres")
        return r.value, n.value

    def solve_history(self, n):
        it = np.zeros(n, dtype=np.int32)
        fr = np.zeros(n)
        lr = np.zeros(n)
        check(lib().mgcm_solve_history(self.h, n, it.ctypes.data_as(ctypes.POINTER(ctypes.c_int)), _dp(fr), _dp(lr)),
              "mgcm_solve_history")
        return it, fr, lr

    def cg2d(self, b, x, maxIters, nIterMin=-1):
        b = np.ascontiguousarray(b, dtype=np.float64).copy()
        x = np.ascontiguousarray(x, dtype=np.float64).copy()
        f, mn, la = ctypes.c_double(), ctypes.c_double(), ctypes.c_double()
        it, itm = ctypes.c_int(maxIters), ctypes.c_int(nIterMin)
        check(lib().mgcm_cg2d(self.h, _dp(b), _dp(x), ctypes.byref(f), ctypes.byref(mn), ctypes.byref(la),
                              ctypes.byref(it), ctypes.byref(itm)), "mgcm_cg2d")
        return x, f.value, mn.value, la.value, it.value, itm.value

    def cg2d_sum_plan(self):
        cap = 1 << 24
        plan = np.zeros(cap, dtype=np.int32)
        nt, ppt, ng = ctypes.c_int(), ctypes.c_int(), ctypes.c_int()
        check(lib().mgcm_cg2d_sum_plan(self.h, plan.ctypes.data_as(ctypes.POINTER(ctypes.c_int)), cap,
                                       ctypes.byref(nt), ctypes.byref(ppt), ctypes.byref(ng)), "mgcm_cg2d_sum_plan")
        return plan[:nt.value * ppt.value * ng.value].copy(), nt.value, ppt.value, ng.value

    def cg2d_kernel(self):
        k = lib().mgcm_get_param(self.h, b"cg2dKernel")
        names = {3.0: "bxy", 4.0: "mwg", 5.0: "block_ref", 6.0: "mwg_ref"}
        if k not in names:
            raise RuntimeError("cg2dKernel = %r names no CG2D solver" % (k,))
        return names[k]

    def step_layout(self):
        b = int(lib().mgcm_get_param(self.h, b"stepLayout"))
        return {"dyn_thermo_fused": bool(b & 1), "thermo_second_stream": bool(b & 4),
                "late_join": bool(b & 8), "pipelined": bool(b & 16), "phi_pipelined": bool(b & 32),
                "specialised": bool(b & 64)}

    def ptracers_route(self):
        r = int(lib().mgcm_get_param(self.h, b"ptrRoute"))
        return {"route": ("none", "functional", "batched")[r], "launches": int(lib().mgcm_get_param(self.h, b"ptrLaunches"))}

    def gm_res_flow(self):
        return lib().mgcm_get_param(self.h, b"gmResFlow") != 0.0

    def cg2d_fma(self):
        return lib().mgcm_get_param(self.h, b"cg2dFMA") != 0.0

    def cg2d_parts(self):
        return int(lib().mgcm_get_param(self.h, b"cg2dParts"))

    def kernel_timing(self, enable):
        lib().mgcm_kernel_timing(self.h, 1 if enable else 0)

    def kernel_ms(self, name):
        n = ctypes.c_int()
        ms = lib().mgcm_kernel_ms(self.h, name.encode(), ctypes.byref(n))
        return ms, n.value


MON_FIELDS = ("eta", "uvel", "vvel", "wvel", "theta", "salt")
MON_STATS = ("max", "min", "mean", "sd", "del2")


def monitor(model):
    out = np.zeros(len(MON_FIELDS) * len(MON_STATS))
    check(lib().mgcm_monitor(model.h, _dp(out)), "mgcm_monitor")
    return {"dynstat_%s_%s" % (f, s): float(out[i * 5 + j]) for i, f in enumerate(MON_FIELDS)
            for j, s in enumerate(MON_STATS)}


def mon_stats(g, arr, hfac, mask, area, dr):
    OLx, OLy, sNx, sNy = g.OLx, g.OLy, g.sNx, g.sNy
    nz = arr.shape[1]
    theMin = theMax = 0.0
    noPnts = True
    tNb, tDel2, tVol, tMean = [], [], [], []
    for t in range(arr.shape[0]):
        nb = d2 = vol = mean = 0.0
        for k in range(nz):
            for j in range(1, sNy + 1):
                J = j + OLy - 1
                for i in range(1, sNx + 1):
                    I = i + OLx - 1
                    v = arr[t, k, J, I]
                    msk = mask[t, J, I] * hfac[t, k, J, I]
                    if msk > 0.0:
                        if noPnts:
                            theMin = theMax = v
                            noPnts = False
# ... 72 lines not shown
```

Baseline: 4081 model-days/s.

## Precompute halo source table and specialise solve-side kernels on pinned run options

Adds a precomputed per-point HaloRec table (2D source index, 3D base, i/j, flags) that replaces on-the-fly srcOf lookups and integer div/mod in the r* and hydrostatic-pressure halo paths. It also extends the compile-time option pinning (OptsRun) to more parameters and templates the r*/cg2d, GM tensor and physics kernels on it, enabled through a new default fuse bit. The aim is to cut index arithmetic, dependent loads and runtime branches in fused kernels. In exchange it adds a table to build and a specialised path whose preconditions must match the run options.

```diff
diff --git a/include/mitgcm_amd.h b/include/mitgcm_amd.h
--- a/include/mitgcm_amd.h
+++ b/include/mitgcm_amd.h
@@ -39,6 +39,8 @@
 double *mgcm_device_ptr(mgcm_model *m, const char *name);
 
 int mgcm_set_halo_map(mgcm_model *m, const long *src_of_point, long count);
+
+int mgcm_halo_table(int sNx, int sNy, int OLx, int OLy, int Nr, int nTiles, const long *src_of_point, int *out);
 
 int mgcm_set_uv_map(mgcm_model *m, const long *u1, const long *v1, const long *u0, const long *v0,
                     const int *tileFace, const int *tileEdge, long count);
diff --git a/mitgcm_amd/_lib.py b/mitgcm_amd/_lib.py
--- a/mitgcm_amd/_lib.py
+++ b/mitgcm_amd/_lib.py
@@ -40,6 +40,7 @@
         "mgcm_get": (ci, [vp, cs, PD, cl]),
         "mgcm_device_ptr": (vp, [vp, cs]),
         "mgcm_set_halo_map": (ci, [vp, PL, cl]),
+        "mgcm_halo_table": (ci, [ci] * 6 + [PL, PI]),
         "mgcm_set_uv_map": (ci, [vp, PL, PL, PL, PL, PI, PI, cl]),
         "mgcm_init": (ci, [vp]),
         "mgcm_dynamics": (ci, [vp]),
@@ -94,6 +95,8 @@
         "cg2d_amd_": (None, [PD, PD, PD, PD, PD, PI, PI, PI]),
     }
     for name, (res, args) in sig.items():
+        if name == "mgcm_halo_table" and os.environ.get("MGCM_LIB") and not hasattr(L, name):
+            continue
         fn = getattr(L, name)
         fn.restype = res
         fn.argtypes = args
@@ -102,7 +105,7 @@
 
 
 EXPORTS = ["mgcm_create", "mgcm_destroy", "mgcm_last_error", "mgcm_set_param", "mgcm_get_param", "mgcm_put", "mgcm_put_async", "mgcm_put_batch_async",
-           "mgcm_get", "mgcm_device_ptr", "mgcm_set_halo_map", "mgcm_set_uv_map", "mgcm_init", "mgcm_dynamics", "mgcm_thermodynamics",
+           "mgcm_get", "mgcm_device_ptr", "mgcm_set_halo_map", "mgcm_halo_table", "mgcm_set_uv_map", "mgcm_init", "mgcm_dynamics", "mgcm_thermodynamics",
            "mgcm_solve_for_pressure", "mgcm_momentum_correction_step", "mgcm_integr_continuity",
            "mgcm_blocking_exchanges", "mgcm_prepare", "mgcm_forward_step", "mgcm_sync", "mgcm_cg2d", "mgcm_cg2d_sum_plan", "mgcm_solve_stats", "mgcm_solve_minres", "mgcm_stream_triad", "mgcm_solve_history", "mgcm_monitor",
            "mgcm_kernel_ms", "mgcm_kernel_timing", "mgcm_set_tile_range", "mgcm_set_stream",
diff --git a/mitgcm_amd/csrc/common.h b/mitgcm_amd/csrc/common.h
--- a/mitgcm_amd/csrc/common.h
+++ b/mitgcm_amd/csrc/common.h
@@ -201,11 +201,12 @@
 inline unsigned mg_colf_blocks(long ncols, int nc) { return (unsigned)((ncols + nc - 1) / nc); }
 enum { MG_FUSE_SFP = 1, MG_FUSE_PHI = 4, MG_FUSE_END = 8, MG_FUSE_TREX = 64, MG_FUSE_DT = 128, MG_FUSE_ETAX = 256,
        MG_FUSE_OPE = 1024, MG_FUSE_RING = 2048, MG_FUSE_RINGP = 4096, MG_FUSE_ENDS = 8192, MG_FUSE_PIPE = 16384,
-       MG_FUSE_PHIP = 32768, MG_FUSE_SPEC = 65536 };
+       MG_FUSE_PHIP = 32768, MG_FUSE_SPEC = 65536, MG_FUSE_SPEC2 = 131072 };
 inline int mg_fuse_mask() {
   return getenv("MGCM_STEP_FUSE") ? atoi(getenv("MGCM_STEP_FUSE"))
                                   : MG_FUSE_SFP | MG_FUSE_PHI | MG_FUSE_END | MG_FUSE_DT | MG_FUSE_ETAX | MG_FUSE_OPE |
-                                        MG_FUSE_RING | MG_FUSE_RINGP | MG_FUSE_ENDS | MG_FUSE_PIPE | MG_FUSE_PHIP | MG_FUSE_SPEC;
+                                        MG_FUSE_RING | MG_FUSE_RINGP | MG_FUSE_ENDS | MG_FUSE_PIPE | MG_FUSE_PHIP | MG_FUSE_SPEC |
+                                        MG_FUSE_SPEC2;
 }
 inline bool mg_fuse_on(int bit) { return (mg_fuse_mask() & bit) != 0; }
 inline int mg_fuse_retired(const char **what) {
@@ -249,7 +250,20 @@
   X(gmAdvForm, p.GM_AdvForm != 0, false)                                                            \
   X(gmExtraDiag, p.GM_ExtraDiag != 0, false)                                                        \
   X(implicitDiffusion, p.implicitDiffusion != 0, true)                                              \
-  X(tracForcingOutAB, p.tracForcingOutAB != 0, false)
+  X(tracForcingOutAB, p.tracForcingOutAB != 0, false)                                               \
+          \
+  X(exactConserv, p.exactConserv != 0, true)                                                        \
+  X(realFreshWaterFlux, p.useRealFreshWaterFlux != 0, true)                                         \
+  X(quasiHydrostatic, p.quasiHydrostatic != 0, true)                                                \
+  X(storePhiHyd4Phys, p.storePhiHyd4Phys != 0, true)                                                \
+  X(eosPresFromPhi, p.selectP_inEOS_Zc == 2, true)                                      \
+  X(eosJmd95, p.eosType == 1, true)                                                                 \
+  X(allowFreezing, p.allowFreezing != 0, true)                                                      \
+  X(periodicForcing, p.periodicExternalForcing != 0, true)                                          \
+  X(gmRedi, p.useGMRedi != 0, true)                                                                 \
+  X(ivdc, p.ivdc_kappa != 0.0, true)                                                                \
+  X(opEveryStep, p.nonlinFreeSurf > 2, true)                           \
+  X(cubeCorners, p.cubeCorners != 0, false)
 struct OptsRun {
   static constexpr bool pinned = false;
 #define MG_OPT_RUN(name, expr, pin) \
@@ -272,14 +286,15 @@
   return true;
 }
 
+template <class O = OptsRun>
 __device__ __forceinline__ void sfp_rhs_column(const Dims &d, const Params &p, const Fields &f, long q, bool inner,
                                                const double *sE, const double *sW, const double *sN, const double *sS,
                                                int NC_, int cc) {
-  if (p.useCDscheme) f.etaNm1[q] = f.etaN[q];
+  if (O::cdScheme(p)) f.etaNm1[q] = f.etaN[q];
   f.cg2d_x[q] = f.Bo_surf[q] * f.etaN[q];
   double b = 0.0;
   if (inner) {
-    if (p.useRealFreshWaterFlux) {
+    if (O::realFreshWaterFlux(p)) {
       const double tmpFac = p.freeSurfFac * (1.0 / p.rhoConst) * p.implicDiv2DFlow;
       b = tmpFac * f.rA[q] * f.EmPmR[q] / p.deltaTMom * f.maskInC[q];
     }
@@ -288,7 +303,7 @@
       b = b + sE[s2] - sW[s2];
       b = b + sN[s2] - sS[s2];
     }
-    b = b - p.freeSurfFac * f.rA[q] / p.deltaTMom / p.deltaTFreeSurf * (p.exactConserv ? f.etaH[q] : f.etaN[q]);
+    b = b - p.freeSurfFac * f.rA[q] / p.deltaTMom / p.deltaTFreeSurf * (O::exactConserv(p) ? f.etaH[q] : f.etaN[q]);
   }
   f.cg2d_b[q] = b;
 }
@@ -315,6 +330,20 @@
 __device__ __forceinline__ double ptr_surf_relax(const TracerArgs &a, double trSurf, double drF1, double hFacC1) {
   return (((a.relaxRate * (a.relaxVal - trSurf)) * drF1) * hFacC1);
 }
+
+__host__ __device__ __forceinline__ void mg_ij_of(const Dims &d, long q, int &i, int &j) {
+  const long l = q % d.n2;
+  i = (int)(l % d.nx) - d.OLx + 1;
+  j = (int)(l / d.nx) - d.OLy + 1;
+}
+
+enum { MG_HR_INTERIOR = 1, MG_HR_MAPPED = 2 };
+struct __attribute__((aligned(16))) HaloRec {
+  int at2;
+  int base3;
+  short i, j;
+  int flags;
+};
 
 #define MG_XMAX 8
 struct XFields {
diff --git a/mitgcm_amd/csrc/gm_tensor.h b/mitgcm_amd/csrc/gm_tensor.h
--- a/mitgcm_amd/csrc/gm_tensor.h
+++ b/mitgcm_amd/csrc/gm_tensor.h
@@ -22,6 +22,7 @@
   else if (SlopeSqr > maxSlopeSqr && SlopeSqr < p.GM_slopeSqCutoff) taper = maxSlopeSqr / SlopeSqr;
 }
 
+template <class O = OptsRun>
 __device__ __forceinline__ void gm_tensor_body(const Dims &d, const Params &p, const Fields &f, int lb) {
   MG_PLANE_LB(2 - d.OLx, d.nx - 2, 2 - d.OLy, d.ny - 2, z, lb)
   const int t = d.t0 + z / d.Nr, k = z % d.Nr + 1;
@@ -61,7 +62,7 @@
     const double dSr = op25 * (sR(i - 1, j, k) + sR(i, j, k) + (sR(i - 1, j, kp1) + sR(i, j, kp1)) * maskp1) * mW * gs;
     gm_slope_gkw91(p, dSx, dSy, dSr, SlopeX, SlopeY, SlopeSqr, taper);
     f.Kux[q3] = fmax((p.GM_isopycK * 1.0 * op5 * (1.0 + 1.0)) * taper, p.GM_Kmin_horiz);
-    if (p.GM_ExtraDiag)
+    if (O::gmExtraDiag(p))
       f.Kuz[q3] = -gs * (p.GM_isopycK * 1.0 * op5 * (1.0 + 1.0) - p.GM_skewflx * p.GM_background_K * 1.0 * op5 * (1.0 + 1.0)) *
                   SlopeX * taper;
   }
@@ -72,11 +73,11 @@
     const double dSr = op25 * (sR(i, j - 1, k) + sR(i, j, k) + (sR(i, j - 1, kp1) + sR(i, j, kp1)) * maskp1) * mS * gs;
     gm_slope_gkw91(p, dSx, dSy, dSr, SlopeX, SlopeY, SlopeSqr, taper);
     f.Kvy[q3] = fmax((p.GM_isopycK * 1.0 * op5 * (1.0 + 1.0)) * taper, p.GM_Kmin_horiz);
-    if (p.GM_ExtraDiag)
+    if (O::gmExtraDiag(p))
       f.Kvz[q3] = -gs * (p.GM_isopycK * 1.0 * op5 * (1.0 + 1.0) - p.GM_skewflx * p.GM_background_K * 1.0 * op5 * (1.0 + 1.0)) *
                   SlopeY * taper;
   }
-  if (p.GM_AdvForm) {
+  if (O::gmAdvForm(p)) {
     double psx = 0.0, psy = 0.0;
     if (k >= 2) {
       const double halfRL = 0.5, halfSign = halfRL * gs, half_K = p.GM_background_K * (1.0 + 1.0) * op25;
diff --git a/mitgcm_amd/csrc/kernels_dyn.hip b/mitgcm_amd/csrc/kernels_dyn.hip
--- a/mitgcm_amd/csrc/kernels_dyn.hip
+++ b/mitgcm_amd/csrc/kernels_dyn.hip
@@ -28,7 +28,7 @@
 
 template <bool HO = false>
 __device__ __forceinline__ void del2uv_body(const Dims &d, const Params &p, const Fields &f, int lb,
-                                            const long *__restrict__ srcOf = nullptr) {
+                                            const HaloRec *__restrict__ rec = nullptr) {
   MG_PLANE_LB(1 - d.OLx, d.nx, 1 - d.OLy, d.ny, z, lb)
   const int t = d.t0 + z / d.Nr, k = z % d.Nr + 1;
   const long q3 = MG_I3(d, i, j, k, t);
@@ -38,7 +38,9 @@
     return;
   }
   const double drF = f.drF[k - 1];
-  auto uv3 = [&](int ii, int jj) { return HO ? mg_at_source3(d, srcOf, ii, jj, k, t) : MG_I3(d, ii, jj, k, t); };
+  auto uv3 = [&](int ii, int jj) {
+    return HO ? mg_at_source3(d, rec, ii, jj, t) + (long)(k - 1) * d.n2 : MG_I3(d, ii, jj, k, t);
+  };
   const long qv[5] = {uv3(i, j), uv3(i - 1, j), uv3(i + 1, j), uv3(i, j - 1), uv3(i, j + 1)};
   auto qvAt = [&](int ii, int jj) { return qv[jj == j ? (ii == i ? 0 : ii < i ? 1 : 2) : (jj < j ? 3 : 4)]; };
 #define U(ii, jj) f.uVel[HO ? qvAt(ii, jj) : MG_I3(d, ii, jj, k, t)]
@@ -86,7 +88,7 @@
 
 template <bool HO = false>
 __device__ __forceinline__ void phi_hyd_body(const Dims &d, const Params &p, const Fields &f, int nc, int lb,
-                                             const long *__restrict__ srcOf = nullptr, int fromX = 0) {
+                                             const HaloRec *__restrict__ rec = nullptr, int fromX = 0) {
   extern __shared__ __attribute__((aligned(16))) double lds[];
   MG_COLF_LB(-1, d.sNx + 3, -1, d.sNy + 3, nc, lb)
   const int Nr = d.Nr, NS = Nr * NC_;
@@ -97,12 +99,19 @@
   const double recip_rhoConst = 1.0 / p.rhoConst;
   const long q2 = MG_I2(d, i, j, t);
   double hoFacC = 0.0, hoDhC = 0.0, hoDhW = 0.0, hoDhS = 0.0;
-  const bool hoStash = HO && Nr >= 2 && KW_ >= 4;
   auto hoD0 = [&](long r) {
     double fc_ = 0.0, c_ = 0.0, w_ = 0.0, s_ = 0.0;
-    if constexpr (HO) r_star_next_point<false>(d, p, f, srcOf, r, fromX, fc_, c_, w_, s_);
+    if constexpr (HO) r_star_next_point<false>(d, p, f, rec, r, fromX, fc_, c_, w_, s_);
     return c_ * (f.Ro_surf[r] - f.R_low[r]) * f.rA[r];
   };
+  long hoC = 0, hoE = 0, hoN = 0;
+  if constexpr (HO) {
+    if (valid && qh) {
+      hoC = mg_at_source3(d, rec, i, j, t);
+      hoE = mg_at_source3(d, rec, i + 1, j, t);
+      hoN = mg_at_source3(d, rec, i, j + 1, t);
+    }
+  }
   bool hoHave = false;
   if (valid) MG_COLF_K(k) {
     const int me = (k - 1) * NC_ + cc;
@@ -120,9 +129,10 @@
     double a = f.rhoInSitu[q3];
     if (qh) {
       const double scalingFactor = p.rhoConst * p.gravitySign * (1.0 / p.gravity);
-      const long qc = HO ? mg_at_source3(d, srcOf, i, j, k, t) : q3;
-      const long qe = HO ? mg_at_source3(d, srcOf, i + 1, j, k, t) : MG_I3(d, i + 1, j, k, t);
-      const long qn = HO ? mg_at_source3(d, srcOf, i, j + 1, k, t) : MG_I3(d, i, j + 1, k, t);
+      const long lvl = (long)(k - 1) * d.n2;
+      const long qc = HO ? hoC + lvl : q3;
+      const long qe = HO ? hoE + lvl : MG_I3(d, i + 1, j, k, t);
+      const long qn = HO ? hoN + lvl : MG_I3(d, i, j + 1, k, t);
       const double u0 = f.uVel[qc], u1 = f.uVel[qe];
       const double v0 = f.vVel[qc], v1 = f.vVel[qn];
       double gW = 0.0;
@@ -136,7 +146,7 @@
     if (rstar) {
       if constexpr (HO) {
         if (!hoHave) {
-          r_star_next_point<true>(d, p, f, srcOf, q2, fromX, hoFacC, hoDhC, hoDhW, hoDhS);
+          r_star_next_point<true>(d, p, f, rec, q2, fromX, hoFacC, hoDhC, hoDhW, hoDhS);
           hoHave = true;
         }
         sC[me] = hoDhC * hoOp[0] * hoOp[1] * hoOp[2];
@@ -155,19 +165,16 @@
     }
   }
   if constexpr (HO) {
-    if (valid && rstar) {
-      if (!hoHave && kk == 0) r_star_next_point<true>(d, p, f, srcOf, q2, fromX, hoFacC, hoDhC, hoDhW, hoDhS);
-      if (hoStash && ring) {
-        if (kk == KW_ / 4) sPh[cc] = hoD0(q2 - 1);
-        if (kk == KW_ / 2) sPh[NC_ + cc] = hoD0(q2 - d.nx);
-      }
+    if (valid && rstar && ring && (kk == KW_ / 4 || kk == KW_ / 2)) {
+      const bool west = kk == KW_ / 4;
+      sPh[west ? cc : NC_ + cc] = hoD0(west ? q2 - 1 : q2 - d.nx);
     }
   }
   __syncthreads();
   if (valid && kk == 0) {
     double hoW = 0.0, hoS = 0.0;
     if constexpr (HO) {
-      if (rstar && hoStash && ring) { hoW = sPh[cc]; hoS = sPh[NC_ + cc]; }
+      if (rstar && ring) { hoW = sPh[cc]; hoS = sPh[NC_ + cc]; }
     }
     double phF = 0.0;
     for (int k2 = 1; k2 <= Nr; k2++) {
@@ -180,8 +187,7 @@
       auto d0 = [&](long r) {
         if constexpr (HO) {
           if (r == q2) return hoDhC * (f.Ro_surf[r] - f.R_low[r]) * f.rA[r];
-          if (hoStash) return r == q2 - 1 ? hoW : hoS;
-          return hoD0(r);
+          return r == q2 - 1 ? hoW : hoS;
         } else {
           return f.rStarDhCDt[r] * (f.Ro_surf[r] - f.R_low[r]) * f.rA[r];
         }
diff --git a/mitgcm_amd/csrc/kernels_rstar.hip b/mitgcm_amd/csrc/kernels_rstar.hip
--- a/mitgcm_amd/csrc/kernels_rstar.hip
+++ b/mitgcm_amd/csrc/kernels_rstar.hip
@@ -31,24 +31,27 @@
   exchange_mixed_body(d, u, v, nzUV, uvMap, nU, nV, x, map, nHalo, nullptr, r % nbH, (r / nbH) % nzMax, r / (nbH * nzMax));
 }
 
-template <bool SFP, int PH>
+template <bool SFP, int PH, class O = OptsRun>
 __global__ void __launch_bounds__(256) k_update_r_star_cg2d_a(Dims d, Params p, Fields f, int nc, int opIn,
                                                               const long *__restrict__ srcOf, int nbPc,
                                                               const int *iterPtr, int nbPh) {
   extern __shared__ __attribute__((aligned(16))) double lds[];
   int lb = mg_xcd_block();
   if constexpr (PH != 0) {
-    if (lb < nbPh) { phys_hoist_body(d, p, f, iterPtr, srcOf, lb); return; }
+    if (lb < nbPh) { phys_hoist_body<O>(d, p, f, iterPtr, srcOf, lb); return; }
     lb -= nbPh;
   }
-  if (lb < nbPc) { ucg2d_p_point(d, p, f, srcOf, lb); return; }
-  lb -= nbPc;
+  if constexpr (!O::pinned) {
+    if (lb < nbPc) { ucg2d_p_point(d, p, f, srcOf, lb); return; }
+    lb -= nbPc;
+  }
   MG_COLF_LB(1 - d.OLx, d.nx, 1 - d.OLy, d.ny, nc, lb)
   const int NS = d.Nr * NC_;
   double *sW = lds, *sS = lds + NS;
   double *fE = lds + 2 * NS, *fW = lds + 3 * NS, *fN = lds + 4 * NS, *fS = lds + 5 * NS;
   const long q = MG_I2(d, i, j, t);
-  const bool op = opIn && p.nonlinFreeSurf > 2 && i >= 1 && i <= d.sNx + 1 && j >= 1 && j <= d.sNy + 1;
+  const bool opAny = !O::pinned && opIn && O::opEveryStep(p);
+  const bool op = opAny && i >= 1 && i <= d.sNx + 1 && j >= 1 && j <= d.sNy + 1;
   const bool inner = i >= 1 && i <= d.sNx && j >= 1 && j <= d.sNy;
   if (valid) {
     const double fc = f.rStarFacC[q], fw = f.rStarFacW[q], fs = f.rStarFacS[q];
@@ -74,7 +77,7 @@
         sS[me] = faceArea * f.recip_dyC[q];
       }
       if (SFP) {
-        if (p.useCDscheme) {
+        if (O::cdScheme(p)) {
           f.uNM1[q3] = f.uVel[q3];
           f.vNM1[q3] = f.vVel[q3];
         }
@@ -91,7 +94,7 @@
   }
   __syncthreads();
   if (!valid || kk != 0) return;
-  if (opIn && p.nonlinFreeSurf > 2) {
+  if (opAny) {
     double aW = 0.0, aS = 0.0;
     if (op) {
       for (int k = 1; k <= d.Nr; k++) {
@@ -105,7 +108,7 @@
     f.aW2d[q] = aW;
     f.aS2d[q] = aS;
   }
-  if (SFP) sfp_rhs_column(d, p, f, q, inner, fE, fW, fN, fS, NC_, cc);
+  if (SFP) sfp_rhs_column<O>(d, p, f, q, inner, fE, fW, fN, fS, NC_, cc);
 }
 
 __global__ void __launch_bounds__(256) k_update_cg2d_p(Dims d, Params p, Fields f, const long *__restrict__ srcOf) {
@@ -149,7 +152,7 @@
 }
 
 hipError_t launch_update_r_star_cg2d(const Dims &d, const Params &p, const Fields &f, const long *srcOf, hipStream_t s,
-                                     bool sfp, bool opEarly, bool pcHere, const int *iterPtr, bool keepFac) {
+                                     bool sfp, bool opEarly, bool pcHere, const int *iterPtr, bool keepFac, bool spec) {
   const long n = d.n2 * d.nTiles;
   const unsigned nb = (unsigned)((n + 255) / 256);
   const long ncol = (long)d.nx * d.ny * d.nT;
@@ -160,12 +163,15 @@
   MG_ALLOW_LDS(kPlain);
   MG_ALLOW_LDS(kSfp);
   const int nbPc = (opEarly && pcHere && p.nonlinFreeSurf > 2) ? (int)nb : 0;
+  if (spec && !(sfp && opEarly && !pcHere && iterPtr && keepFac && opts_match(p))) return hipErrorInvalidValue;
   if (iterPtr) {
     if (!sfp) return hipErrorInvalidValue;
     MG_ALLOW_LDS(kSfpPhys);
     MG_ALLOW_LDS(kSfpPhysKeep);
     const int nbPh = phys_hoist_blocks(d);
-    hipLaunchKernelGGL(keepFac ? kSfpPhysKeep : kSfpPhys, dim3(mg_colf_blocks(ncol, nc) + (unsigned)(nbPc + nbPh)), dim3(256),
+    auto kPinned = k_update_r_star_cg2d_a<true, 2, OptsGO90>;
+    MG_ALLOW_LDS(kPinned);
+    hipLaunchKernelGGL(spec ? kPinned : keepFac ? kSfpPhysKeep : kSfpPhys, dim3(mg_colf_blocks(ncol, nc) + (unsigned)(nbPc + nbPh)), dim3(256),
                        mg_colf_lds(d.Nr, nc, nArr), s, d, p, f, nc, opEarly ? 0 : 1, srcOf, nbPc, iterPtr, nbPh);
   } else if (keepFac) {
     return hipErrorInvalidValue;
diff --git a/mitgcm_amd/csrc/kernels_solve.hip b/mitgcm_amd/csrc/kernels_solve.hip
--- a/mitgcm_amd/csrc/kernels_solve.hip
+++ b/mitgcm_amd/csrc/kernels_solve.hip
@@ -907,20 +907,21 @@
   f.etaH[q] = x;
 }
 
-template <bool GM>
-__global__ void __launch_bounds__(256) k_corr_cont(Dims d, Params p, Fields f, int atInit, int nc,
+template <bool GM, class O = OptsRun>
+__global__ void __launch_bounds__(256) k_corr_cont(Dims d, Params p, Fields f, int atInitIn, int nc,
                                                    const long *__restrict__ etaSrc, int nbGm) {
   extern __shared__ __attribute__((aligned(16))) double lds[];
+  const int atInit = O::pinned ? 0 : atInitIn;
   int lb = mg_xcd_block();
   if constexpr (GM) {
-    if (lb < nbGm) { gm_tensor_body(d, p, f, lb); return; }
+    if (lb < nbGm) { gm_tensor_body<O>(d, p, f, lb); return; }
     lb -= nbGm;
   }
   MG_COLF_LB(1, d.sNx, 1, d.sNy, nc, lb)
   const int NS = d.Nr * NC_;
   double *sDiv = lds, *sMask = lds + NS, *sU = lds + 2 * NS, *sV = lds + 3 * NS, *sH0 = lds + 4 * NS;
   const long q = MG_I2(d, i, j, t);
-  const bool rstar = p.nonlinFreeSurf > 0 && p.select_rStar != 0;
+  const bool rstar = O::pinned || (p.nonlinFreeSurf > 0 && p.select_rStar != 0);
   if (valid && atInit != 0) MG_COLF_K(k) {
     const int me = (k - 1) * NC_ + cc;
     const double drF = f.drF[k - 1];
@@ -936,7 +937,7 @@
   } else if (valid) {
     const double psFac = p.pfFacMom * p.implicSurfPress;
     auto eta = [&](long qq) {
-      if (!etaSrc) return f.etaN[qq];
+      if (!O::pinned && !etaSrc) return f.etaN[qq];
       const long sq = etaSrc[qq];
       return f.recip_Bo[qq] * f.cg2d_x[sq >= 0 ? sq : qq];
     };
@@ -978,11 +979,11 @@
   __syncthreads();
   if (valid && kk == 0) {
     double rStarDhDt = 0.0;
-    if (p.exactConserv) {
+    if (O::exactConserv(p)) {
       double hDiv = 0.0;
       for (int k2 = 1; k2 <= d.Nr; k2++) hDiv = hDiv + sMask[(k2 - 1) * NC_ + cc] * sDiv[(k2 - 1) * NC_ + cc];
       double dEtaHdt;
-      if (atInit == 1 && p.nIter0 != 0 && p.useRealFreshWaterFlux) {
+      if (atInit == 1 && p.nIter0 != 0 && O::realFreshWaterFlux(p)) {
         dEtaHdt = f.dEtaHdt[q];
         double pm = dEtaHdt + hDiv * f.recip_rA[q];
         f.PmEpR[q] = pm * p.rhoConst;
@@ -992,7 +993,7 @@
         if (f.PmEpR) f.PmEpR[q] = 0.0;
         f.cg2d_b[q] = f.etaN[q];
       } else {
-        const double facEmP = p.useRealFreshWaterFlux ? 1.0 / p.rhoConst : 0.0;
+        const double facEmP = O::realFreshWaterFlux(p) ? 1.0 / p.rhoConst : 0.0;
         dEtaHdt = -(hDiv * f.recip_rA[q]) - facEmP * f.EmPmR[q];
         f.cg2d_b[q] = f.etaH[q] + p.implicDiv2DFlow * dEtaHdt * p.deltaTFreeSurf;
       }
@@ -1277,7 +1278,8 @@
 }
 
 hipError_t launch_corr_cont(const Dims &d, const Params &p, const Fields &f, int atInit, hipStream_t s,
-                            const long *etaSrc, bool gmNext) {
+                            const long *etaSrc, bool gmNext, bool spec) {
+  if (spec && !(gmNext && atInit == 0 && etaSrc && opts_match(p))) return hipErrorInvalidValue;
   const long ncol = (long)d.sNx * d.sNy * d.nT;
   const int nArr = (p.nonlinFreeSurf > 0 && p.select_rStar != 0) ? 5 : 4;
   if (atInit == 0 && !(p.nonlinFreeSurf > 0 && p.select_rStar != 0) && d.Nr == 50) {
@@ -1288,8 +1290,10 @@
   const int nc = d.Nr >= 30 ? 32 : 16;
   if (gmNext) {
     const int nbGm = (int)mg_plane_blocks(d.nx - 2, d.ny - 2, d.nT * d.Nr);
-    MG_ALLOW_LDS(k_corr_cont<true>);
-    hipLaunchKernelGGL(k_corr_cont<true>, dim3(mg_colf_blocks(ncol, nc) + (unsigned)nbGm), dim3(256),
+    auto kGen = k_corr_cont<true>, kPinned = k_corr_cont<true, OptsGO90>;
+    MG_ALLOW_LDS(kGen);
+    MG_ALLOW_LDS(kPinned);
+    hipLaunchKernelGGL(spec ? kPinned : kGen, dim3(mg_colf_blocks(ncol, nc) + (unsigned)nbGm), dim3(256),
                        mg_colf_lds(d.Nr, nc, nArr), s, d, p, f, atInit, nc, etaSrc, nbGm);
     return hipGetLastError();
   }
diff --git a/mitgcm_amd/csrc/kernels_step.hip b/mitgcm_amd/csrc/kernels_step.hip
--- a/mitgcm_amd/csrc/kernels_step.hip
+++ b/mitgcm_amd/csrc/kernels_step.hip
@@ -270,23 +270,22 @@
   return launch_mom_tail(d, p, f, iterPtr, s);
 }
 
-__global__ void __launch_bounds__(256) k_rstar_exch_phi(Dims d, Params p, Fields f, const long *__restrict__ srcOf, int nbR,
+__global__ void __launch_bounds__(256) k_rstar_exch_phi(Dims d, Params p, Fields f, const HaloRec *__restrict__ rec, int nbR,
                                                         XFields x, const long *__restrict__ map, int nHalo, int *ctr,
                                                         int nbX, int nzMax, int nbXall, int fromX, int empNext, int nc,
                                                         int nbPhi) {
   int lb = mg_xcd_block();
-  if (lb < nbPhi) { phi_hyd_body<true>(d, p, f, nc, lb, srcOf, fromX); return; }
+  if (lb < nbPhi) { phi_hyd_body<true>(d, p, f, nc, lb, rec, fromX); return; }
   lb -= nbPhi;
-  if (lb < nbR) { calc_r_star_body<true>(d, p, f, srcOf, lb, fromX, empNext); return; }
+  if (lb < nbR) { calc_r_star_body<true, true>(d, p, f, nullptr, lb, fromX, empNext, rec); return; }
   lb -= nbR;
   if (lb < nbXall) { exchange_multi_body(d, x, map, nHalo, ctr, lb % nbX, (lb / nbX) % nzMax, lb / (nbX * nzMax)); return; }
-  del2uv_body<true>(d, p, f, lb - nbXall, srcOf);
+  del2uv_body<true>(d, p, f, lb - nbXall, rec);
 }
 
 bool phi_pipe_ok(const Dims &d, const Params &p) {
-  (void)d;
   return mg_fuse_on(MG_FUSE_PHIP) && p.nonlinFreeSurf > 0 && p.select_rStar > 0 && p.exactConserv && !p.cubeCorners &&
-         dyn_thermo_takes_gm(p) && !phi_flat_on(p);
+         dyn_thermo_takes_gm(p) && !phi_flat_on(p) && d.Nr >= 2;
 }
 
 hipError_t launch_phi_del2(const Dims &d, const Params &p, const Fields &f, hipStream_t s) {
@@ -294,9 +293,9 @@
   return hipGetLastError();
 }
 
-hipError_t launch_rstar_exch_phi(const Dims &d, const Params &p, const Fields &f, const long *srcOf, const XFields &x,
+hipError_t launch_rstar_exch_phi(const Dims &d, const Params &p, const Fields &f, const HaloRec *rec, const XFields &x,
                                  const long *map, int nHalo, int *ctr, hipStream_t s, int fromX, int empNext) {
-  if (!phi_pipe_ok(d, p) || !srcOf || d.nT != d.nTiles) return hipErrorInvalidValue;
+  if (!phi_pipe_ok(d, p) || !rec || d.nT != d.nTiles) return hipErrorInvalidValue;
   const long n = d.n2 * d.nTiles;
   const int nbR = (int)((n + 255) / 256);
   int nzMax = 1;
@@ -305,10 +304,11 @@
   const int nbXall = nbX * nzMax * (x.n > 0 ? x.n : 1);
   int nc, nArr, nbPhi;
   phi_frame(d, p, nc, nArr, nbPhi);
+  if (256 / nc < 4) return hipErrorInvalidValue;
   const int nbDel = del2_needed(p) ? (int)mg_plane_blocks(d.nx, d.ny, d.nT * d.Nr) : 0;
   MG_ALLOW_LDS(k_rstar_exch_phi);
   hipLaunchKernelGGL(k_rstar_exch_phi, dim3((unsigned)(nbPhi + nbR + nbXall + nbDel)), dim3(256), mg_colf_lds(d.Nr, nc, nArr),
-                     s, d, p, f, srcOf, nbR, x, map, nHalo, ctr, nbX, nzMax, nbXall, fromX, empNext, nc, nbPhi);
+                     s, d, p, f, rec, nbR, x, map, nHalo, ctr, nbX, nzMax, nbXall, fromX, empNext, nc, nbPhi);
   return hipGetLastError();
 }
 
diff --git a/mitgcm_amd/csrc/launch.h b/mitgcm_amd/csrc/launch.h
--- a/mitgcm_amd/csrc/launch.h
+++ b/mitgcm_amd/csrc/launch.h
@@ -22,7 +22,7 @@
 hipError_t launch_exch_eta(const Dims &, const Params &, const Fields &, const long *, bool, int, hipStream_t,
                            int fromX = 0);
 hipError_t launch_corr_cont(const Dims &, const Params &, const Fields &, int, hipStream_t, const long *etaSrc = nullptr,
-                            bool gmNext = false);
+                            bool gmNext = false, bool spec = false);
 hipError_t launch_halo_pack(const Dims &, const XFields &, const long *, long, double *, int, hipStream_t);
 
 hipError_t launch_cgd(const Dims &, const Params &, const Fields &, int, double, double *, hipStream_t);
@@ -37,7 +37,7 @@
                              int, int *, hipStream_t, int fromX = 0, int empNext = 0);
 hipError_t launch_update_r_star_cg2d(const Dims &, const Params &, const Fields &, const long *, hipStream_t, bool sfp = false,
                                      bool opEarly = false, bool pcHere = false, const int *iterPtr = nullptr,
-                                     bool keepFac = false);
+                                     bool keepFac = false, bool spec = false);
 
 bool phys_ring_ok(const Dims &, const Params &, const Fields &);
 hipError_t launch_oceanic_phys(const Dims &, const Params &, const Fields &, const int *, hipStream_t, bool gm = true,
@@ -53,7 +53,7 @@
 bool dyn_thermo_spec_ok(const Params &);
 bool phi_pipe_ok(const Dims &, const Params &);
 hipError_t launch_phi_del2(const Dims &, const Params &, const Fields &, hipStream_t);
-hipError_t launch_rstar_exch_phi(const Dims &, const Params &, const Fields &, const long *, const XFields &, const long *, int,
+hipError_t launch_rstar_exch_phi(const Dims &, const Params &, const Fields &, const HaloRec *, const XFields &, const long *, int,
                                  int *, hipStream_t, int fromX, int empNext);
 bool dyn_thermo_takes_gm(const Params &);
 bool gm_phi_fusable(const Dims &, const Params &);
diff --git a/mitgcm_amd/csrc/model.hip b/mitgcm_amd/csrc/model.hip
--- a/mitgcm_amd/csrc/model.hip
+++ b/mitgcm_amd/csrc/model.hip
@@ -133,6 +133,7 @@
   std::map<std::string, double> extra;
   long *d_halo = nullptr;
   long *d_srcOf = nullptr;
+  mgcm::HaloRec *d_haloRec = nullptr;
   int nHalo = 0;
   long *d_haloAll = nullptr;
   int nHaloAll = 0;
@@ -311,14 +312,48 @@
   }
 }
 
+namespace mgcm {
+int mg_build_halo_table(const Dims &d, const long *srcOf, HaloRec *out) {
+  if (d.n3 * d.nTiles >= (1L << 31) || d.nx + d.OLx >= (1 << 15) || d.ny + d.OLy >= (1 << 15)) return -1;
+  const long N2 = d.n2 * d.nTiles;
+  for (long q = 0; q < N2; q++) {
+    const long sq = srcOf[q], at = sq >= 0 ? sq : q;
+    int i, j, iq, jq;
+    mg_ij_of(d, at, i, j);
+    mg_ij_of(d, q, iq, jq);
+    HaloRec h;
+    h.at2 = (int)at;
+    h.base3 = (int)((at / d.n2) * d.n3 + at % d.n2);
+    h.i = (short)i;
+    h.j = (short)j;
+    h.flags = ((iq >= 1 && iq <= d.sNx && jq >= 1 && jq <= d.sNy) ? MG_HR_INTERIOR : 0) | (sq >= 0 ? MG_HR_MAPPED : 0);
+    out[q] = h;
+  }
+  return 0;
+}
+}
+int mgcm_halo_table(int sNx, int sNy, int OLx, int OLy, int Nr, int nTiles, const long *srcOf, int *out) {
+  mgcm::Dims d{};
+  d.sNx = sNx; d.sNy = sNy; d.OLx = OLx; d.OLy = OLy; d.Nr = Nr; d.nTiles = nTiles; d.nT = nTiles;
+  d.nx = sNx + 2 * OLx; d.ny = sNy + 2 * OLy; d.n2 = (long)d.nx * d.ny; d.n3 = d.n2 * Nr;
+  static_assert(sizeof(mgcm::HaloRec) == 4 * sizeof(int), "a HaloRec is four ints to the caller");
+  return mgcm::mg_build_halo_table(d, srcOf, reinterpret_cast<mgcm::HaloRec *>(out));
+}
+
 static int upload_halo(mgcm_model *m) {
   if (m->d_halo) { hipFree(m->d_halo); m->d_halo = nullptr; }
   if (m->d_srcOf) { hipFree(m->d_srcOf); m->d_srcOf = nullptr; }
+  if (m->d_haloRec) { hipFree(m->d_haloRec); m->d_haloRec = nullptr; }
   const long N2 = m->d.n2 * m->d.nTiles;
   std::vector<long> srcOf(N2, -1);
   for (size_t h = 0; h + 1 < m->h_halo.size(); h += 2) srcOf[m->h_halo[h]] = m->h_halo[h + 1];
   HIPCHK(hipMalloc(&m->d_srcOf, N2 * sizeof(long)));
   HIPCHK(hipMemcpy(m->d_srcOf, srcOf.data(), N2 * sizeof(long), hipMemcpyHostToDevice));
+  std::vector<mgcm::HaloRec> rec(N2);
+  if (mgcm::mg_build_halo_table(m->d, srcOf.data(), rec.data()) == 0) {
+    HIPCHK(hipMalloc(&m->d_haloRec, N2 * sizeof(mgcm::HaloRec)));
+    HIPCHK(hipMemcpy(m->d_haloRec, rec.data(), N2 * sizeof(mgcm::HaloRec), hipMemcpyHostToDevice));
+  }
   std::vector<long> loc;
   const long lo = (long)m->d.t0 * m->d.n2, hi = (long)(m->d.t0 + m->d.nT) * m->d.n2;
   for (size_t h = 0; h + 1 < m->h_halo.size(); h += 2)
@@ -855,6 +890,7 @@
   if (m->monBuf) hipFree(m->monBuf);
   if (m->d_halo) hipFree(m->d_halo);
   if (m->d_srcOf) hipFree(m->d_srcOf);
+  if (m->d_haloRec) hipFree(m->d_haloRec);
   if (m->d_haloAll) hipFree(m->d_haloAll);
   for (int q = 0; q < 2; q++) {
     if (m->d_uv[q]) hipFree(m->d_uv[q]);
@@ -1226,9 +1262,9 @@
   return launch_exchange_uv_pairs(da, us, vs, 3, m->d_uvAll[0], m->nUvUAll[0], m->nUvVAll[0], m->stream);
 }
 static hipError_t update_r_star_cg2d(mgcm_model *m, bool sfp = false, bool opEarly = false, bool pcHere = false,
-                                     const int *physNext = nullptr, bool keepFac = false) {
+                                     const int *physNext = nullptr, bool keepFac = false, bool spec = false) {
   return launch_update_r_star_cg2d(all_tiles(m->d), m->p, m->f, m->d_srcOf, m->stream, sfp, opEarly, pcHere, physNext,
-                                   keepFac);
+                                   keepFac, spec);
 }
 
 int mgcm_init(mgcm_model *m) {
@@ -1754,6 +1790,7 @@
   bool pipeOk, phiPipeOk, pipe, hoist, valid, phiPipe, phiNext, empNext;
   bool resFlow, resFlowFold;
   bool spec;
+  bool spec2;
 };
 static StepPlan plan_step(const mgcm_model *m, StepMode mode) {
   const Params &p = m->p;
@@ -1793,20 +1830,21 @@
   pl.resFlowFold = pl.resFlow && pl.dtFused;
   pl.pipeOk = gmFold && pl.sfpFused && pl.endFused && mg_fuse_on(MG_FUSE_PIPE) && p.select_rStar > 0 &&
               p.useRealFreshWaterFlux && p.exactConserv && m->d_srcOf && !totPhiHalo && !pl.resFlow;
-  pl.phiPipeOk = pl.pipeOk && phi_pipe_ok(d, p);
+  pl.phiPipeOk = pl.pipeOk && phi_pipe_ok(d, p) && m->d_haloRec;
   pl.pipe = mode != STEP_PLAIN;
   pl.hoist = mode == STEP_HOIST;
   pl.valid = !pl.pipe || pl.pipeOk;
   pl.phiPipe = pl.pipe && pl.phiPipeOk;
   pl.phiNext = pl.hoist && pl.phiPipe;
   pl.empNext = pl.hoist && p.periodicExternalForcing;
+  pl.spec2 = pl.spec && pl.phiPipe && pl.opEarly && pl.etaX && mg_fuse_on(MG_FUSE_SPEC2);
   pl.ringPhys = !pl.pipe && !pl.ringAside && ringSep && mg_fuse_on(MG_FUSE_RINGP) && phys_ring_ok(d, p, m->f);
   pl.momRing = !pl.ringAside && !pl.ringPhys;
   return pl;
 }
 static int step_layout_bits(const StepPlan &pl) {
   return (pl.dtFused ? 1 : 0) | (pl.forkable && !pl.dtFused ? 4 : 0) | (pl.forkable && pl.forkLate ? 8 : 0) |
-         (pl.pipe ? 16 : 0) | (pl.phiPipe ? 32 : 0) | (pl.spec ? 64 : 0);
+         (pl.pipe ? 16 : 0) | (pl.phiPipe ? 32 : 0) | (pl.spec ? 64 : 0) | (pl.spec2 ? 128 : 0);
 }
 
 static int fork_thermo(mgcm_model *m, bool ring, bool trEx) {
@@ -1846,16 +1884,18 @@
     } else if (dynamics_on(m, pl.momRing)) return -1;
     if (pl.forkEarly) HIPCHK(hipStreamWaitEvent(m->stream, m->evJoin, 0));
     if (pl.rstar)
-      TIMED(K_RSTAR, update_r_star_cg2d(m, pl.sfpFused, pl.opEarly, false, pl.hoist ? m->d_ctr : nullptr, pl.phiNext));
+      TIMED(K_RSTAR, update_r_star_cg2d(m, pl.sfpFused, pl.opEarly, false, pl.hoist ? m->d_ctr : nullptr, pl.phiNext,
+                                        pl.spec2 && pl.hoist));
     if (!pl.sfpFused) TIMED(K_RHS, launch_sfp_rhs(m->d, m->p, m->f, m->stream));
     if (pl.thermoLate && fork_thermo(m, pl.ringAside, pl.trEx)) return -1;
     TIMED(K_CG2D, launch_cg2d(m, m->p.cg2dMaxIters, m->p.cg2dUseMinResSol - 1));
     if (!pl.etaX) TIMED(K_ETA, launch_exch_eta(m->d, m->p, m->f, m->d_srcOf, false, 0, m->stream));
     if (pl.thermoLate) HIPCHK(hipStreamWaitEvent(m->stream, m->evJoin, 0));
-    TIMED(K_CONT, launch_corr_cont(m->d, m->p, m->f, 0, m->stream, pl.etaX ? m->d_srcOf : nullptr, pl.hoist));
+    TIMED(K_CONT, launch_corr_cont(m->d, m->p, m->f, 0, m->stream, pl.etaX ? m->d_srcOf : nullptr, pl.hoist,
+                                   pl.spec2 && pl.hoist));
     if (pl.etaHAlone) TIMED(K_ETA, launch_exch_eta(m->d, m->p, m->f, m->d_srcOf, true, 0, m->stream, fromX));
     if (pl.endFused && pl.phiNext)
-      TIMED(K_RSTAR, launch_rstar_exch_phi(m->d, m->p, m->f, m->d_srcOf, blocking_fields(m, 1, false), m->d_halo, m->nHalo,
+      TIMED(K_RSTAR, launch_rstar_exch_phi(m->d, m->p, m->f, m->d_haloRec, blocking_fields(m, 1, false), m->d_halo, m->nHalo,
                                            m->d_ctr, m->stream, fromX, pl.empNext ? 1 : 0));
     else if (pl.endFused)
       TIMED(K_RSTAR, launch_rstar_exch(m->d, m->p, m->f, m->d_srcOf, pl.fuseEtaH, blocking_fields(m), m->d_halo, m->nHalo,
diff --git a/mitgcm_amd/csrc/phys.h b/mitgcm_amd/csrc/phys.h
--- a/mitgcm_amd/csrc/phys.h
+++ b/mitgcm_amd/csrc/phys.h
@@ -25,18 +25,20 @@
   const double bulkMod = bMfresh + bMsalt + bMpres;
   return rhoP0 / (1.0 - locPres * 1.0e-05 / bulkMod) - p.rhoConst;
 }
+template <class O = OptsRun>
 __device__ __forceinline__ double pressure_for_eos(const Params &p, const Fields &f, int kRef, long q3) {
-  if (p.selectP_inEOS_Zc == 2) return p.rhoConst * (f.totPhiHyd[q3] + f.phiRefC[kRef - 1]) + 0.0;
+  if (O::eosPresFromPhi(p)) return p.rhoConst * (f.totPhiHyd[q3] + f.phiRefC[kRef - 1]) + 0.0;
   return f.pRef4EOS[kRef - 1] + 0.0;
 }
+template <class O = OptsRun>
 __device__ __forceinline__ double find_rho(const Params &p, const Fields &f, int kRef, long q3, double t, double s) {
-  if (p.eosType == 1) return jmd95_rho(p, pressure_for_eos(p, f, kRef, q3), t, s);
+  if (O::eosJmd95(p)) return jmd95_rho(p, pressure_for_eos<O>(p, f, kRef, q3), t, s);
   const double refTemp = f.tRef[kRef - 1], refSalt = f.sRef[kRef - 1];
   const double dRho = p.rhoNil - p.rhoConst;
   return p.rhoNil * (p.sBeta * (s - refSalt) - p.tAlpha * (t - refTemp)) + dRho;
 }
 
-template <bool HOIST>
+template <bool HOIST, class O = OptsRun>
 __device__ __forceinline__ double oceanic_phys_point_t(const Dims &d, const Params &p, const Fields &f, const int *iterPtr,
                                                        const long *__restrict__ srcOf, int i, int j, int k, int t) {
   const long q = MG_I2(d, i, j, t), q31 = MG_I3(d, i, j, 1, t);
@@ -48,9 +50,9 @@
   }
   auto theta_at = [&](int kk) {
     const double v = f.theta[HOIST ? r31 + (long)(kk - 1) * d.n2 : MG_I3(d, i, j, kk, t)];
-    return (kk == 1 && p.allowFreezing && v < -1.9) ? -1.9 : v;
+    return (kk == 1 && O::allowFreezing(p) && v < -1.9) ? -1.9 : v;
   };
-  if (k == 1 && p.periodicExternalForcing) {
+  if (k == 1 && O::periodicForcing(p)) {
     const long N2 = d.n2 * d.nTiles;
     const double cycleLength = p.externForcingCycle, recSpacing = p.externForcingPeriod;
     const double currentTime = (double)(*iterPtr + (HOIST ? 1 : 0)) * p.deltaTClock;
@@ -70,7 +72,7 @@
   }
   if (k == 1) {
     const double th1 = theta_at(1), s1 = f.salt[HOIST ? r31 : q31];
-    if (p.allowFreezing && own) f.theta[q31] = th1;
+    if (O::allowFreezing(p) && own) f.theta[q31] = th1;
     const double mass2rUnit = 1.0 / p.rhoConst, recip_Cp = 1.0 / p.HeatCapacity_Cp;
     const double hFac1 = HOIST ? f.h0FacC[q31] * f.rStarFacC[q] : f.hFacC[q31];
     double sfT = -(f.lambdaThetaClimRelax[q] * (th1 - f.SST[q]) * f.drF[0] * hFac1);
@@ -78,7 +80,7 @@
     sfT = sfT - f.Qnet[q] * recip_Cp * mass2rUnit;
     sfS = sfS - 0.0 * mass2rUnit;
     const double UNSET_RL = 123456.7;
-    if (p.nonlinFreeSurf > 0 && p.useRealFreshWaterFlux) {
+    if (O::nlfs0(p) && O::realFreshWaterFlux(p)) {
       const double pmepr = HOIST ? -f.EmPmR[q] : f.PmEpR[q];
       if (p.temp_EvPrRn != UNSET_RL) sfT = sfT + pmepr * (p.temp_EvPrRn - th1) * mass2rUnit;
       if (p.salt_EvPrRn != UNSET_RL) sfS = sfS + pmepr * (p.salt_EvPrRn - s1) * mass2rUnit;
@@ -94,29 +96,30 @@
   }
   const long q3 = MG_I3(d, i, j, k, t);
   const long r3 = HOIST ? r31 + (long)(k - 1) * d.n2 : q3;
-  const double rho = find_rho(p, f, k, r3, theta_at(k), f.salt[r3]);
+  const double rho = find_rho<O>(p, f, k, r3, theta_at(k), f.salt[r3]);
   f.rhoInSitu[q3] = rho;
-  const bool calcConvect = p.ivdc_kappa != 0.0;
+  const bool calcConvect = O::ivdc(p);
   double conv = 0.0, sigmaR = 0.0;
-  if (k >= 2 && (calcConvect || p.useGMRedi)) {
+  if (k >= 2 && (calcConvect || O::gmRedi(p))) {
     const long q3u = MG_I3(d, i, j, k - 1, t);
-    const double rhoKm1 = find_rho(p, f, k, r3, theta_at(k - 1), f.salt[r3 - d.n2]);
+    const double rhoKm1 = find_rho<O>(p, f, k, r3, theta_at(k - 1), f.salt[r3 - d.n2]);
     sigmaR = f.maskC[q3] * f.maskC[q3u] * f.recip_drC[k - 1] * p.rkSign * (rho - rhoKm1);
     if (calcConvect) conv = (-sigmaR * p.gravitySign > 0.0) ? 1.0 : 0.0;
   }
   f.IVDConvCount[q3] = conv;
-  if (p.useGMRedi) f.sigmaR[q3] = sigmaR;
+  if (O::gmRedi(p)) f.sigmaR[q3] = sigmaR;
   return rho;
 }
 __device__ __forceinline__ double oceanic_phys_point(const Dims &d, const Params &p, const Fields &f, const int *iterPtr,
                                                      int i, int j, int k, int t) {
   return oceanic_phys_point_t<false>(d, p, f, iterPtr, nullptr, i, j, k, t);
 }
+template <class O = OptsRun>
 __device__ __forceinline__ void phys_hoist_body(const Dims &d, const Params &p, const Fields &f, const int *iterPtr,
                                                 const long *__restrict__ srcOf, int lb) {
   MG_PLANE_LB(1 - d.OLx, d.nx, 1 - d.OLy, d.ny, z, lb)
   const int t = d.t0 + z / d.Nr, k = z % d.Nr + 1;
-  oceanic_phys_point_t<true>(d, p, f, iterPtr, srcOf, i, j, k, t);
+  oceanic_phys_point_t<true, O>(d, p, f, iterPtr, srcOf, i, j, k, t);
 }
 inline int phys_hoist_blocks(const Dims &d) { return (int)mg_plane_blocks(d.nx, d.ny, d.nT * d.Nr); }
 
diff --git a/mitgcm_amd/csrc/rstar.h b/mitgcm_amd/csrc/rstar.h
--- a/mitgcm_amd/csrc/rstar.h
+++ b/mitgcm_amd/csrc/rstar.h
@@ -12,43 +12,29 @@
   return fromX ? f.recip_Bo[q] * f.cg2d_x[q] : f.etaN[q];
 }
 
-template <bool NARROW>
-__device__ __forceinline__ void mg_ij_of(const Dims &d, long q, int &i, int &j) {
-  if constexpr (NARROW) {
-    const int l = (int)q % (int)d.n2;
-    i = l % d.nx - d.OLx + 1;
-    j = l / d.nx - d.OLy + 1;
-  } else {
-    const long l = q % d.n2;
-    i = (int)(l % d.nx) - d.OLx + 1;
-    j = (int)(l / d.nx) - d.OLy + 1;
-  }
-}
-
 template <bool FUSE, bool WS = true, bool SHORT = false>
 __device__ __forceinline__ void calc_r_star_fac(const Dims &d, const Params &p, const Fields &f,
-                                                const long *__restrict__ srcOf, long q, int fromX, double oc, double ow,
-                                                double os, double &fc, double &fw, double &fs) {
+                                                const long *__restrict__ srcOf, const HaloRec *__restrict__ rec, long q,
+                                                int fromX, double oc, double ow, double os, double &fc, double &fw,
+                                                double &fs) {
   auto inner = [&](int ii, int jj) { return ii >= 1 && ii <= d.sNx && jj >= 1 && jj <= d.sNy; };
   int i, j;
   long r;
   if constexpr (SHORT) {
-    mg_ij_of<true>(d, q, i, j);
-    r = q;
-    if (!inner(i, j)) {
-      const long sq = srcOf[q];
-      if (sq >= 0) { r = sq; mg_ij_of<true>(d, r, i, j); }
-    }
+    const HaloRec h = rec[q];
+    r = h.at2;
+    i = h.i;
+    j = h.j;
   } else {
     const long sq = srcOf[q];
     r = sq >= 0 ? sq : q;
-    mg_ij_of<false>(d, r, i, j);
+    mg_ij_of(d, r, i, j);
   }
   auto eta = [&](long qq, int ii, int jj) {
     if constexpr (SHORT) {
       if (inner(ii, jj)) return f.cg2d_b[qq];
-      const long sqq = srcOf[qq];
-      if (sqq >= 0) return f.cg2d_b[sqq];
+      const long sqq = rec[qq].at2;
+      if (sqq != qq) return f.cg2d_b[sqq];
       return fromX ? f.recip_Bo[qq] * f.cg2d_x[qq] : f.etaN[qq];
     } else {
       return FUSE ? eta_exch(d, f, srcOf, qq, fromX) : f.etaH[qq];
@@ -62,7 +48,7 @@
   if constexpr (WS) {
     const long rv = (!SHORT && p.cubeCorners) ? q : r;
     int iv = i, jv = j;
-    if constexpr (!SHORT) mg_ij_of<false>(d, rv, iv, jv);
+    if constexpr (!SHORT) mg_ij_of(d, rv, iv, jv);
     if (iv >= 1 && iv <= d.sNx + 1 && jv >= 1 && jv <= d.sNy) {
       if (f.maskInW[rv] != 0.0) {
         const double tmp = f.rSurfW[rv] - f.rLowW[rv];
@@ -82,9 +68,11 @@
   }
 }
 
-template <bool FUSE>
+template <bool FUSE, bool TAB = false>
 __device__ __forceinline__ void calc_r_star_body(const Dims &d, const Params &p, const Fields &f,
-                                                 const long *__restrict__ srcOf, int lb, int fromX, int empNext = 0) {
+                                                 const long *__restrict__ srcOf, int lb, int fromX, int empNext = 0,
+                                                 const HaloRec *__restrict__ rec = nullptr) {
+  static_assert(FUSE || !TAB, "the table form is the fused pass's");
   const long q = (long)lb * blockDim.x + threadIdx.x;
   if (q >= d.n2 * d.nTiles) return;
   const int t = (int)(q / d.n2);
@@ -92,14 +80,20 @@
   if constexpr (FUSE) {
     if (p.nonlinFreeSurf > 0 && p.useRealFreshWaterFlux) f.PmEpR[q] = -f.EmPmR[q];
     if (empNext) f.EmPmR[q] = f.EmPmRnext[q];
-    const double x = eta_exch(d, f, srcOf, q, fromX);
+    double x;
+    if constexpr (TAB) {
+      const HaloRec h = rec[q];
+      x = (h.flags & (MG_HR_INTERIOR | MG_HR_MAPPED)) ? f.cg2d_b[h.at2] : fromX ? f.recip_Bo[q] * f.cg2d_x[q] : f.etaN[q];
+    } else {
+      x = eta_exch(d, f, srcOf, q, fromX);
+    }
     f.etaHnm1[q] = f.etaH[q];
     f.etaN[q] = x;
     f.etaH[q] = x;
   }
   const double oc = f.rStarFacC[q], ow = f.rStarFacW[q], os = f.rStarFacS[q];
   double fc, fw, fs;
-  calc_r_star_fac<FUSE>(d, p, f, srcOf, q, fromX, oc, ow, os, fc, fw, fs);
+  calc_r_star_fac<FUSE, true, TAB>(d, p, f, srcOf, rec, q, fromX, oc, ow, os, fc, fw, fs);
   f.rStarFacC[q] = fc;
   f.rStarFacW[q] = fw;
   f.rStarFacS[q] = fs;
@@ -113,11 +107,11 @@
 
 template <bool WS>
 __device__ __forceinline__ void r_star_next_point(const Dims &d, const Params &p, const Fields &f,
-                                                  const long *__restrict__ srcOf, long q, int fromX, double &facC,
+                                                  const HaloRec *__restrict__ rec, long q, int fromX, double &facC,
                                                   double &dhC, double &dhW, double &dhS) {
   const double oc = f.rStarFacCPrev[q], ow = WS ? f.rStarFacWPrev[q] : 0.0, os = WS ? f.rStarFacSPrev[q] : 0.0;
   double fc, fw, fs;
-  calc_r_star_fac<true, WS, true>(d, p, f, srcOf, q, fromX, oc, ow, os, fc, fw, fs);
+  calc_r_star_fac<true, WS, true>(d, p, f, nullptr, rec, q, fromX, oc, ow, os, fc, fw, fs);
   facC = fc;
   dhC = (fc - oc) / p.deltaTFreeSurf;
   if constexpr (WS) {
@@ -126,11 +120,9 @@
   }
 }
 
-__device__ __forceinline__ long mg_at_source3(const Dims &d, const long *__restrict__ srcOf, int i, int j, int k, int t) {
-  if (i >= 1 && i <= d.sNx && j >= 1 && j <= d.sNy) return MG_I3(d, i, j, k, t);
-  const long sq = srcOf[MG_I2(d, i, j, t)];
-  if (sq < 0) return MG_I3(d, i, j, k, t);
-  return (sq / d.n2) * d.n3 + (long)(k - 1) * d.n2 + sq % d.n2;
+__device__ __forceinline__ long mg_at_source3(const Dims &d, const HaloRec *__restrict__ rec, int i, int j, int t) {
+  if (i >= 1 && i <= d.sNx && j >= 1 && j <= d.sNy) return MG_I3(d, i, j, 1, t);
+  return rec[MG_I2(d, i, j, t)].base3;
 }
 
 }
diff --git a/mitgcm_amd/model.py b/mitgcm_amd/model.py
--- a/mitgcm_amd/model.py
+++ b/mitgcm_amd/model.py
@@ -251,7 +251,7 @@
         b = int(lib().mgcm_get_param(self.h, b"stepLayout"))
         return {"dyn_thermo_fused": bool(b & 1), "thermo_second_stream": bool(b & 4),
                 "late_join": bool(b & 8), "pipelined": bool(b & 16), "phi_pipelined": bool(b & 32),
-                "specialised": bool(b & 64)}
+                "specialised": bool(b & 64), "solve_side_specialised": bool(b & 128)}
 
     def ptracers_route(self):
         r = int(lib().mgcm_get_param(self.h, b"ptrRoute"))
```

New measurement: 4153 model-days/s, median of 6. 1.8% higher.
